# mycrazycracy/speaker-embedding-with-phonetic-information

Hardware: AMD Instinct MI355X
Metric: utterance-embeddings/sec (400-frame chunks) (higher is better)
Workload: dtype fp16mx; 1 GPU; v2_xvector TDNN, 256 chunks x 400 frames per GPU per step, utterance-sharded, weights broadcast once over RCCL; topology=v2_xvector, batch_chunks_per_gpu=256, frames_per_chunk=400, precision=default, arithmetic=fp16mx, lanes=2, output_node=embedding, chunk_lengths=400, library=xvec_hip 0.4 (gfx950; kernels 1123b5fc04a88fd3)

## Files before the change

### include/xvec_hip.h

```cpp
#ifndef XVEC_HIP_H_
#define XVEC_HIP_H_

#include <stddef.h>
#include <stdint.h>

#ifdef __cplusplus
extern "C" {
#endif

typedef enum {
  XV_OK = 0,
  XV_ERR_IO = 1,
  XV_ERR_MODEL = 2,
  XV_ERR_DEVICE = 3,
  XV_ERR_ARG = 4,
  XV_ERR_INTERNAL = 5
} xv_status;

typedef enum {
  XV_PREC_DEFAULT = -1,
  XV_PREC_BF16X3 = 0,
  XV_PREC_BF16 = 1,
  XV_PREC_FP16 = 2,
  XV_PREC_FP16X3 = 3,
// ... 55 lines not shown
  int32_t lite_dropped;
  float tail;
} xv_calibration;
xv_status xv_ctx_calibrate(xv_ctx* c, const float* feats, const int32_t* row_offsets, int32_t B, float tol, xv_calibration* out);
xv_status xv_ctx_set_fast_mode(xv_ctx* c, int32_t precision);
xv_status xv_ctx_fast_mode(const xv_ctx* c, int32_t* precision);
xv_status xv_ctx_set_lite_layers(xv_ctx* c, uint64_t mask);
xv_status xv_ctx_lite_layers(const xv_ctx* c, uint64_t* mask);
xv_status xv_calibrate_table(xv_ctx* c, const char* feature_rspecifier, int32_t chunk_size, int32_t min_chunk_size,
                             int32_t pad_input, int32_t max_utts, float tol, xv_calibration* out);
xv_status xv_ctx_set_calibration(xv_ctx* c, int32_t enable, float tol);
xv_status xv_calibration_file_read(const char* path, int32_t* found, uint64_t* model, int32_t* precision, uint64_t* lite_mask);
xv_status xv_calibration_file_publish(const char* path, uint64_t model, int32_t precision, uint64_t lite_mask, float tol,
                                      const char* note, int32_t* published, uint64_t* adopted_model, int32_t* adopted_precision,
                                      uint64_t* adopted_lite_mask);
xv_status xv_ctx_model_fingerprint(const xv_ctx* c, uint64_t* fingerprint);
xv_status xv_ctx_share_calibration(xv_ctx* c, const char* path, float tol, const char* note, int32_t* outcome);
xv_status xv_ctx_set_calibration_file(xv_ctx* c, const char* path);

xv_status xv_ctx_set_profiling(xv_ctx* c, int32_t enable);
size_t xv_ctx_profile_report(xv_ctx* c, char* buf, size_t n);

xv_status xv_extract_utterances(xv_ctx* c, const float* feats, const int32_t* row_offsets, int32_t n_utts,
                                int32_t chunk_size, int32_t min_chunk_size, int32_t pad_input, float* out,
                                int32_t* ok);

xv_status xv_extract_table(xv_ctx* c, const char* feature_rspecifier, const char* vector_wspecifier, int32_t chunk_size,
                           int32_t min_chunk_size, int32_t pad_input, int32_t batch_frames, int64_t* num_done,
                           int64_t* num_failed);

xv_status xv_recognize_feature_pipeline(const char* rspecifier, int32_t* found, char* feats, size_t feats_cap, char* vad, size_t vad_cap,
                                        int32_t* cmn_window, int32_t* min_cmn_window, int32_t* center);
xv_status xv_frontend_cmvn_select(xv_ctx* c, const float* raw, const int32_t* raw_off, int32_t n_utts, const float* vad,
                                  int32_t cmn_window, int32_t center, float* out, int32_t* out_off);

xv_status xv_plan_chunks(int32_t num_rows, int32_t chunk_size, int32_t min_chunk_size, int32_t pad_input,
                         int32_t min_net_frames, int32_t cap, int32_t* start, int32_t* len, int32_t* left_pad,
                         int32_t* right_pad, int32_t* n_chunks);

xv_status xv_ctx_create_broadcast(const xv_model* m, const int* devices, int n, int precision, xv_ctx** out);

xv_status xv_backend_apply(int device, const float* x, int32_t n, int32_t dim, const float* mean, const float* transform,
                           int32_t t_rows, int32_t t_cols, int32_t normalize, int32_t scaleup, float* out, float* ratio);
xv_status xv_segment_mean(int device, const float* x, int32_t n, int32_t dim, const int32_t* seg_off, const int32_t* idx,
                          int32_t n_seg, int32_t acc64, float* out);

xv_status xv_scatter_stats(int device, const float* x, int32_t n, int32_t dim, const int32_t* seg_off, const int32_t* idx,
                           int32_t n_seg, double* s_tot, double* sums, double* s_bet, float* device_ms);
xv_status xv_plda_transform(int device, const float* x, int32_t n, int32_t dim, const double* transform, const double* offset,
                            const double* psi, const double* num, int32_t normalize, int32_t simple, float* y, double* scale,
                            float* device_ms);
xv_status xv_plda_score(int device, const float* u, const double* num_u, int32_t n_u, const float* v, int32_t n_v, int32_t dim,
                        const double* psi, const int32_t* trials, int64_t n_trials, double* scores, float* device_ms);
xv_status xv_lda_estimate(int32_t dim, int64_t n, const double* s_tot, const double* s_bet, const float* mean,
                          double total_covariance_factor, double covariance_floor, int32_t lda_dim, float* out, int32_t* n_floored);
xv_status xv_plda_estimate(int32_t dim, int32_t n_spk, const double* sums, const int32_t* counts, const double* s_tot,
                           const double* s_bet, int32_t num_em_iters, double* mean, double* transform, double* psi,
                           int32_t* n_floored);
xv_status xv_plda_adapt(int32_t dim, int64_t n, const double* m, const double* v, const double* mean, const double* transform,
                        const double* psi, double mean_diff_scale, double within_covar_scale, double between_covar_scale,
                        double* mean_out, double* transform_out, double* psi_out, double* s_out);

typedef struct {
  float sample_frequency, frame_length_ms, frame_shift_ms, dither, preemphasis_coefficient, blackman_coeff;
  int32_t remove_dc_offset, window_type, round_to_power_of_two, snip_edges;
  int32_t num_mel_bins;
  float low_freq, high_freq;
  int32_t num_ceps;
  float cepstral_lifter;
  int32_t use_energy, raw_energy;
  float energy_floor;
} xv_mfcc_options;
typedef struct {
  float vad_energy_threshold, vad_energy_mean_scale, vad_proportion_threshold;
  int32_t vad_frames_context;
} xv_vad_options;
void xv_mfcc_options_default(xv_mfcc_options* opts);
int64_t xv_mfcc_num_frames(const xv_mfcc_options* opts, int64_t n_samples);
uint64_t xv_mfcc_utt_seed(const char* key);
xv_status xv_mfcc_compute(int device, const xv_mfcc_options* opts, const float* samples, const int64_t* sample_offsets,
                          int32_t n_utts, const uint64_t* utt_seeds, float* out, int32_t* out_row_offsets);
xv_status xv_mfcc_compute_i16(int device, const xv_mfcc_options* opts, const int16_t* samples, const int64_t* sample_offsets,
                              int32_t n_utts, const uint64_t* utt_seeds, float* out, int32_t* out_row_offsets);
xv_status xv_mfcc_kernel_time(int device, const xv_mfcc_options* opts, const int16_t* samples, const int64_t* sample_offsets,
                              int32_t n_utts, int32_t reps, float* kernel_ms);
xv_status xv_vad_energy(int device, const xv_vad_options* vad_opts, const float* feats, const int32_t* row_offsets,
                        int32_t n_utts, int32_t dim, float* out);
xv_status xv_wave_read(const char* rxfilename, int32_t channel, int32_t* rate, int16_t** samples, int64_t* n);
void xv_wave_free(int16_t* samples);

typedef struct {
  int32_t shift_output, normalize_output;
  float duration, volume;
  int32_t input_wave_channel, rir_channel, noise_channel;
} xv_reverb_options;
void xv_reverb_options_default(xv_reverb_options* opts);
int64_t xv_reverb_output_length(const xv_reverb_options* opts, float sample_rate, int64_t n_samples, int64_t rir_len);
xv_status xv_wav_reverberate(int device, const xv_reverb_options* opts, float sample_rate, const void* samples,
                             int32_t samples_are_i16, const int64_t* sample_offsets, int32_t n_utts, const float* rirs,
                             const int64_t* rir_offsets, int32_t n_rirs, const int32_t* utt_rir, const float* noises,
                             const int64_t* noise_offsets, int32_t n_noises, const int32_t* utt_add_offsets,
                             const int32_t* add_noise, const float* add_snr, const float* add_start, int64_t* out_offsets,
                             float* out_f32, int16_t* out_i16, int64_t* clipped);
xv_status xv_reverb_kernel_time(int device, const xv_reverb_options* opts, float sample_rate, const void* samples,
                                int32_t samples_are_i16, const int64_t* sample_offsets, int32_t n_utts, const float* rirs,
                                const int64_t* rir_offsets, int32_t n_rirs, const int32_t* utt_rir, const float* noises,
                                const int64_t* noise_offsets, int32_t n_noises, const int32_t* utt_add_offsets,
                                const int32_t* add_noise, const float* add_snr, const float* add_start, int32_t reps,
                                float* kernel_ms);
xv_status xv_recognize_wav_pipeline(const char* rxfilename, int32_t* found, char* description, size_t description_cap);
xv_status xv_wave_write(const char* wxfilename, int32_t rate, const float* samples, int64_t n, int64_t* clipped);

typedef struct {
  const void* hi;
  const void* lo;
  int32_t ld;
  int32_t row_shift;
  int32_t k_len;
  const void* gmax;
  const void* lo4; const void* lo4_scale;
} xv_seg_desc;
typedef struct {
  int32_t precision, epilogue;
  int32_t nseg;
  xv_seg_desc seg[8];
  const void* w_hi; const void* w_lo; int32_t ldw;
  int32_t rows;
  int32_t n_pad;
  const float* bias; const float* scale; const float* offset;
  int32_t relu, bn;
  void* out_hi; void* out_lo; int32_t ldo;
  float* out_f32; int32_t ldf; int32_t m_valid;
  float* partial; int32_t ldp; const int8_t* grp_range;
  void* hip_stream;
  const void* w4; int32_t ldw4; const void* w4_scale;
  void* gmax_out;
  const void* w4b; int32_t ldw4b; const void* w4b_scale;
  void* out_lo4; void* out_lo4_scale;
  int32_t p8;
  const int8_t* out_range;
  int32_t ksplit;
} xv_gemm_desc;
xv_status xv_pack_mx_residual(const float* w, const uint16_t* w_hi_f16, int32_t n_pad, int32_t nseg,
                              const int32_t* seg_src, const int32_t* seg_shift, const int32_t* seg_klen, uint8_t* w4,
                              uint8_t* w4_scale);
xv_status xv_pack_mx_residual64(const float* w, const uint16_t* w_hi_f16, int32_t n_pad, int32_t nseg, const int32_t* seg_src,
                                const int32_t* seg_shift, const int32_t* seg_klen, uint8_t* w4, uint8_t* w4_scale);
xv_status xv_pack_mx_weights(const float* w, int32_t n_pad, int32_t nseg, const int32_t* seg_src, const int32_t* seg_shift,
                             const int32_t* seg_klen, uint8_t* w4b, uint8_t* w4b_scale);
xv_status xv_pack_mx_weights64(const float* w, int32_t n_pad, int32_t nseg, const int32_t* seg_src, const int32_t* seg_shift,
                               const int32_t* seg_klen, uint8_t* w4b, uint8_t* w4b_scale);
xv_status xv_tile_mx_scales(const uint8_t* natural, int32_t n_pad, int32_t k_len, int32_t epilogue, uint8_t* tiled);
xv_status xv_kernel_tdnn_gemm(const xv_gemm_desc* d);

xv_status xv_compressed_size(int32_t rows, int32_t cols, int32_t method, size_t* nbytes, const char** format);
xv_status xv_compress_matrices(int device, const float* feats, const int32_t* row_off, int32_t n, int32_t cols, int32_t method,
                               uint8_t* out_bytes, int64_t* out_off, int32_t* nonfinite_flags);
xv_status xv_compress_kernel_time(int device, const float* feats, const int32_t* row_off, int32_t n, int32_t cols, int32_t method,
                                  int32_t reps, float* kernel_ms);
xv_status xv_cmvn_sliding(int device, const float* raw, const int32_t* raw_off, int32_t n, int32_t cols, int32_t cmn_window,
                          int32_t min_cmn_window, int32_t center, float* out);

xv_status xv_cmvn_stats(int device, const float* feats, const int32_t* row_off, int32_t n_utts, int32_t cols, double* stats,
                        float* device_ms);
xv_status xv_cmvn_norm(const double* stats, int32_t cols, int32_t norm_means, int32_t norm_vars, int32_t reverse,
                       const int32_t* skip_dims, int32_t n_skip, float* norm, int32_t* num_floored);
xv_status xv_cmvn_apply(int device, const float* feats, const int32_t* row_off, int32_t n_utts, int32_t cols, const float* norms,
                        const int32_t* utt_norm, float* out);
xv_status xv_cmvn_kernel_time(int device, const float* feats, const int32_t* row_off, int32_t n_utts, int32_t cols, int32_t reps,
                              float* stats_ms, float* apply_ms);

typedef struct {
  const float* feats;
  const int32_t* row_offsets;
  const int32_t* dev_off;
  int32_t B;
  int32_t rows;
  int32_t pad_left, pad_right;
  int32_t dim, noff;
  int32_t off[8];
  const void* w_hi; const void* w_lo;
  int32_t ldw, seg_pad;
  int32_t n_pad;
  int32_t epi_prec;
  const float* bias; const float* scale; const float* offset;
  int32_t relu, bn;
  void* out_hi; void* out_lo; int32_t ldo;
  void* out_lo4; void* out_lo4_scale;
  void* gmax_out; const int8_t* out_range;
  int32_t row0, nrows;
  int32_t max_wgs;
  void* hip_stream;
} xv_first_layer_desc;
xv_status xv_kernel_first_layer(const xv_first_layer_desc* d);
typedef struct {
  int32_t precision;
  const float* feats; const int32_t* src_off; const int32_t* dev_off; const int32_t* grp_utt;
  int32_t rows;
  int32_t dim, ld;
  void* out_hi; void* out_lo;
  int32_t pad_left, pad_right;
  void* zero_words; int32_t n_zero_words;
  void* hip_stream;
} xv_prep_input_desc;
xv_status xv_kernel_prep_input(const xv_prep_input_desc* d);
typedef struct {
  int32_t precision;
  const float* partial; int32_t ldp;
  const int32_t* utt_grp0; const int32_t* utt_grp1; const int32_t* utt_count;
  int32_t B, dim;
  float var_floor;
  void* out_hi; void* out_lo; int32_t ld;
  void* hip_stream;
} xv_pool_finalise_desc;
xv_status xv_kernel_pool_finalise(const xv_pool_finalise_desc* d);
typedef struct {
  const float* src; const void* src16; int32_t ld;
  const int32_t* out_row; int32_t n_out;
  int32_t dim, log_softmax;
  float* out; int32_t out_ld;
  void* hip_stream;
} xv_frame_output_desc;
xv_status xv_kernel_frame_output(const xv_frame_output_desc* d);

#ifdef __cplusplus
}
#endif
#endif
```

### speaker-embedding-with-phonetic-information_amd/__init__.py

```python
import ctypes
import os
import subprocess
import sys

_HERE = os.path.dirname(os.path.abspath(__file__))
CSRC = os.path.join(_HERE, "csrc")
LIB_PATH = os.environ.get("XVEC_LIB") or os.path.join(_HERE, "libxvec_hip.so")
BIN_DIR = os.path.join(_HERE, "bin")

XV_OK = 0
XV_ERR_IO, XV_ERR_MODEL, XV_ERR_DEVICE, XV_ERR_ARG, XV_ERR_INTERNAL = 1, 2, 3, 4, 5
PREC_BF16X3, PREC_BF16, PREC_FP16, PREC_FP16X3, PREC_FP16X2, PREC_AUTO, PREC_FP16MX, PREC_FP16MX2, PREC_FP16X3E = range(9)
PREC_DEFAULT = -1
PRECISIONS = {"default": PREC_DEFAULT, "bf16x3": PREC_BF16X3, "bf16": PREC_BF16, "fp16": PREC_FP16, "fp16x3": PREC_FP16X3,
              "fp16x2": PREC_FP16X2, "auto": PREC_AUTO, "fp16mx": PREC_FP16MX, "fp16mx2": PREC_FP16MX2}
PRECISION_NAMES = {v: k for k, v in PRECISIONS.items()}
MFMA_PASSES = {"bf16x3": 3, "bf16": 1, "fp16": 1, "fp16x3": 3, "fp16x2": 2, "fp16mx": 1.25}
EPI_ACT, EPI_F32, EPI_STATS = 0, 1, 2


class XvError(RuntimeError):
    def __init__(self, status, msg):
        super().__init__("xvec_hip status %d: %s" % (status, msg))
        self.status = status


class ModelInfo(ctypes.Structure):
    _fields_ = [(n, ctypes.c_int32) for n in ("input_dim", "output_dim", "left_context", "right_context",
                                              "min_frames", "num_layers", "output_is_segment", "reserved")]


class SegDesc(ctypes.Structure):
    _fields_ = [("hi", ctypes.c_void_p), ("lo", ctypes.c_void_p), ("ld", ctypes.c_int32),
                ("row_shift", ctypes.c_int32), ("k_len", ctypes.c_int32), ("gmax", ctypes.c_void_p),
                ("lo4", ctypes.c_void_p), ("lo4_scale", ctypes.c_void_p)]


class GemmDesc(ctypes.Structure):
    _fields_ = [("precision", ctypes.c_int32), ("epilogue", ctypes.c_int32), ("nseg", ctypes.c_int32),
                ("seg", SegDesc * 8),
                ("w_hi", ctypes.c_void_p), ("w_lo", ctypes.c_void_p), ("ldw", ctypes.c_int32),
                ("rows", ctypes.c_int32), ("n_pad", ctypes.c_int32),
                ("bias", ctypes.c_void_p), ("scale", ctypes.c_void_p), ("offset", ctypes.c_void_p),
                ("relu", ctypes.c_int32), ("bn", ctypes.c_int32),
                ("out_hi", ctypes.c_void_p), ("out_lo", ctypes.c_void_p), ("ldo", ctypes.c_int32),
                ("out_f32", ctypes.c_void_p), ("ldf", ctypes.c_int32), ("m_valid", ctypes.c_int32),
                ("partial", ctypes.c_void_p), ("ldp", ctypes.c_int32), ("grp_range", ctypes.c_void_p),
                ("hip_stream", ctypes.c_void_p),
                ("w4", ctypes.c_void_p), ("ldw4", ctypes.c_int32), ("w4_scale", ctypes.c_void_p),
                ("gmax_out", ctypes.c_void_p),
                ("w4b", ctypes.c_void_p), ("ldw4b", ctypes.c_int32), ("w4b_scale", ctypes.c_void_p),
                ("out_lo4", ctypes.c_void_p), ("out_lo4_scale", ctypes.c_void_p),
                ("p8", ctypes.c_int32),
                ("out_range", ctypes.c_void_p), ("ksplit", ctypes.c_int32)]


class FirstLayerDesc(ctypes.Structure):
    _fields_ = [("feats", ctypes.c_void_p), ("row_offsets", ctypes.c_void_p), ("dev_off", ctypes.c_void_p), ("B", ctypes.c_int32),
                ("rows", ctypes.c_int32), ("pad_left", ctypes.c_int32), ("pad_right", ctypes.c_int32),
                ("dim", ctypes.c_int32), ("noff", ctypes.c_int32), ("off", ctypes.c_int32 * 8),
                ("w_hi", ctypes.c_void_p), ("w_lo", ctypes.c_void_p), ("ldw", ctypes.c_int32), ("seg_pad", ctypes.c_int32),
                ("n_pad", ctypes.c_int32), ("epi_prec", ctypes.c_int32),
                ("bias", ctypes.c_void_p), ("scale", ctypes.c_void_p), ("offset", ctypes.c_void_p),
                ("relu", ctypes.c_int32), ("bn", ctypes.c_int32),
                ("out_hi", ctypes.c_void_p), ("out_lo", ctypes.c_void_p), ("ldo", ctypes.c_int32),
                ("out_lo4", ctypes.c_void_p), ("out_lo4_scale", ctypes.c_void_p),
                ("gmax_out", ctypes.c_void_p), ("out_range", ctypes.c_void_p),
                ("row0", ctypes.c_int32), ("nrows", ctypes.c_int32), ("max_wgs", ctypes.c_int32),
                ("hip_stream", ctypes.c_void_p)]


class PrepInputDesc(ctypes.Structure):
    _fields_ = [("precision", ctypes.c_int32), ("feats", ctypes.c_void_p), ("src_off", ctypes.c_void_p), ("dev_off", ctypes.c_void_p),
                ("grp_utt", ctypes.c_void_p), ("rows", ctypes.c_int32), ("dim", ctypes.c_int32), ("ld", ctypes.c_int32),
                ("out_hi", ctypes.c_void_p), ("out_lo", ctypes.c_void_p), ("pad_left", ctypes.c_int32), ("pad_right", ctypes.c_int32),
                ("zero_words", ctypes.c_void_p), ("n_zero_words", ctypes.c_int32), ("hip_stream", ctypes.c_void_p)]


class PoolFinaliseDesc(ctypes.Structure):
    _fields_ = [("precision", ctypes.c_int32), ("partial", ctypes.c_void_p), ("ldp", ctypes.c_int32),
                ("utt_grp0", ctypes.c_void_p), ("utt_grp1", ctypes.c_void_p), ("utt_count", ctypes.c_void_p),
                ("B", ctypes.c_int32), ("dim", ctypes.c_int32), ("var_floor", ctypes.c_float),
                ("out_hi", ctypes.c_void_p), ("out_lo", ctypes.c_void_p), ("ld", ctypes.c_int32), ("hip_stream", ctypes.c_void_p)]


class FrameOutputDesc(ctypes.Structure):
    _fields_ = [("src", ctypes.c_void_p), ("src16", ctypes.c_void_p), ("ld", ctypes.c_int32),
                ("out_row", ctypes.c_void_p), ("n_out", ctypes.c_int32), ("dim", ctypes.c_int32), ("log_softmax", ctypes.c_int32),
                ("out", ctypes.c_void_p), ("out_ld", ctypes.c_int32), ("hip_stream", ctypes.c_void_p)]


class Calibration(ctypes.Structure):
    _fields_ = [("chosen", ctypes.c_int32), ("checked", ctypes.c_int32), ("err_mx", ctypes.c_float), ("err_mx2", ctypes.c_float),
                ("checked_mx", ctypes.c_int32), ("err_lite", ctypes.c_float), ("lite_mask", ctypes.c_uint64),
                ("err_holdout", ctypes.c_float), ("checked_holdout", ctypes.c_int32), ("lite_dropped", ctypes.c_int32),
                ("tail", ctypes.c_float)]

    def as_dict(self):
        d = {"chosen": PRECISION_NAMES.get(self.chosen, str(self.chosen)), "checked": self.checked, "checked_mx": self.checked_mx,
             "err_mx": self.err_mx, "err_mx2": self.err_mx2, "tail": self.tail}
        if self.lite_mask:
            d["lite_mask"] = int(self.lite_mask)
            d["err_lite"] = self.err_lite
            d["err_holdout"] = self.err_holdout
            d["checked_holdout"] = self.checked_holdout
        if self.lite_dropped:
            d["lite_dropped"] = self.lite_dropped
        return d


ABI_SYMBOLS = [
    "xv_last_error", "xv_version", "xv_model_load", "xv_model_load_rxfilename", "xv_model_free", "xv_model_info",
    "xv_model_macs", "xv_model_describe", "xv_model_pack", "xv_ctx_create", "xv_ctx_create_from_blob",
    "xv_ctx_create_from_device_blob", "xv_ctx_free",
    "xv_ctx_info", "xv_forward_batch", "xv_forward_batch_device", "xv_ctx_synchronize", "xv_ctx_set_profiling",
    "xv_ctx_profile_report", "xv_extract_utterances", "xv_ctx_calibrate", "xv_ctx_set_fast_mode", "xv_ctx_fast_mode",
    "xv_calibrate_table", "xv_ctx_set_calibration", "xv_ctx_model_fingerprint", "xv_ctx_share_calibration",
    "xv_ctx_set_calibration_file", "xv_calibration_file_read", "xv_calibration_file_publish", "xv_recognize_feature_pipeline", "xv_ctx_set_lite_layers", "xv_ctx_lite_layers",
    "xv_extract_table", "xv_frontend_cmvn_select", "xv_plan_chunks", "xv_ctx_create_broadcast", "xv_kernel_tdnn_gemm",
    "xv_backend_apply", "xv_segment_mean", "xv_scatter_stats", "xv_plda_transform", "xv_plda_score", "xv_lda_estimate",
    "xv_plda_estimate", "xv_plda_adapt",
    "xv_mfcc_options_default", "xv_mfcc_num_frames", "xv_mfcc_utt_seed", "xv_mfcc_compute", "xv_mfcc_compute_i16", "xv_mfcc_kernel_time", "xv_vad_energy",
    "xv_reverb_options_default", "xv_reverb_output_length", "xv_wav_reverberate", "xv_reverb_kernel_time", "xv_wave_write", "xv_recognize_wav_pipeline",
    "xv_compressed_size", "xv_compress_matrices", "xv_compress_kernel_time", "xv_cmvn_sliding",
    "xv_cmvn_stats", "xv_cmvn_norm", "xv_cmvn_apply", "xv_cmvn_kernel_time",
    "xv_kernel_first_layer", "xv_kernel_prep_input", "xv_kernel_pool_finalise", "xv_kernel_frame_output",
    "xv_wave_read", "xv_wave_free", "xv_pack_mx_residual", "xv_pack_mx_residual64", "xv_tile_mx_scales", "xv_pack_mx_weights", "xv_pack_mx_weights64",
]

_lib = None


def build(verbose=False):
    cmd = ["make", "-C", CSRC, "-j8"]
    res = subprocess.run(cmd, stdout=subprocess.PIPE, stderr=subprocess.STDOUT, text=True)
    if verbose or res.returncode != 0:
        print(res.stdout)
    if res.returncode != 0:
        raise RuntimeError("building libxvec_hip.so failed")
    return LIB_PATH


def lib():
    global _lib
    if _lib is not None:
        return _lib
    if not os.path.exists(LIB_PATH):
        raise ImportError("%s is missing - run `python -c 'import __graft_entry__ as g; g.build()'` "
                          "(there is no Python/CPU fallback for the HIP path)" % LIB_PATH)
    if os.environ.get("XVEC_NO_TORCH_PRELOAD", "") != "1":
        try:
            import torch
        except Exception:
            pass
    L = ctypes.CDLL(LIB_PATH)
    L.xv_last_error.restype = ctypes.c_char_p
    L.xv_version.restype = ctypes.c_char_p
    L.xv_model_macs.restype = ctypes.c_double
    L.xv_model_macs.argtypes = [ctypes.c_void_p, ctypes.c_int32]
    L.xv_model_describe.restype = ctypes.c_size_t
    L.xv_model_describe.argtypes = [ctypes.c_void_p, ctypes.c_char_p, ctypes.c_size_t]
    L.xv_model_load.argtypes = [ctypes.c_void_p, ctypes.c_size_t, ctypes.c_char_p, ctypes.c_char_p,
                                ctypes.POINTER(ctypes.c_void_p)]
    L.xv_model_load_rxfilename.argtypes = [ctypes.c_char_p, ctypes.c_char_p, ctypes.c_char_p,
                                           ctypes.POINTER(ctypes.c_void_p)]
    L.xv_model_free.argtypes = [ctypes.c_void_p]
    L.xv_model_free.restype = None
    L.xv_model_info.argtypes = [ctypes.c_void_p, ctypes.POINTER(ModelInfo)]
    L.xv_model_pack.argtypes = [ctypes.c_void_p, ctypes.c_int, ctypes.c_void_p, ctypes.POINTER(ctypes.c_size_t)]
    L.xv_ctx_create.argtypes = [ctypes.c_void_p, ctypes.c_int, ctypes.c_int, ctypes.POINTER(ctypes.c_void_p)]
    L.xv_ctx_create_from_blob.argtypes = [ctypes.c_void_p, ctypes.c_size_t, ctypes.c_int,
                                          ctypes.POINTER(ctypes.c_void_p)]
    L.xv_ctx_create_from_device_blob.argtypes = [ctypes.c_void_p, ctypes.c_size_t, ctypes.c_int,
                                                 ctypes.POINTER(ctypes.c_void_p)]
    L.xv_pack_mx_residual.argtypes = [ctypes.c_void_p, ctypes.c_void_p, ctypes.c_int32, ctypes.c_int32, ctypes.c_void_p,
                                      ctypes.c_void_p, ctypes.c_void_p, ctypes.c_void_p, ctypes.c_void_p]
    L.xv_pack_mx_residual64.argtypes = L.xv_pack_mx_residual.argtypes
    L.xv_pack_mx_weights.argtypes = [ctypes.c_void_p, ctypes.c_int32, ctypes.c_int32, ctypes.c_void_p, ctypes.c_void_p,
                                     ctypes.c_void_p, ctypes.c_void_p, ctypes.c_void_p]
    L.xv_pack_mx_weights64.argtypes = L.xv_pack_mx_weights.argtypes
    L.xv_tile_mx_scales.argtypes = [ctypes.c_void_p, ctypes.c_int32, ctypes.c_int32, ctypes.c_int32, ctypes.c_void_p]
    L.xv_ctx_free.argtypes = [ctypes.c_void_p]
    L.xv_ctx_free.restype = None
    L.xv_ctx_info.argtypes = [ctypes.c_void_p, ctypes.POINTER(ModelInfo), ctypes.POINTER(ctypes.c_int32),
                              ctypes.POINTER(ctypes.c_int32)]
    L.xv_forward_batch.argtypes = [ctypes.c_void_p, ctypes.c_void_p, ctypes.c_void_p, ctypes.c_int32, ctypes.c_void_p]
    L.xv_forward_batch_device.argtypes = [ctypes.c_void_p, ctypes.c_void_p, ctypes.c_void_p, ctypes.c_int32,
                                          ctypes.c_void_p, ctypes.c_int32, ctypes.c_void_p]
    L.xv_ctx_synchronize.argtypes = [ctypes.c_void_p]
    L.xv_ctx_set_profiling.argtypes = [ctypes.c_void_p, ctypes.c_int32]
    L.xv_ctx_profile_report.argtypes = [ctypes.c_void_p, ctypes.c_char_p, ctypes.c_size_t]
    L.xv_ctx_profile_report.restype = ctypes.c_size_t
    L.xv_extract_utterances.argtypes = [ctypes.c_void_p, ctypes.c_void_p, ctypes.c_void_p, ctypes.c_int32,
                                        ctypes.c_int32, ctypes.c_int32, ctypes.c_int32, ctypes.c_void_p, ctypes.c_void_p]
    L.xv_ctx_create_broadcast.argtypes = [ctypes.c_void_p, ctypes.POINTER(ctypes.c_int), ctypes.c_int, ctypes.c_int,
                                          ctypes.POINTER(ctypes.c_void_p)]
    L.xv_kernel_tdnn_gemm.argtypes = [ctypes.POINTER(GemmDesc)]
    L.xv_kernel_first_layer.argtypes = [ctypes.POINTER(FirstLayerDesc)]
    L.xv_kernel_prep_input.argtypes = [ctypes.POINTER(PrepInputDesc)]
    L.xv_kernel_pool_finalise.argtypes = [ctypes.POINTER(PoolFinaliseDesc)]
    L.xv_kernel_frame_output.argtypes = [ctypes.POINTER(FrameOutputDesc)]
    L.xv_ctx_calibrate.argtypes = [ctypes.c_void_p, ctypes.c_void_p, ctypes.c_void_p, ctypes.c_int32, ctypes.c_float,
                                   ctypes.POINTER(Calibration)]
    L.xv_ctx_set_fast_mode.argtypes = [ctypes.c_void_p, ctypes.c_int32]
    L.xv_ctx_fast_mode.argtypes = [ctypes.c_void_p, ctypes.POINTER(ctypes.c_int32)]
    L.xv_ctx_set_lite_layers.argtypes = [ctypes.c_void_p, ctypes.c_uint64]
    L.xv_ctx_lite_layers.argtypes = [ctypes.c_void_p, ctypes.POINTER(ctypes.c_uint64)]
    L.xv_calibrate_table.argtypes = [ctypes.c_void_p, ctypes.c_char_p, ctypes.c_int32, ctypes.c_int32, ctypes.c_int32,
                                     ctypes.c_int32, ctypes.c_float, ctypes.POINTER(Calibration)]
    L.xv_ctx_set_calibration.argtypes = [ctypes.c_void_p, ctypes.c_int32, ctypes.c_float]
    L.xv_ctx_model_fingerprint.argtypes = [ctypes.c_void_p, ctypes.POINTER(ctypes.c_uint64)]
    L.xv_ctx_share_calibration.argtypes = [ctypes.c_void_p, ctypes.c_char_p, ctypes.c_float, ctypes.c_char_p,
                                           ctypes.POINTER(ctypes.c_int32)]
    L.xv_ctx_set_calibration_file.argtypes = [ctypes.c_void_p, ctypes.c_char_p]
    L.xv_calibration_file_read.argtypes = [ctypes.c_char_p, ctypes.POINTER(ctypes.c_int32), ctypes.POINTER(ctypes.c_uint64),
                                           ctypes.POINTER(ctypes.c_int32), ctypes.POINTER(ctypes.c_uint64)]
    L.xv_calibration_file_publish.argtypes = [ctypes.c_char_p, ctypes.c_uint64, ctypes.c_int32, ctypes.c_uint64, ctypes.c_float,
                                              ctypes.c_char_p, ctypes.POINTER(ctypes.c_int32), ctypes.POINTER(ctypes.c_uint64),
                                              ctypes.POINTER(ctypes.c_int32), ctypes.POINTER(ctypes.c_uint64)]
    _lib = L
    return L


def _check(status):
    if status != XV_OK:
        raise XvError(status, lib().xv_last_error().decode(errors="replace"))


class Model:

    def __init__(self, raw=None, rxfilename=None, nnet_config=None, output_node=None):
        L = lib()
        self._h = ctypes.c_void_p()
        cfg = nnet_config.encode() if nnet_config else None
        node = output_node.encode() if output_node else None
        if raw is not None:
            buf = ctypes.create_string_buffer(bytes(raw), len(raw))
            _check(L.xv_model_load(buf, len(raw), cfg, node, ctypes.byref(self._h)))
        else:
            _check(L.xv_model_load_rxfilename(rxfilename.encode(), cfg, node, ctypes.byref(self._h)))

    def __del__(self):
        if getattr(self, "_h", None) and self._h.value and lib is not None:
            lib().xv_model_free(self._h)
            self._h = ctypes.c_void_p()

    @property
    def info(self):
        mi = ModelInfo()
        _check(lib().xv_model_info(self._h, ctypes.byref(mi)))
        return mi

    def macs(self, frames):
        return lib().xv_model_macs(self._h, int(frames))

    def describe(self):
        n = lib().xv_model_describe(self._h, None, 0)
        buf = ctypes.create_string_buffer(n)
        lib().xv_model_describe(self._h, buf, n)
        return buf.value.decode()

    def pack(self, precision=PREC_DEFAULT):
        n = ctypes.c_size_t(0)
        _check(lib().xv_model_pack(self._h, precision, None, ctypes.byref(n)))
        buf = ctypes.create_string_buffer(n.value)
        _check(lib().xv_model_pack(self._h, precision, buf, ctypes.byref(n)))
        return buf.raw[:n.value]


class Context:

    def __init__(self, model=None, blob=None, device=0, precision=PREC_DEFAULT, device_blob=None):
# ... 608 lines not shown
                add_noise.append(len(noise_list) - 1)
                add_snr.append(snr)
                add_start.append(start)
            add_off[u + 1] = len(add_noise)
    noise_flat, noise_off = _ragged(noise_list, np.float32)
    add_noise = np.array(add_noise + [0], dtype=np.int32)
    add_snr = np.array(add_snr + [0], dtype=np.float32)
    add_start = np.array(add_start + [0], dtype=np.float32)
    lens = [reverb_output_length(off[u + 1] - off[u], rir_off[utt_rir[u] + 1] - rir_off[utt_rir[u]] if utt_rir[u] >= 0 else 0,
                                 rate, options=o) for u in range(n)]
    total = max(1, sum(max(0, x) for x in lens))
    common = (device, ctypes.byref(o), float(rate), samples.ctypes.data, 1 if i16 else 0, off.ctypes.data, n,
              rir_flat.ctypes.data, rir_off.ctypes.data, len(rir_list), utt_rir.ctypes.data,
              noise_flat.ctypes.data, noise_off.ctypes.data, len(noise_list), add_off.ctypes.data if additive is not None else None,
              add_noise.ctypes.data, add_snr.ctypes.data, add_start.ctypes.data)
    if kernel_time_reps > 0:
        L.xv_reverb_kernel_time.argtypes = _REVERB_ARGTYPES + [ctypes.c_int32, ctypes.POINTER(ctypes.c_float)]
        ms = ctypes.c_float(0)
        _check(L.xv_reverb_kernel_time(*common, int(kernel_time_reps), ctypes.byref(ms)))
        return ms.value
    out = np.empty(total, dtype=np.float32)
    out16 = np.empty(total, dtype=np.int16) if return_int16 else None
    clipped = np.zeros(max(1, n), dtype=np.int64)
    out_off = np.zeros(n + 1, dtype=np.int64)
    L.xv_wav_reverberate.argtypes = _REVERB_ARGTYPES + [ctypes.c_void_p, ctypes.c_void_p, ctypes.c_void_p, ctypes.c_void_p]
    _check(L.xv_wav_reverberate(*common, out_off.ctypes.data, out.ctypes.data, out16.ctypes.data if return_int16 else None,
                                clipped.ctypes.data))
    assert list(np.diff(out_off)) == [max(0, x) for x in lens]
    if return_int16:
        return [(out[out_off[u]:out_off[u + 1]].copy(), out16[out_off[u]:out_off[u + 1]].copy(), int(clipped[u])) for u in range(n)]
    return [out[out_off[u]:out_off[u + 1]].copy() for u in range(n)]


def _pack_matrices(mats, what):
    import numpy as np
    ms = [np.ascontiguousarray(m, dtype=np.float32) for m in mats]
    if any(m.ndim != 2 for m in ms):
        raise XvError(XV_ERR_ARG, "%s: every matrix must be two-dimensional" % what)
    widths = {m.shape[1] for m in ms if m.shape[0] > 0}
    if len(widths) > 1:
        raise XvError(XV_ERR_ARG, "%s: the matrices of one call share their column count" % what)
    cols = widths.pop() if widths else 0
    off = np.zeros(len(ms) + 1, dtype=np.int32)
    off[1:] = np.cumsum([m.shape[0] if cols else 0 for m in ms])
    rows = [m for m in ms if m.shape[0] > 0 and cols]
    packed = np.concatenate(rows, axis=0) if rows else np.zeros((0, max(cols, 1)), np.float32)
    return np.ascontiguousarray(packed), off, cols


def compressed_size(rows, cols, method=1):
    L = lib()
    n, fmt = ctypes.c_size_t(0), ctypes.c_char_p()
    L.xv_compressed_size.argtypes = [ctypes.c_int32, ctypes.c_int32, ctypes.c_int32, ctypes.POINTER(ctypes.c_size_t),
                                     ctypes.POINTER(ctypes.c_char_p)]
    _check(L.xv_compressed_size(rows, cols, method, ctypes.byref(n), ctypes.byref(fmt)))
    return int(n.value), fmt.value.decode()


def compress(mats, method=1, device=0, return_flags=False, kernel_time_reps=0):
    import numpy as np
    L = lib()
    packed, off, cols = _pack_matrices(mats, "compress")
    n = len(off) - 1
    common = [device, packed.ctypes.data if packed.size else None, off.ctypes.data, n, cols, method]
    types = [ctypes.c_int, ctypes.c_void_p, ctypes.c_void_p, ctypes.c_int32, ctypes.c_int32, ctypes.c_int32]
    if kernel_time_reps > 0:
        ms = ctypes.c_float(0)
        L.xv_compress_kernel_time.argtypes = types + [ctypes.c_int32, ctypes.POINTER(ctypes.c_float)]
        _check(L.xv_compress_kernel_time(*common, int(kernel_time_reps), ctypes.byref(ms)))
        return ms.value
    total = sum(compressed_size(int(off[u + 1] - off[u]), cols, method)[0] for u in range(n))
    out = np.zeros(max(1, total), dtype=np.uint8)
    out_off = np.zeros(n + 1, dtype=np.int64)
    flags = np.zeros(max(1, n), dtype=np.int32)
    L.xv_compress_matrices.argtypes = types + [ctypes.c_void_p, ctypes.c_void_p, ctypes.c_void_p]
    _check(L.xv_compress_matrices(*common, out.ctypes.data, out_off.ctypes.data, flags.ctypes.data))
    assert int(out_off[n]) == total
    objs = [out[out_off[u]:out_off[u + 1]].tobytes() for u in range(n)]
    return (objs, [bool(f) for f in flags[:n]]) if return_flags else objs


def cmvn_sliding(mats, cmn_window=600, min_cmn_window=100, center=False, device=0):
    import numpy as np
    L = lib()
    packed, off, cols = _pack_matrices(mats, "cmvn_sliding")
    n = len(off) - 1
    out = np.empty_like(packed)
    L.xv_cmvn_sliding.argtypes = [ctypes.c_int, ctypes.c_void_p, ctypes.c_void_p, ctypes.c_int32, ctypes.c_int32, ctypes.c_int32,
                                  ctypes.c_int32, ctypes.c_int32, ctypes.c_void_p]
    _check(L.xv_cmvn_sliding(device, packed.ctypes.data if packed.size else None, off.ctypes.data, n, max(cols, 1), cmn_window,
                             min_cmn_window, 1 if center else 0, out.ctypes.data if out.size else None))
    return [out[off[u]:off[u + 1]].copy() for u in range(n)]


def cmvn_stats(feats_list, device=0, kernel_time_reps=0):
    import numpy as np
    L = lib()
    packed, off, cols = _pack_matrices(feats_list, "cmvn_stats")
    n = len(off) - 1
    if cols < 1:
        raise XvError(XV_ERR_ARG, "cmvn_stats: no matrix with rows and columns")
    if kernel_time_reps > 0:
        a, b = ctypes.c_float(0), ctypes.c_float(0)
        L.xv_cmvn_kernel_time.argtypes = [ctypes.c_int, ctypes.c_void_p, ctypes.c_void_p, ctypes.c_int32, ctypes.c_int32, ctypes.c_int32,
                                          ctypes.POINTER(ctypes.c_float), ctypes.POINTER(ctypes.c_float)]
        _check(L.xv_cmvn_kernel_time(device, packed.ctypes.data, off.ctypes.data, n, cols, int(kernel_time_reps), ctypes.byref(a),
                                     ctypes.byref(b)))
        return a.value, b.value
    stats = np.zeros((n, 2, cols + 1), dtype=np.float64)
    L.xv_cmvn_stats.argtypes = [ctypes.c_int, ctypes.c_void_p, ctypes.c_void_p, ctypes.c_int32, ctypes.c_int32, ctypes.c_void_p,
                                ctypes.c_void_p]
    _check(L.xv_cmvn_stats(device, packed.ctypes.data if packed.size else None, off.ctypes.data, n, cols, stats.ctypes.data, None))
    return stats


def cmvn_norm(stats, norm_means=True, norm_vars=False, reverse=False, skip_dims=(), return_floored=False):
    import numpy as np
    L = lib()
    st = np.ascontiguousarray(stats, dtype=np.float64)
    if st.ndim != 2 or st.shape[0] != 2 or st.shape[1] < 2:
        raise XvError(XV_ERR_ARG, "cmvn_norm: the statistics are a [2][cols + 1] matrix")
    cols = st.shape[1] - 1
    skip = np.ascontiguousarray(list(skip_dims), dtype=np.int32)
    norm = np.zeros((2, cols), dtype=np.float32)
    floored = ctypes.c_int32(0)
    L.xv_cmvn_norm.argtypes = [ctypes.c_void_p, ctypes.c_int32, ctypes.c_int32, ctypes.c_int32, ctypes.c_int32, ctypes.c_void_p,
                               ctypes.c_int32, ctypes.c_void_p, ctypes.POINTER(ctypes.c_int32)]
    _check(L.xv_cmvn_norm(st.ctypes.data, cols, int(bool(norm_means)), int(bool(norm_vars)), int(bool(reverse)),
                          skip.ctypes.data if skip.size else None, int(skip.size), norm.ctypes.data, ctypes.byref(floored)))
    return (norm, int(floored.value)) if return_floored else norm


def apply_cmvn(feats_list, norms, utt_norm, device=0):
    import numpy as np
    L = lib()
    packed, off, cols = _pack_matrices(feats_list, "apply_cmvn")
    n = len(off) - 1
    nm = np.ascontiguousarray(norms, dtype=np.float32)
    un = np.ascontiguousarray(utt_norm, dtype=np.int32)
    if un.shape != (n,) or nm.ndim != 3 or nm.shape[1:] != (2, max(cols, 1)) or (n and (un.min() < 0 or un.max() >= nm.shape[0])):
        raise XvError(XV_ERR_ARG, "apply_cmvn: norms are [n_norms][2][cols] and utt_norm names one of them per matrix")
    out = np.empty_like(packed)
    L.xv_cmvn_apply.argtypes = [ctypes.c_int, ctypes.c_void_p, ctypes.c_void_p, ctypes.c_int32, ctypes.c_int32, ctypes.c_void_p,
                                ctypes.c_void_p, ctypes.c_void_p]
    _check(L.xv_cmvn_apply(device, packed.ctypes.data if packed.size else None, off.ctypes.data, n, max(cols, 1), nm.ctypes.data,
                           un.ctypes.data, out.ctypes.data if out.size else None))
    return [out[off[u]:off[u + 1]].copy() for u in range(n)]


def kernel_tdnn_gemm(desc):
    _check(lib().xv_kernel_tdnn_gemm(ctypes.byref(desc)))


def kernel_first_layer(desc):
    _check(lib().xv_kernel_first_layer(ctypes.byref(desc)))


def kernel_prep_input(desc):
    _check(lib().xv_kernel_prep_input(ctypes.byref(desc)))


def kernel_pool_finalise(desc):
    _check(lib().xv_kernel_pool_finalise(ctypes.byref(desc)))


def kernel_frame_output(desc):
    _check(lib().xv_kernel_frame_output(ctypes.byref(desc)))


def pack_mx_residual(w, w_hi_f16, segs, walk64=False):
    import numpy as np
    w = np.ascontiguousarray(w, dtype=np.float32)
    hi = np.ascontiguousarray(w_hi_f16, dtype=np.uint16)
    n_pad, K = w.shape
    src = np.array([s[0] for s in segs], dtype=np.int32)
    shift = np.array([s[1] for s in segs], dtype=np.int32)
    klen = np.array([s[2] for s in segs], dtype=np.int32)
    assert int(klen.sum()) == K and K % 128 == 0
    w4 = np.zeros((n_pad, K // 128 * 64), dtype=np.uint8)
    sc = np.zeros((n_pad, K // 32), dtype=np.uint8)
    fn = lib().xv_pack_mx_residual64 if walk64 else lib().xv_pack_mx_residual
    _check(fn(w.ctypes.data, hi.ctypes.data, n_pad, len(segs), src.ctypes.data, shift.ctypes.data,
              klen.ctypes.data, w4.ctypes.data, sc.ctypes.data))
    return w4, sc


def pack_mx_weights(w, segs, walk64=False):
    import numpy as np
    w = np.ascontiguousarray(w, dtype=np.float32)
    n_pad, K = w.shape
    src = np.array([s[0] for s in segs], dtype=np.int32)
    shift = np.array([s[1] for s in segs], dtype=np.int32)
    klen = np.array([s[2] for s in segs], dtype=np.int32)
    assert int(klen.sum()) == K and np.all(klen % (256 if walk64 else 128) == 0)
    w4b = np.zeros((n_pad, 2 * K if walk64 else K // 2), dtype=np.uint8)
    sc = np.zeros((n_pad, K // 32), dtype=np.uint8)
    fn = lib().xv_pack_mx_weights64 if walk64 else lib().xv_pack_mx_weights
    _check(fn(w.ctypes.data, n_pad, len(segs), src.ctypes.data, shift.ctypes.data, klen.ctypes.data, w4b.ctypes.data, sc.ctypes.data))
    return w4b, sc


def tile_mx_scales(scales, epilogue):
    import numpy as np
    sc = np.ascontiguousarray(scales, dtype=np.uint8)
    out = np.zeros(sc.size, dtype=np.uint8)
    _check(lib().xv_tile_mx_scales(sc.ctypes.data, sc.shape[0], sc.shape[1] * 32, int(epilogue), out.ctypes.data))
    return out
```

### speaker-embedding-with-phonetic-information_amd/csrc/capi.cc

```cpp
#include <dlfcn.h>
#include <stdlib.h>
#include <string.h>

#include <algorithm>
#include <memory>
#include <string>
#include <vector>

#include "../../include/xvec_hip.h"
#include "backend.h"
#include "cmvn.h"
#include "compress.h"
#include "engine.h"
#include "extractor.h"
#include "feat.h"
#include "reverb.h"
#include "wave.h"
#include "kernels.h"
#include "calib_file.h"
#include "fuse_pipe.h"
#include "fuse_wav.h"
#include "multi_gpu.h"
#include "nnet3_raw.h"
#include "plda.h"
#include "plda_kernels.h"
#include "program.h"
#include "table_extract.h"

struct xv_model {
  xv::TdnnProgram prog;
};

struct xv_ctx {
  std::unique_ptr<xv::Engine> eng;
  bool calibrate = false;
  float calibrate_tol = 7.5e-5f;
  std::string calibration_file;
};

namespace {

thread_local std::string g_err;

xv_status Fail(xv_status s, const std::string& m) {
  g_err = m;
  return s;
}

template <class F>
xv_status Guard(F&& f) {
  try {
    g_err.clear();
    return f();
  } catch (const xv::KioError& e) {
    return Fail(XV_ERR_IO, e.what());
  } catch (const xv::EngineError& e) {
    return Fail(XV_ERR_DEVICE, e.what());
  } catch (const std::bad_alloc&) {
    return Fail(XV_ERR_INTERNAL, "out of host memory");
  } catch (const std::exception& e) {
    return Fail(XV_ERR_INTERNAL, e.what());
  } catch (...) {
    return Fail(XV_ERR_INTERNAL, "unknown exception");
  }
}

void FillInfo(const xv::BlobInfo& b, xv_model_info_t* info) {
  memset(info, 0, sizeof *info);
  info->input_dim = b.input_dim;
  info->output_dim = b.output_dim;
  info->left_context = b.left_context;
  info->right_context = b.right_context;
  info->min_frames = b.min_frames;
  info->num_layers = (int32_t)b.layers.size();
  info->output_is_segment = b.output_is_segment;
}

xv_status LoadCommon(xv::RawNnet& net, const char* nnet_config, const char* output_node, xv_model** out) {
  if (nnet_config && *nnet_config) net.ApplyNnetConfig(nnet_config);
  std::unique_ptr<xv_model> m(new xv_model);
  try {
    m->prog = xv::LowerToProgram(net, output_node && *output_node ? output_node : "output");
  } catch (const xv::KioError& e) {
    return Fail(XV_ERR_MODEL, e.what());
  }
  *out = m.release();
  return XV_OK;
}

}

extern "C" {

const char* xv_last_error(void) { return g_err.c_str(); }
#ifndef XVEC_KERNELS_SHA
#define XVEC_KERNELS_SHA "unknown"
#endif
#ifdef XVEC_SCHED_FUZZ
#define XVEC_BUILD_KIND "; schedule-fuzzing build"
#else
#define XVEC_BUILD_KIND ""
#endif
const char* xv_version(void) { return "xvec_hip 0.4 (gfx950; kernels " XVEC_KERNELS_SHA XVEC_BUILD_KIND ")"; }

xv_status xv_model_load(const void* raw, size_t n, const char* nnet_config, const char* output_node, xv_model** out) {
  if (!raw || !out) return Fail(XV_ERR_ARG, "xv_model_load: null argument");
  return Guard([&] {
    xv::RawNnet net;
    net.Read(std::string((const char*)raw, n));
    return LoadCommon(net, nnet_config, output_node, out);
  });
}

xv_status xv_model_load_rxfilename(const char* rxfilename, const char* nnet_config, const char* output_node,
                                   xv_model** out) {
  if (!rxfilename || !out) return Fail(XV_ERR_ARG, "xv_model_load_rxfilename: null argument");
  return Guard([&] {
    xv::RawNnet net;
    net.ReadFrom(rxfilename);
    return LoadCommon(net, nnet_config, output_node, out);
  });
}

void xv_model_free(xv_model* m) { delete m; }

xv_status xv_model_info(const xv_model* m, xv_model_info_t* info) {
  if (!m || !info) return Fail(XV_ERR_ARG, "xv_model_info: null argument");
  memset(info, 0, sizeof *info);
  info->input_dim = m->prog.input_dim;
  info->output_dim = m->prog.output_dim;
  info->left_context = m->prog.left_context;
  info->right_context = m->prog.right_context;
  info->min_frames = m->prog.min_frames;
  info->num_layers = (int32_t)m->prog.layers.size();
  info->output_is_segment = m->prog.output_is_segment;
  return XV_OK;
}

double xv_model_macs(const xv_model* m, int32_t frames) { return m ? m->prog.Macs(frames) : 0.0; }

size_t xv_model_describe(const xv_model* m, char* buf, size_t n) {
  if (!m) return 0;
  const std::string s = m->prog.Describe();
  if (buf && n) {
    const size_t k = s.size() < n - 1 ? s.size() : n - 1;
    memcpy(buf, s.data(), k);
    buf[k] = 0;
  }
  return s.size() + 1;
}

xv_status xv_model_pack(const xv_model* m, int precision, void* blob, size_t* nbytes) {
  if (!m || !nbytes) return Fail(XV_ERR_ARG, "xv_model_pack: null argument");
  return Guard([&] {
    std::vector<uint8_t> b = xv::PackModelPolicy(m->prog, precision);
    if (blob) {
      if (*nbytes < b.size()) return Fail(XV_ERR_ARG, "xv_model_pack: buffer too small");
      memcpy(blob, b.data(), b.size());
    }
    *nbytes = b.size();
    return XV_OK;
  });
}

xv_status xv_ctx_create(const xv_model* m, int device, int precision, xv_ctx** out) {
  if (!m || !out) return Fail(XV_ERR_ARG, "xv_ctx_create: null argument");
  return Guard([&] {
    std::vector<uint8_t> b = xv::PackModelPolicy(m->prog, precision);
    std::unique_ptr<xv_ctx> c(new xv_ctx);
    c->eng.reset(new xv::Engine(b.data(), b.size(), device));
    *out = c.release();
// ... 724 lines not shown
    size_t total = 0;
    for (int u = 0; u < n; ++u) {
      size_t nb = 0;
      xv::CompressedSize(row_off[u + 1] - row_off[u], cols, method, &nb, nullptr);
      total += nb;
    }
    std::vector<uint8_t> out(total + 1);
    float best = 0.f;
    for (int r = 0; r <= reps; ++r) {
      float ms = 0.f;
      xv::CompressMatrices(device, feats, row_off, n, cols, method, out.data(), off.data(), nullptr, &ms);
      if (r == 1 || (r > 1 && ms < best)) best = ms;
    }
    *kernel_ms = best;
    return XV_OK;
  });
}

xv_status xv_cmvn_sliding(int device, const float* raw, const int32_t* raw_off, int32_t n, int32_t cols, int32_t cmn_window,
                          int32_t min_cmn_window, int32_t center, float* out) {
  if (n < 0 || cols < 1 || !raw_off) return Fail(XV_ERR_ARG, "xv_cmvn_sliding: bad argument");
  return Guard([&] {
    xv::CmvnSliding(device, raw, raw_off, n, cols, cmn_window, min_cmn_window, center != 0, out);
    return XV_OK;
  });
}

xv_status xv_cmvn_stats(int device, const float* feats, const int32_t* row_off, int32_t n_utts, int32_t cols, double* stats,
                        float* device_ms) {
  if (n_utts < 0 || cols < 1 || !row_off || (n_utts > 0 && !stats)) return Fail(XV_ERR_ARG, "xv_cmvn_stats: bad argument");
  return Guard([&] {
    xv::CmvnStats(device, feats, row_off, n_utts, cols, stats, device_ms);
    return XV_OK;
  });
}

xv_status xv_cmvn_norm(const double* stats, int32_t cols, int32_t norm_means, int32_t norm_vars, int32_t reverse,
                       const int32_t* skip_dims, int32_t n_skip, float* norm, int32_t* num_floored) {
  return Guard([&] {
    try {
      const int floored = xv::CmvnNorm(stats, cols, norm_means != 0, norm_vars != 0, reverse != 0, skip_dims, n_skip, norm);
      if (num_floored) *num_floored = floored;
    } catch (const xv::CmvnArgError& e) {
      return Fail(XV_ERR_ARG, e.what());
    }
    return XV_OK;
  });
}

xv_status xv_cmvn_apply(int device, const float* feats, const int32_t* row_off, int32_t n_utts, int32_t cols, const float* norms,
                        const int32_t* utt_norm, float* out) {
  if (n_utts < 0 || cols < 1 || !row_off || (n_utts > 0 && (!utt_norm || !norms))) return Fail(XV_ERR_ARG, "xv_cmvn_apply: bad argument");
  int n_norms = 0;
  for (int u = 0; u < n_utts; ++u) {
    if (utt_norm[u] < 0) return Fail(XV_ERR_ARG, "xv_cmvn_apply: negative norm index");
    n_norms = utt_norm[u] + 1 > n_norms ? utt_norm[u] + 1 : n_norms;
  }
  return Guard([&] {
    xv::CmvnApply(device, feats, row_off, n_utts, cols, norms, n_norms, utt_norm, out);
    return XV_OK;
  });
}

xv_status xv_cmvn_kernel_time(int device, const float* feats, const int32_t* row_off, int32_t n_utts, int32_t cols, int32_t reps,
                              float* stats_ms, float* apply_ms) {
  if (!feats || !row_off || !stats_ms || !apply_ms || n_utts < 1 || cols < 1 || reps < 1)
    return Fail(XV_ERR_ARG, "xv_cmvn_kernel_time: bad argument");
  return Guard([&] {
    std::vector<double> stats((size_t)n_utts * 2 * (cols + 1));
    std::vector<float> norms((size_t)n_utts * 2 * cols), out((size_t)row_off[n_utts] * cols);
    std::vector<int32_t> utt_norm(n_utts);
    float best_s = 0.f, best_a = 0.f;
    for (int r = 0; r <= reps; ++r) {
      float ms = 0.f;
      xv::CmvnStats(device, feats, row_off, n_utts, cols, stats.data(), &ms);
      if (r == 1 || (r > 1 && ms < best_s)) best_s = ms;
      if (r == 0)
        for (int u = 0; u < n_utts; ++u) {
          utt_norm[u] = u;
          xv::CmvnNorm(stats.data() + (size_t)u * 2 * (cols + 1), cols, true, true, false, nullptr, 0, norms.data() + (size_t)u * 2 * cols);
        }
      xv::CmvnApply(device, feats, row_off, n_utts, cols, norms.data(), n_utts, utt_norm.data(), out.data(), &ms);
      if (r == 1 || (r > 1 && ms < best_a)) best_a = ms;
    }
    *stats_ms = best_s;
    *apply_ms = best_a;
    return XV_OK;
  });
}

xv_status xv_ctx_create_broadcast(const xv_model* m, const int* devices, int n, int precision, xv_ctx** out) {
  if (!m || !devices || !out || n < 1) return Fail(XV_ERR_ARG, "xv_ctx_create_broadcast: bad argument");
  return Guard([&]() -> xv_status {
    const std::vector<uint8_t> blob = xv::PackModelPolicy(m->prog, precision);
    std::vector<std::unique_ptr<xv::Engine>> engines = xv::CreateEnginesBroadcast(blob, std::vector<int>(devices, devices + n));
    for (int i = 0; i < n; ++i) {
      xv_ctx* c = new xv_ctx;
      c->eng = std::move(engines[i]);
      out[i] = c;
    }
    return XV_OK;
  });
}

xv_status xv_kernel_tdnn_gemm(const xv_gemm_desc* d) {
  if (!d) return Fail(XV_ERR_ARG, "xv_kernel_tdnn_gemm: null descriptor");
  return Guard([&] {
    if (d->nseg < 1 || d->nseg > xv::kMaxSeg || d->rows % xv::kBM || d->n_pad % xv::kBN)
      return Fail(XV_ERR_ARG, "xv_kernel_tdnn_gemm: bad geometry");
    xv::GemmArgs a;
    memset(&a, 0, sizeof a);
    a.nseg = d->nseg;
    for (int j = 0; j < d->nseg; ++j) {
      if (d->seg[j].k_len % xv::kBK) return Fail(XV_ERR_ARG, "xv_kernel_tdnn_gemm: k_len must be a multiple of 32");
      a.seg[j].hi = (const uint16_t*)d->seg[j].hi;
      a.seg[j].lo = (const uint16_t*)d->seg[j].lo;
      a.seg[j].ld = d->seg[j].ld;
      a.seg[j].row_shift = d->seg[j].row_shift;
      a.seg[j].ksteps = d->seg[j].k_len / xv::kBK;
      a.seg[j].gmax = (const unsigned*)d->seg[j].gmax;
      a.seg[j].lo4 = (const uint8_t*)d->seg[j].lo4;
      a.seg[j].lo4s = (const uint8_t*)d->seg[j].lo4_scale;
      a.total_ksteps += a.seg[j].ksteps;
    }
    a.w_hi = (const uint16_t*)d->w_hi;
    a.w_lo = (const uint16_t*)d->w_lo;
    a.ldw = d->ldw;
    a.m_tiles = d->rows / xv::kBM;
    a.n_tiles = d->n_pad / xv::kBN;
    a.relu = d->relu;
    a.bn = d->bn;
    a.bias = d->bias;
    a.scale = d->scale;
    a.offset = d->offset;
    a.out_hi = (uint16_t*)d->out_hi;
    a.out_lo = (uint16_t*)d->out_lo;
    a.ldo = d->ldo;
    a.out_f32 = d->out_f32;
    a.ldf = d->ldf;
    a.m_valid = d->m_valid;
    a.partial = d->partial;
    a.ldp = d->ldp;
    a.grp_range = d->grp_range;
    a.w4 = (const uint8_t*)d->w4;
    a.ldw4 = d->ldw4;
    a.w4_scale = (const uint8_t*)d->w4_scale;
    a.gmax_out = (unsigned*)d->gmax_out;
    a.w4b = (const uint8_t*)d->w4b;
    a.ldw4b = d->ldw4b;
    a.w4b_scale = (const uint8_t*)d->w4b_scale;
    a.out_lo4 = (uint8_t*)d->out_lo4;
    a.out_lo4s = (uint8_t*)d->out_lo4_scale;
    a.p8 = d->p8;
    a.out_range = d->out_range;
    if (d->ksplit > 1) {
      if (d->precision < xv::kPrecBf16x3 || d->precision > xv::kPrecFp16x3 || a.p8 ||
          (d->epilogue != xv::kEpiAct && d->epilogue != xv::kEpiF32))
        return Fail(XV_ERR_ARG, "xv_kernel_tdnn_gemm: split-K needs XV_PREC_BF16X3 .. XV_PREC_FP16X3, epilogue 0 or 1 and no p8");
      a.ksteps_per_slice = xv::SplitKStepsPerSlice(a.total_ksteps);
      a.ksplit = (a.total_ksteps + a.ksteps_per_slice - 1) / a.ksteps_per_slice;
      if (a.ksplit != d->ksplit)
        return Fail(XV_ERR_ARG, "xv_kernel_tdnn_gemm: " + std::to_string(a.total_ksteps) + " K steps are split over " +
                                    std::to_string(a.ksplit) + " slices, not " + std::to_string(d->ksplit));
      void* ws = nullptr;
      hipError_t e = hipMalloc(&ws, (size_t)a.ksplit * d->rows * d->n_pad * 4);
      if (e != hipSuccess) return Fail(XV_ERR_DEVICE, std::string("hipMalloc(split-K workspace): ") + hipGetErrorString(e));
      a.splitk_ws = (float*)ws;
      e = xv::launch_tdnn_gemm(a, d->precision, d->epilogue, (hipStream_t)d->hip_stream);
      const hipError_t e2 = hipStreamSynchronize((hipStream_t)d->hip_stream);
      (void)hipFree(ws);
      if (e != hipSuccess || e2 != hipSuccess)
        return Fail(XV_ERR_DEVICE, std::string("tdnn_gemm split-K launch: ") + hipGetErrorString(e != hipSuccess ? e : e2));
      return XV_OK;
    }
    if (a.p8) {
      if (!xv::gemm_p8_applicable(a, d->precision) || (d->epilogue != xv::kEpiAct && d->epilogue != xv::kEpiStats))
        return Fail(XV_ERR_ARG, "xv_kernel_tdnn_gemm: p8 needs XV_PREC_FP16, XV_PREC_FP16MX or XV_PREC_FP16MX2, epilogue 0 or 2, rows and n_pad "
                                "multiples of 256, K groups of whole 64-column tiles (128-column blocks for XV_PREC_FP16MX, 256 for XV_PREC_FP16MX2)");
    } else
    if (d->precision == xv::kPrecFp16Mx2 && !xv::gemm_mx2_applicable(a))
      return Fail(XV_ERR_ARG, "xv_kernel_tdnn_gemm: XV_PREC_FP16MX2 needs what XV_PREC_FP16MX needs and the 4-bit planes of the "
                              "weights and of every source (whole 128-column steps)");
    if (!a.p8 && d->precision == xv::kPrecFp16Mx && !xv::gemm_mx_applicable(a))
      return Fail(XV_ERR_ARG, "xv_kernel_tdnn_gemm: XV_PREC_FP16MX needs the residual plane, a group-max table per source, "
                              "K groups of whole 128-column blocks and an even number of 128-row tiles");
    hipError_t e = xv::launch_tdnn_gemm(a, d->precision, d->epilogue, (hipStream_t)d->hip_stream);
    if (e != hipSuccess) return Fail(XV_ERR_DEVICE, std::string("tdnn_gemm launch: ") + hipGetErrorString(e));
    return XV_OK;
  });
}

namespace {
struct DevMem {
  void* p = nullptr;
  ~DevMem() {
    if (p) (void)hipFree(p);
  }
  hipError_t Alloc(size_t n) { return hipMalloc(&p, n ? n : 1); }
};
}

xv_status xv_kernel_first_layer(const xv_first_layer_desc* d) {
  if (!d) return Fail(XV_ERR_ARG, "xv_kernel_first_layer: null descriptor");
  return Guard([&] {
    const char* who = "xv_kernel_first_layer: ";
    if (!d->feats || !d->row_offsets || !d->dev_off || !d->w_hi || !d->w_lo || !d->bias || !d->out_hi || (d->bn && (!d->scale || !d->offset)))
      return Fail(XV_ERR_ARG, std::string(who) + "a required pointer is null");
    const int p = d->epi_prec;
    if (p != xv::kPrecBf16x3 && p != xv::kPrecFp16x3 && p != xv::kPrecFp16x2 && p != xv::kPrecFp16x3E)
      return Fail(XV_ERR_ARG, std::string(who) + "epi_prec must be XV_PREC_BF16X3, XV_PREC_FP16X3, XV_PREC_FP16X2 or XV_PREC_FP16X3E");
    if ((p == xv::kPrecBf16x3 || p == xv::kPrecFp16x3) && !d->out_lo) return Fail(XV_ERR_ARG, std::string(who) + "the split planes need out_lo");
    if (p == xv::kPrecFp16x3E && (!d->out_lo4 || !d->out_lo4_scale))
      return Fail(XV_ERR_ARG, std::string(who) + "XV_PREC_FP16X3E needs out_lo4 and out_lo4_scale");
    if (d->B < 1 || d->rows < xv::kFirstRows || d->rows % xv::kFirstRows || d->n_pad < xv::kBN || d->n_pad % xv::kBN ||
        d->ldo < d->n_pad || d->ldo % 64 || d->pad_left < 0 || d->pad_right < 0)
      return Fail(XV_ERR_ARG, std::string(who) + "bad geometry (rows: multiple of 64, n_pad: multiple of 128, ldo: multiple of 64, >= n_pad)");
    if (d->nrows < xv::kFirstRows || d->nrows % xv::kFirstRows || d->row0 < 0 || d->row0 % xv::kFirstRows || d->row0 + (long)d->nrows > d->rows)
      return Fail(XV_ERR_ARG, std::string(who) + "row0 and nrows must be multiples of 64 inside [0, rows]");
    if (d->dim < 1 || d->noff < 1 || d->noff > 8) return Fail(XV_ERR_ARG, std::string(who) + "dim >= 1 and 1 .. 8 offsets");
    int off[8];
    for (int j = 0; j < d->noff; ++j) {
      off[j] = d->off[j];
      if (off[j] < -15 || off[j] > 15) return Fail(XV_ERR_ARG, std::string(who) + "time offsets beyond +-15 frames");
    }
    if (!xv::FirstLayerApplicable(d->dim, d->noff, off))
      return Fail(XV_ERR_ARG, std::string(who) + "tdnn_first_kernel cannot run this shape (dim rounded up to 8 must be <= 24, noff x that <= 128, "
                                                 "and (64 + offset span) x that <= 2048)");
    if (d->seg_pad < d->dim || (long)(d->noff - 1) * d->seg_pad + d->dim > d->ldw)
      return Fail(XV_ERR_ARG, std::string(who) + "the weight planes do not hold noff segments of dim columns");
    const int ngrp = d->rows / xv::kRowAlign;
    std::vector<int32_t> grp_utt(ngrp, -1);
    long next_free = 0;
    if (d->row_offsets[0] < 0) return Fail(XV_ERR_ARG, std::string(who) + "negative row offset");
    for (int b = 0; b < d->B; ++b) {
      const long len = (long)d->row_offsets[b + 1] - d->row_offsets[b];
      const long span = (len + d->pad_left + d->pad_right + xv::kRowAlign - 1) / xv::kRowAlign * xv::kRowAlign;
      if (len < 1 || d->dev_off[b] % xv::kRowAlign || d->dev_off[b] < next_free || d->dev_off[b] + span > d->rows)
        return Fail(XV_ERR_ARG, std::string(who) + "chunk " + std::to_string(b) + ": empty, not on a 16-row boundary, overlapping or beyond rows");
      next_free = d->dev_off[b] + span;
      for (long g = d->dev_off[b] / xv::kRowAlign; g < next_free / xv::kRowAlign; ++g) grp_utt[g] = b;
    }
    std::vector<int32_t> grp_src((size_t)ngrp * 4);
    xv::FillFirstGroupSources(ngrp, grp_utt.data(), d->dev_off, d->row_offsets, d->pad_left, d->pad_right, grp_src.data());
    hipStream_t s = (hipStream_t)d->hip_stream;
    DevMem tab, wch, wcl;
    const size_t wc_bytes = (size_t)d->n_pad * xv::kFirstK * 2;
    hipError_t e = tab.Alloc(grp_src.size() * 4);
    if (e == hipSuccess) e = wch.Alloc(wc_bytes);
    if (e == hipSuccess) e = wcl.Alloc(wc_bytes);
    if (e == hipSuccess) e = hipMemcpy(tab.p, grp_src.data(), grp_src.size() * 4, hipMemcpyHostToDevice);
    if (e != hipSuccess) return Fail(XV_ERR_DEVICE, std::string("first_layer tables: ") + hipGetErrorString(e));
    xv::FirstArgs fa;
    memset(&fa, 0, sizeof fa);
    fa.g.n_tiles = d->n_pad / xv::kBN;
    fa.g.m_tiles = d->rows / xv::kBM;
    fa.g.relu = d->relu;
    fa.g.bn = d->bn;
    fa.g.bias = d->bias;
    fa.g.scale = d->scale;
    fa.g.offset = d->offset;
    fa.g.out_hi = (uint16_t*)d->out_hi;
    fa.g.out_lo = (uint16_t*)d->out_lo;
    fa.g.ldo = d->ldo;
    fa.g.out_lo4 = (uint8_t*)d->out_lo4;
    fa.g.out_lo4s = (uint8_t*)d->out_lo4_scale;
    fa.g.gmax_out = (unsigned*)d->gmax_out;
    fa.g.out_range = d->out_range;
    fa.feats = d->feats;
    fa.feats_valid_idx = (long)d->row_offsets[0] * d->dim;
    fa.grp_src = (const int4*)tab.p;
    fa.rows = d->rows;
    fa.dim = d->dim;
    fa.row0 = d->row0;
    fa.nrows = d->nrows;
    fa.noff = d->noff;
    for (int j = 0; j < d->noff; ++j) fa.off[j] = off[j];
    fa.wc_hi = (const uint16_t*)wch.p;
    fa.wc_lo = (const uint16_t*)wcl.p;
    fa.max_wgs = d->max_wgs > 0 ? d->max_wgs : 0;
    e = xv::launch_compact_first((const uint16_t*)d->w_hi, d->ldw, d->seg_pad, d->n_pad, d->noff, d->dim, (uint16_t*)wch.p, s);
    if (e == hipSuccess) e = xv::launch_compact_first((const uint16_t*)d->w_lo, d->ldw, d->seg_pad, d->n_pad, d->noff, d->dim, (uint16_t*)wcl.p, s);
    if (e == hipSuccess) e = xv::launch_tdnn_first(fa, p, s);
    const hipError_t e2 = hipStreamSynchronize(s);
    if (e != hipSuccess || e2 != hipSuccess)
      return Fail(XV_ERR_DEVICE, std::string("tdnn_first launch: ") + hipGetErrorString(e != hipSuccess ? e : e2));
    return XV_OK;
  });
}

xv_status xv_kernel_prep_input(const xv_prep_input_desc* d) {
  if (!d) return Fail(XV_ERR_ARG, "xv_kernel_prep_input: null descriptor");
  return Guard([&] {
    if (d->precision < xv::kPrecBf16x3 || d->precision > xv::kPrecFp16x3) return Fail(XV_ERR_ARG, "xv_kernel_prep_input: precision must be 0 .. 3");
    const bool split = xv::PrecXPlanes(d->precision) == 2;
    if (!d->feats || !d->src_off || !d->dev_off || !d->grp_utt || !d->out_hi || (split && !d->out_lo))
      return Fail(XV_ERR_ARG, "xv_kernel_prep_input: a required pointer is null");
    if (d->rows < xv::kBM || d->rows % xv::kBM || d->ld < xv::kBK || d->ld % xv::kBK || d->dim < 1 || d->dim > d->ld || d->pad_left < 0 ||
        d->pad_right < 0 || d->n_zero_words < 0 || (d->n_zero_words > 0 && !d->zero_words))
      return Fail(XV_ERR_ARG, "xv_kernel_prep_input: bad geometry (rows: multiple of 128, ld: multiple of 32, >= dim)");
    xv::PrepArgs a;
    memset(&a, 0, sizeof a);
    a.feats = d->feats;
    a.src_off = d->src_off;
    a.dev_off = d->dev_off;
    a.grp_utt = d->grp_utt;
    a.rows = d->rows;
    a.dim = d->dim;
    a.ld = d->ld;
    a.out_hi = (uint16_t*)d->out_hi;
    a.out_lo = (uint16_t*)d->out_lo;
    a.pad_left = d->pad_left;
    a.pad_right = d->pad_right;
    a.zero_words = (unsigned*)d->zero_words;
    a.n_zero_words = d->n_zero_words;
    const hipError_t e = xv::launch_prep_input(a, d->precision, (hipStream_t)d->hip_stream);
    if (e != hipSuccess) return Fail(XV_ERR_DEVICE, std::string("prep_input launch: ") + hipGetErrorString(e));
    return XV_OK;
  });
}

xv_status xv_kernel_pool_finalise(const xv_pool_finalise_desc* d) {
  if (!d) return Fail(XV_ERR_ARG, "xv_kernel_pool_finalise: null descriptor");
  return Guard([&] {
    if (d->precision < xv::kPrecBf16x3 || d->precision > xv::kPrecFp16x3) return Fail(XV_ERR_ARG, "xv_kernel_pool_finalise: precision must be 0 .. 3");
    const bool split = xv::PrecXPlanes(d->precision) == 2;
    if (!d->partial || !d->utt_grp0 || !d->utt_grp1 || !d->utt_count || !d->out_hi || (split && !d->out_lo))
      return Fail(XV_ERR_ARG, "xv_kernel_pool_finalise: a required pointer is null");
    if (d->B < 1 || d->dim < 1 || d->ldp < d->dim || d->ld < 2 * d->dim)
      return Fail(XV_ERR_ARG, "xv_kernel_pool_finalise: bad geometry (ldp >= dim, ld >= 2 dim)");
    xv::PoolArgs a;
    memset(&a, 0, sizeof a);
    a.partial = d->partial;
    a.ldp = d->ldp;
    a.utt_grp0 = d->utt_grp0;
    a.utt_grp1 = d->utt_grp1;
    a.utt_count = d->utt_count;
    a.B = d->B;
    a.dim = d->dim;
    a.var_floor = d->var_floor;
    a.out_hi = (uint16_t*)d->out_hi;
    a.out_lo = (uint16_t*)d->out_lo;
    a.ld = d->ld;
    const hipError_t e = xv::launch_pool_finalise(a, d->precision, (hipStream_t)d->hip_stream);
// ... 120 lines not shown
```

### speaker-embedding-with-phonetic-information_amd/csrc/engine.cc

```cpp
#include "engine.h"
#include "knobs.h"

#include <stddef.h>
#include <time.h>
#include <stdlib.h>
#include <string.h>

#include <algorithm>
#include <atomic>
#include <cmath>
#include <exception>
#include <sstream>
#include <thread>

namespace xv {

namespace {

constexpr int kDefaultFastMinPooledMx2 = 160;
constexpr int kHalo = 32;
constexpr uint32_t kBlobVersion = 8;
constexpr uint64_t kNone = ~0ull;

uint64_t Hash64(const uint8_t* p, size_t n) {
// ... 483 lines not shown
        ok = ok && b.w4 != kNone && b.ldw4b == b.k_pad / 128 * 64 && inside(b.w4b, (uint64_t)b.n_pad * b.ldw4b) &&
             b.w4b_scale != kNone && inside(b.w4b_scale, 2 * (uint64_t)b.n_pad * (uint64_t)(b.k_pad / kBK));
      const uint64_t sc_bytes = 2 * (uint64_t)b.n_pad * (uint64_t)(b.k_pad / kBK);
      if (b.w4p != kNone)
        ok = ok && b.w4 != kNone && b.n_pad % 256 == 0 && inside(b.w4p, (uint64_t)b.n_pad * b.ldw4) && b.w4p_scale != kNone &&
             inside(b.w4p_scale, sc_bytes);
      else
        ok = ok && b.w4p_scale == kNone;
      if (b.w4bp != kNone)
        ok = ok && b.w4p != kNone && b.w4b != kNone && inside(b.w4bp, (uint64_t)b.n_pad * b.k_pad * 2) && b.w4bp_scale != kNone &&
             inside(b.w4bp_scale, sc_bytes);
      else
        ok = ok && b.w4bp_scale == kNone;
      if (!ok) throw EngineError("model blob: layer " + std::to_string(i) + " is inconsistent");
    }
    BlobLayerInfo li;
    li.name = b.name;
    li.in_dim = b.in_dim;
    li.out_dim = b.out_dim;
    li.k_pad = b.k_pad;
    li.n_pad = b.n_pad;
    li.relu = b.relu;
    li.bn = b.bn;
    li.log_softmax = b.log_softmax;
    li.segment_level = b.segment_level;
    li.left = b.left;
    li.right = b.right;
    li.has_w4 = b.w4 != kNone;
    li.has_w4b = b.w4b != kNone;
    li.has_w4p = b.w4p != kNone;
    for (int j = 0; j < b.nsrc; ++j) {
      LayerSource s;
      s.layer = b.src_layer[j];
      s.offset = b.src_offset[j];
      s.dim = b.src_dim[j];
      li.src.push_back(s);
    }
    info.layers.push_back(li);
  }
  return info;
}

double BlobInfo::Macs(int T) const {
  const int n = (int)layers.size();
  std::vector<int> nl(n, 1 << 30), nr(n, 1 << 30);
  const int root = output_is_segment ? pooled_layer : output_layer;
  nl[root] = layers[root].left;
  nr[root] = layers[root].right;
  for (int i = n - 1; i >= 0; --i) {
    if (layers[i].segment_level || nl[i] == (1 << 30)) continue;
    for (const LayerSource& s : layers[i].src)
      if (s.layer >= 0) {
        nl[s.layer] = std::min(nl[s.layer], nl[i] + s.offset);
        nr[s.layer] = std::min(nr[s.layer], nr[i] - s.offset);
      }
  }
  double macs = 0;
  for (int i = 0; i < n; ++i) {
    if (layers[i].segment_level) macs += (double)layers[i].in_dim * layers[i].out_dim;
    else if (nl[i] != (1 << 30)) macs += (double)layers[i].in_dim * layers[i].out_dim * std::max(0, T - nl[i] - nr[i]);
  }
  return macs;
}

void Engine::Check(hipError_t e, const char* what) const {
  if (e != hipSuccess) {
    std::ostringstream m;
    m << what << ": " << hipGetErrorString(e) << " (HIP error " << (int)e << ", device " << device_ << ")";
    throw EngineError(m.str());
  }
}

Engine::Engine(const uint8_t* blob, size_t n, int device, const void* device_image) : device_(device) {
  info_ = ParseBlobInfo(blob, n);
  int count = 0;
  hipError_t e = hipGetDeviceCount(&count);
  if (e != hipSuccess || count <= 0)
    throw EngineError("no HIP device available: this library has no CPU path (hipGetDeviceCount: " +
                      std::string(hipGetErrorString(e)) + ")");
  if (device < 0 || device >= count) throw EngineError("HIP device index out of range");
  Check(hipSetDevice(device_), "hipSetDevice");
  hipDeviceProp_t prop;
  Check(hipGetDeviceProperties(&prop, device_), "hipGetDeviceProperties");
  if (strncmp(prop.gcnArchName, "gfx950", 6) != 0)
    throw EngineError(std::string("kernels are built for gfx950 (MI355X) only; device is ") + prop.gcnArchName);
  frame_mode_ = !info_.output_is_segment;
  if (frame_mode_) {
    if (info_.pooled_layer >= 0) throw EngineError("a frame-level output that depends on statistics pooling is not supported");
    pad_left_ = info_.left_context;
    pad_right_ = info_.right_context;
  } else {
    if (info_.pooled_layer < 0) throw EngineError("model has no statistics pooling");
    for (size_t i = 0; i < info_.layers.size(); ++i)
      for (const LayerSource& s : info_.layers[i].src)
        if (s.layer == info_.pooled_layer)
          throw EngineError("the pooled layer must feed only the statistics pooling");
  }
  nplanes_ = PrecWPlanes(info_.precision);
  fast_mode_ = info_.precision;
  if (info_.precision == kPrecAuto || info_.precision == kPrecFp16Mx2) {
    const char* e = getenv("XVEC_FAST_MIN_POOLED");
    fast_min_pooled_ = (e && *e) ? atoi(e) : (info_.precision == kPrecAuto ? kDefaultFastMinPooled : kDefaultFastMinPooledMx2);
    mx2_min_pooled_ = (e && *e) ? atoi(e) : kDefaultFastMinPooledMx2;
    mx_min_pooled_ = (e && *e) ? atoi(e) : kDefaultFastMinPooled;
  }
  Check(hipStreamCreateWithFlags(&stream_, hipStreamNonBlocking), "hipStreamCreate");
  {
    const char* e = getenv("XVEC_LANES");
    int nl = e && *e ? atoi(e) : 2;
    if (nl < 1) nl = 1;
    if (nl > kMaxLanes) nl = kMaxLanes;
    lanes_.resize(nl);
    for (Lane& L : lanes_) {
      Check(hipStreamCreateWithFlags(&L.stream, hipStreamNonBlocking), "hipStreamCreate(lane)");
      Check(hipEventCreateWithFlags(&L.done, hipEventDisableTiming), "hipEventCreate(lane)");
      L.act.resize(info_.layers.size());
    }
  }

  BlobHeader h;
  memcpy(&h, blob, sizeof h);
  blob_data_bytes_ = (size_t)(h.total_bytes - h.data_offset);
  Check(hipMalloc(&d_blob_, blob_data_bytes_), "hipMalloc(weights)");
  if (device_image)
    Check(hipMemcpy(d_blob_, (const uint8_t*)device_image + h.data_offset, blob_data_bytes_, hipMemcpyDeviceToDevice),
          "hipMemcpy(weights, device to device)");
  else
    Check(hipMemcpy(d_blob_, blob + h.data_offset, blob_data_bytes_, hipMemcpyHostToDevice), "hipMemcpy(weights)");
  layers_.resize(info_.layers.size());
  for (size_t i = 0; i < layers_.size(); ++i) {
    BlobLayer b;
    memcpy(&b, blob + sizeof h + i * sizeof(BlobLayer), sizeof b);
    const uint8_t* base = (const uint8_t*)d_blob_;
    layers_[i].w_hi = (const uint16_t*)(base + b.w_hi);
    layers_[i].w_lo = b.w_lo == kNone ? nullptr : (const uint16_t*)(base + b.w_lo);
    layers_[i].bias = (const float*)(base + b.bias);
    layers_[i].scale = (const float*)(base + b.scale);
    layers_[i].offset = (const float*)(base + b.offset);
    layers_[i].w4 = b.w4 == kNone ? nullptr : base + b.w4;
    layers_[i].w4_scale = b.w4_scale == kNone ? nullptr : base + b.w4_scale;
    layers_[i].ldw4 = b.ldw4;
    layers_[i].w4b = b.w4b == kNone ? nullptr : base + b.w4b;
    layers_[i].w4b_scale = b.w4b_scale == kNone ? nullptr : base + b.w4b_scale;
    layers_[i].ldw4b = b.ldw4b;
    layers_[i].w4p = b.w4p == kNone ? nullptr : base + b.w4p;
    layers_[i].w4p_scale = b.w4p_scale == kNone ? nullptr : base + b.w4p_scale;
    layers_[i].w4bp = b.w4bp == kNone ? nullptr : base + b.w4bp;
    layers_[i].w4bp_scale = b.w4bp_scale == kNone ? nullptr : base + b.w4bp_scale;
  }
  Check(hipStreamSynchronize(nullptr), "hipStreamSynchronize(weights)");
  {
    use_p8_ = DebugKnobInt("p8", 1) != 0;
    p8_whole_ = DebugKnobInt("p8_whole", 0);
  }
  in_ld_ = RoundUp(info_.input_dim, kBK);
  stats_ld_ = RoundUp(2 * info_.pool_dim, kBK);
  {
    const bool allow = DebugKnobInt("first_kernel", 1) != 0 && nplanes_ == 2;
    need_prep_ = false;
    for (size_t i = 0; i < layers_.size(); ++i) {
      const BlobLayerInfo& li = info_.layers[i];
      bool reads_input = false, only_input = !li.segment_level && !li.src.empty();
      int off[kMaxSeg] = {0};
      for (size_t j = 0; j < li.src.size(); ++j) {
        if (li.src[j].layer == kSrcInput) reads_input = true;
        if (li.src[j].layer != kSrcInput || li.src[j].dim != info_.input_dim) only_input = false;
        off[j] = li.src[j].offset;
      }
      const bool planes_out = (int)i != info_.pooled_layer && !(frame_mode_ && (int)i == info_.output_layer);
      if (allow && only_input && planes_out && layers_[i].w_lo && FirstLayerApplicable(info_.input_dim, (int)li.src.size(), off)) {
        first_buf_.emplace_back();
        first_buf_.emplace_back();
        Buf& bh = first_buf_[first_buf_.size() - 2];
        Buf& bl = first_buf_[first_buf_.size() - 1];
        Ensure(&bh, (size_t)li.n_pad * kFirstK * 2, false);
        Ensure(&bl, (size_t)li.n_pad * kFirstK * 2, false);
        const int seg_pad = SrcKPad(info_.input_dim, kSrcInput, false, info_.precision);
        Check(launch_compact_first(layers_[i].w_hi, li.k_pad, seg_pad, li.n_pad, (int)li.src.size(), info_.input_dim, (uint16_t*)bh.p, stream_),
              "compact_first launch");
        Check(launch_compact_first(layers_[i].w_lo, li.k_pad, seg_pad, li.n_pad, (int)li.src.size(), info_.input_dim, (uint16_t*)bl.p, stream_),
              "compact_first launch");
        layers_[i].first = true;
        layers_[i].wc_hi = (const uint16_t*)bh.p;
        layers_[i].wc_lo = (const uint16_t*)bl.p;
      } else if (reads_input) {
        need_prep_ = true;
      }
    }
    Check(hipStreamSynchronize(stream_), "hipStreamSynchronize(compact_first)");
  }
}

Engine::~Engine() {
  (void)hipSetDevice(device_);
  if (stream_) (void)hipStreamSynchronize(stream_);
  plan_cache_.clear();
  auto fr = [](Buf& b) {
    if (b.p) (void)hipFree(b.p);
    b.p = nullptr;
  };
  if (stream_) release_stream_workspace(stream_);
  for (Lane& L : lanes_) {
    if (L.stream) (void)hipStreamSynchronize(L.stream);
    if (L.stream) release_stream_workspace(L.stream);
    fr(L.gmax);
    for (ActBuf& a : L.act) {
      fr(a.act_hi);
      fr(a.act_lo);
      fr(a.act_lo4);
      fr(a.act_lo4s);
    }
    fr(L.in_hi);
    fr(L.in_lo);
    fr(L.partial);
    fr(L.stats_hi);
    fr(L.stats_lo);
    fr(L.out_f32);
    fr(L.splitk_ws);
    fr(L.frame_f32);
    if (L.done) (void)hipEventDestroy(L.done);
    if (L.stream) (void)hipStreamDestroy(L.stream);
  }
  for (HostSlot& S : host_slots_) {
    if (S.done) {
      (void)hipEventSynchronize(S.done);
      (void)hipEventDestroy(S.done);
    }
    if (S.h2d_done) (void)hipEventDestroy(S.h2d_done);
    S.plan.reset();
    fr(S.d_feats);
    fr(S.d_out);
    fr(S.d_tables);
    fr(S.d_raw);
    fr(S.d_prefix);
    fr(S.d_fetab);
    fr(S.d_cm);
    if (S.h_fetab) (void)hipHostFree(S.h_fetab);
    if (S.h_feats) (void)hipHostFree(S.h_feats);
    if (S.h_out) (void)hipHostFree(S.h_out);
    if (S.h_tables) (void)hipHostFree(S.h_tables);
  }
  for (Buf& b : first_buf_) fr(b);
  fr(feats_stage_);
  fr(fe_raw_);
  fr(fe_tab_);
  fr(fe_prefix_);
  fr(fe_out_);
  fr(out_stage_);
  if (d_blob_) (void)hipFree(d_blob_);
  if (copy_stream_) (void)hipStreamDestroy(copy_stream_);
  if (stream_) (void)hipStreamDestroy(stream_);
}

void Engine::Ensure(Buf* b, size_t bytes, bool zero, hipStream_t consumer) {
  if (b->bytes >= bytes && b->p) return;
  if (b->p) Check(hipFree(b->p), "hipFree");
  b->p = nullptr;
  Check(hipMalloc(&b->p, bytes), "hipMalloc");
  b->bytes = bytes;
  if (zero) {
    Check(hipMemsetAsync(b->p, 0, bytes, consumer), "hipMemsetAsync");
  }
}

void Engine::EnsureCapacity(Lane& L, int rows, int b_pad, hipStream_t s) {
  bool grew = false;
  if (rows > L.cap_rows) {
    grew = true;
    if (L.busy) Check(hipEventSynchronize(L.done), "hipEventSynchronize(lane)");
    const size_t r = (size_t)rows + 2 * kHalo;
    Ensure(&L.in_hi, r * in_ld_ * 2, true, s);
    if (nplanes_ == 2) Ensure(&L.in_lo, r * in_ld_ * 2, true, s);
    for (size_t i = 0; i < layers_.size(); ++i) {
      const BlobLayerInfo& li = info_.layers[i];
      if (li.segment_level) continue;
      if ((int)i == info_.pooled_layer) {
        Ensure(&L.partial, (size_t)(rows / kRowAlign) * 2 * li.n_pad * 4, true, s);
        continue;
      }
      if (frame_mode_ && (int)i == info_.output_layer) {
        Ensure(&L.frame_f32, (size_t)rows * li.n_pad * (logits16() ? 2 : 4), false);
        continue;
      }
      Ensure(&L.act[i].act_hi, r * li.n_pad * 2, true, s);
      if (nplanes_ == 2) Ensure(&L.act[i].act_lo, r * li.n_pad * 2, true, s);
      if (info_.precision == kPrecFp16Mx2 && !frame_mode_) {
        Ensure(&L.act[i].act_lo4, r * (li.n_pad / 2), true, s);
        Ensure(&L.act[i].act_lo4s, r * Lo4ScalePitch(li.n_pad), true, s);
      }
    }
    if (fast_mx() || can_switch_fast_mode()) Ensure(&L.gmax, layers_.size() * (size_t)(rows / kRowAlign) * 4, true, s);
    L.gmax_stride = rows / kRowAlign;
    L.cap_rows = rows;
  }
  if (!frame_mode_ && b_pad > L.cap_b) {
    if (L.busy) Check(hipEventSynchronize(L.done), "hipEventSynchronize(lane)");
    Ensure(&L.stats_hi, (size_t)b_pad * stats_ld_ * 2, true, s);
    if (nplanes_ == 2) Ensure(&L.stats_lo, (size_t)b_pad * stats_ld_ * 2, true, s);
    for (size_t i = 0; i < layers_.size(); ++i) {
      const BlobLayerInfo& li = info_.layers[i];
      if (!li.segment_level) continue;
      if ((int)i == info_.output_layer) {
        Ensure(&L.out_f32, (size_t)b_pad * li.n_pad * 4, true, s);
      } else {
        Ensure(&L.act[i].act_hi, (size_t)b_pad * li.n_pad * 2, true, s);
        if (nplanes_ == 2) Ensure(&L.act[i].act_lo, (size_t)b_pad * li.n_pad * 2, true, s);
// ... 199 lines not shown
    const bool frame_src = !li.segment_level && src.layer >= 0 && !info_.layers[src.layer].segment_level;
    sg.gmax = (mx_pass && frame_src) ? gmax_of(src.layer) : nullptr;
    if (fast_mx2() && frame_src) {
      const int pn = info_.layers[src.layer].n_pad;
      sg.lo4 = (const uint8_t*)L.act[src.layer].act_lo4.p + (size_t)kHalo * (pn / 2);
      sg.lo4s = (const uint8_t*)L.act[src.layer].act_lo4s.p + (size_t)kHalo * Lo4ScalePitch(pn);
    }
    ksteps += sg.ksteps;
  }
  ga.total_ksteps = ksteps;
  ga.w_hi = dl.w_hi;
  ga.w_lo = dl.w_lo;
  ga.ldw = li.k_pad;
  ga.w4 = dl.w4;
  ga.w4_scale = dl.w4_scale;
  ga.ldw4 = dl.ldw4;
  ga.w4b = dl.w4b;
  ga.w4b_scale = dl.w4b_scale;
  ga.ldw4b = dl.ldw4b;
  ga.n_tiles = li.n_pad / kBN;
  ga.relu = li.relu;
  ga.bn = li.bn;
  ga.bias = dl.bias;
  ga.scale = dl.scale;
  ga.offset = dl.offset;
  int epi;
  if (!li.segment_level) {
    ga.m_tiles = plan.rows / kBM;
    if ((int)i == info_.pooled_layer) {
      epi = kEpiStats;
      ga.partial = (float*)L.partial.p;
      ga.ldp = li.n_pad;
      ga.grp_range = plan.d_grp_range;
    } else if (frame_mode_ && (int)i == info_.output_layer && logits16()) {
      epi = kEpiAct;
      ga.out_hi = (uint16_t*)L.frame_f32.p;
      ga.out_lo = nullptr;
      ga.ldo = li.n_pad;
    } else if (frame_mode_ && (int)i == info_.output_layer) {
      epi = kEpiF32;
      ga.out_f32 = (float*)L.frame_f32.p;
      ga.ldf = li.n_pad;
      ga.m_valid = plan.rows;
    } else {
      epi = kEpiAct;
      ga.out_hi = ActBase(L.act[i].act_hi, li.n_pad);
      ga.out_lo = ActBase(L.act[i].act_lo, li.n_pad);
      ga.ldo = li.n_pad;
      if (fast_mx2()) {
        ga.out_lo4 = (uint8_t*)L.act[i].act_lo4.p + (size_t)kHalo * (li.n_pad / 2);
        ga.out_lo4s = (uint8_t*)L.act[i].act_lo4s.p + (size_t)kHalo * Lo4ScalePitch(li.n_pad);
      }
      if (mx_pass) {
        ga.gmax_out = gmax_of((int)i);
        ga.out_range = plan.d_act_range + (size_t)i * plan.ngrp * 2;
      }
    }
  } else {
    ga.m_tiles = plan.b_pad / kBM;
    const int per = SplitKStepsPerSlice(ksteps);
    ga.ksteps_per_slice = per;
    ga.ksplit = (ksteps + per - 1) / per;
    if (ga.ksplit > 1) {
      Ensure(&L.splitk_ws, (size_t)ga.ksplit * plan.b_pad * li.n_pad * 4, false);
      ga.splitk_ws = (float*)L.splitk_ws.p;
    }
    if ((int)i == info_.output_layer) {
      epi = kEpiF32;
      ga.out_f32 = direct_out ? out_dev : (float*)L.out_f32.p;
      ga.ldf = direct_out ? out_ld : li.n_pad;
      ga.m_valid = plan.B;
    } else {
      epi = kEpiAct;
      ga.out_hi = (uint16_t*)L.act[i].act_hi.p;
      ga.out_lo = (uint16_t*)L.act[i].act_lo.p;
      ga.ldo = li.n_pad;
    }
  }
  if (ga.w4_scale && epi == kEpiStats) ga.w4_scale += (size_t)li.n_pad * (li.k_pad / kBK);
  if (ga.w4b_scale && epi == kEpiStats) ga.w4b_scale += (size_t)li.n_pad * (li.k_pad / kBK);
  return epi;
}

FirstArgs Engine::FirstLayerArgs(const Plan& plan, size_t i, const GemmArgs& ga, const float* feats_dev, int r0, int r1) const {
  const BlobLayerInfo& li = info_.layers[i];
  FirstArgs fa;
  memset(&fa, 0, sizeof fa);
  fa.g = ga;
  fa.feats = feats_dev;
  fa.feats_valid_idx = (long)plan.src_off[0] * info_.input_dim;
  fa.grp_src = (const int4*)plan.d_grp_src;
  fa.rows = plan.rows;
  fa.dim = info_.input_dim;
  fa.noff = (int)li.src.size();
  for (int j = 0; j < fa.noff; ++j) fa.off[j] = li.src[j].offset;
  fa.wc_hi = layers_[i].wc_hi;
  fa.wc_lo = layers_[i].wc_lo;
  fa.row0 = r0;
  fa.nrows = r1 - r0;
  return fa;
}

static GemmArgs SliceRows(GemmArgs g, long r0, long r1) {
  g.m_tiles = (int)((r1 - r0) / kBM);
  g.m_valid = (int)(r1 - r0);
  for (int j = 0; j < g.nseg; ++j) {
    Seg& sg = g.seg[j];
    sg.hi += r0 * sg.ld;
    if (sg.lo) sg.lo += r0 * sg.ld;
    if (sg.lo4) sg.lo4 += r0 * (sg.ld / 2);
    if (sg.lo4s) sg.lo4s += r0 * Lo4ScalePitch(sg.ld);
  }
  if (g.out_hi) g.out_hi += r0 * g.ldo;
  if (g.out_lo) g.out_lo += r0 * g.ldo;
  if (g.out_lo4) g.out_lo4 += r0 * (g.ldo / 2);
  if (g.out_lo4s) g.out_lo4s += r0 * Lo4ScalePitch(g.ldo);
  if (g.out_f32) g.out_f32 += r0 * g.ldf;
  if (g.partial) g.partial += (r0 / kRowAlign) * 2 * g.ldp;
  if (g.grp_range) g.grp_range += (r0 / kRowAlign) * 2;
  return g;
}

int Engine::LaunchPrec(size_t i, int epi, bool fast, GemmArgs* g) const {
  const BlobLayerInfo& li = info_.layers[i];
  const DevLayer& dl = layers_[i];
  int p = slow_prec();
  if (!fast) {
    g->gmax_out = nullptr;
    g->out_range = nullptr;
    for (int j = 0; j < g->nseg; ++j) g->seg[j].gmax = nullptr;
    if (dl.first || p != kPrecFp16 || li.segment_level) return p;
  } else if (dl.first) {
    return (fast_mx2() && (!lite_mask_ || lite_emits_[i])) ? (int)kPrecFp16x3E : (int)kPrecFp16x2;
  } else if (fast_mx2() && lite_mask_ && lite_[i] && gemm_mx_applicable(*g)) {
    p = (lite_emits_[i] && epi == kEpiAct) ? (int)kPrecFp16MxE : (int)kPrecFp16Mx;
    if (p == kPrecFp16Mx) {
      g->out_lo4 = nullptr;
      g->out_lo4s = nullptr;
    }
  } else if (fast_mx2()) {
    p = gemm_mx2_applicable(*g) ? (int)kPrecFp16Mx2 : (int)kPrecFp16x3E;
    if (p == kPrecFp16x3E && epi != kEpiAct) throw EngineError("fp16mx2: layer " + li.name + " cannot run the mode");
    if (p == kPrecFp16x3E) return p;
  } else {
    p = (fast_mx() && gemm_mx_applicable(*g)) ? (int)kPrecFp16Mx : (int)kPrecFp16x2;
    if (p == kPrecFp16x2) return p;
  }
  const bool mx = p != kPrecFp16, mx2 = p == kPrecFp16Mx2;
  if (!use_p8_ || (epi != kEpiAct && epi != kEpiStats) || (mx && !dl.w4p) || (mx2 && !dl.w4bp)) return p;
  const size_t so = epi == kEpiStats ? (size_t)li.n_pad * (li.k_pad / kBK) : 0;
  GemmArgs g8 = *g;
  g8.p8 = 1;
  g8.p8_whole = p8_whole_;
  if (mx) {
    g8.w4 = dl.w4p;
    g8.w4_scale = dl.w4p_scale + so;
  }
  if (mx2) {
    g8.w4b = dl.w4bp;
    g8.ldw4b = li.k_pad * 2;
    g8.w4b_scale = dl.w4bp_scale + so;
  }
  if (gemm_p8_applicable(g8, p)) *g = g8;
  return p;
}

PrepArgs Engine::PrepInputArgs(const Lane& L, const Plan& plan, const float* feats_dev, bool mx_pass) const {
  PrepArgs pa;
  pa.feats = feats_dev;
  pa.src_off = plan.d_src_off;
  pa.dev_off = plan.d_dev_off;
  pa.grp_utt = plan.d_grp_utt;
  pa.rows = plan.rows;
  pa.dim = info_.input_dim;
  pa.ld = in_ld_;
  pa.out_hi = ActBase(L.in_hi, in_ld_);
  pa.out_lo = ActBase(L.in_lo, in_ld_);
  pa.pad_left = pad_left_;
  pa.pad_right = pad_right_;
  pa.zero_words = mx_pass ? (unsigned*)L.gmax.p : nullptr;
  pa.n_zero_words = mx_pass ? (int)(layers_.size() * (size_t)L.gmax_stride) : 0;
  return pa;
}

PoolArgs Engine::PoolingArgs(const Lane& L, const Plan& plan) const {
  PoolArgs po;
  po.partial = (const float*)L.partial.p;
  po.ldp = info_.layers[info_.pooled_layer].n_pad;
  po.utt_grp0 = plan.d_utt_grp0;
  po.utt_grp1 = plan.d_utt_grp1;
  po.utt_count = plan.d_utt_count;
  po.B = plan.B;
  po.dim = info_.pool_dim;
  po.var_floor = info_.variance_floor;
  po.out_hi = (uint16_t*)L.stats_hi.p;
  po.out_lo = (uint16_t*)L.stats_lo.p;
  po.ld = stats_ld_;
  return po;
}

FrameOutArgs Engine::OutputArgs(const Lane& L, const Plan& plan, float* out_dev, int out_ld) const {
  const BlobLayerInfo& ol = info_.layers[info_.output_layer];
  FrameOutArgs fo;
  fo.src = logits16() ? nullptr : (const float*)(frame_mode_ ? L.frame_f32.p : L.out_f32.p);
  fo.src16 = logits16() ? (const uint16_t*)L.frame_f32.p : nullptr;
  fo.ld = ol.n_pad;
  fo.out_row = frame_mode_ ? plan.d_out_row : nullptr;
  fo.n_out = frame_mode_ ? plan.n_out : plan.B;
  fo.dim = info_.output_dim;
  fo.log_softmax = ol.log_softmax;
  fo.out = out_dev;
  fo.out_ld = out_ld;
  return fo;
}

void Engine::ForwardOnLane(size_t lane, const Plan& plan, const float* feats_dev, float* out_dev, int out_ld,
                           hipStream_t stream) {
  Check(hipSetDevice(device_), "hipSetDevice");
  Lane& L = lanes_[lane % lanes_.size()];
  hipStream_t s = stream ? stream : L.stream;
  if (stream && stream != stream_ && std::find(ext_streams_.begin(), ext_streams_.end(), stream) == ext_streams_.end()) {
    bool own = false;
    for (const Lane& l : lanes_) own = own || l.stream == stream;
    if (!own) ext_streams_.push_back(stream);
  }
  if (L.busy) Check(hipStreamWaitEvent(s, L.done, 0), "hipStreamWaitEvent(lane)");
  EnsureCapacity(L, plan.rows, plan.b_pad, s);
  const bool mx_pass = fast_mx() && plan.rows_fast > 0;
  std::vector<hipEvent_t> prof_run;
  const bool first_prof = prof_on_ && prof_labels_.empty();
  auto arm = [&](const std::string& label) {
    if (!prof_on_) return;
    hipEvent_t e0, e1;
    Check(hipEventCreate(&e0), "hipEventCreate");
    Check(hipEventCreate(&e1), "hipEventCreate");
    prof_run.push_back(e0);
    prof_run.push_back(e1);
    if (first_prof) prof_labels_.push_back(label);
    set_launch_events(e0, e1);
  };
  auto disarm = [&]() {
    if (prof_on_) set_launch_events(nullptr, nullptr);
  };
  const PrepArgs pa = PrepInputArgs(L, plan, feats_dev, mx_pass);
  if (need_prep_) {
    arm("prep_input");
    Check(launch_prep_input(pa, slow_prec(), s), "prep_input launch");
    disarm();
  } else if (pa.n_zero_words > 0) {
    Check(hipMemsetAsync(pa.zero_words, 0, (size_t)pa.n_zero_words * 4, s), "hipMemsetAsync(group maxima)");
  }

  const BlobLayerInfo& ol = info_.layers[info_.output_layer];
  const bool direct_out = ol.segment_level && !ol.log_softmax && ol.n_pad == info_.output_dim && (out_ld & 3) == 0 &&
                          out_ld >= ol.n_pad && ((uintptr_t)out_dev & 15) == 0;
  for (size_t i = 0; i < layers_.size(); ++i) {
    const BlobLayerInfo& li = info_.layers[i];
    GemmArgs ga;
    const int epi = LayerArgs(L, plan, i, mx_pass, out_dev, out_ld, direct_out, &ga);
    arm(std::string("tdnn_gemm<") + (epi == kEpiAct ? "act" : epi == kEpiF32 ? "f32" : "stats") + ">:" + li.name);
    if (!layers_[i].first && (li.segment_level || plan.rows_fast == 0)) {
      const int p = LaunchPrec(i, epi, false, &ga);
      Check(launch_tdnn_gemm(ga, p, epi, s), "tdnn_gemm launch");
      if (first_prof) prof_labels_.back() += std::string(" ") + last_gemm_kernel();
    } else {
      for (int region = 0; region < 2; ++region) {
        const int r0 = region == 0 ? 0 : plan.rows_fast, r1 = region == 0 ? plan.rows_fast : plan.rows;
        if (r1 <= r0) continue;
        if (layers_[i].first) {
          FirstArgs fa = FirstLayerArgs(plan, i, ga, feats_dev, r0, r1);
          const int p = LaunchPrec(i, epi, region == 0, &fa.g);
          Check(launch_tdnn_first(fa, p, s), "tdnn_first launch");
        } else {
          GemmArgs gr = SliceRows(ga, r0, r1);
          const int p = LaunchPrec(i, epi, region == 0, &gr);
          Check(launch_tdnn_gemm(gr, p, epi, s), "tdnn_gemm launch");
        }
        if (first_prof) prof_labels_.back() += std::string(" ") + last_gemm_kernel();
      }
    }
    disarm();

    if ((int)i == info_.pooled_layer) {
      arm("pool_finalise");
      Check(launch_pool_finalise(PoolingArgs(L, plan), slow_prec(), s), "pool_finalise launch");
      disarm();
    }
  }
  if (frame_mode_ || ol.log_softmax) {
    arm("frame_output");
    Check(launch_frame_output(OutputArgs(L, plan, out_dev, out_ld), s), "frame_output launch");
    disarm();
  } else if (!direct_out) {
    Check(hipMemcpy2DAsync(out_dev, (size_t)out_ld * 4, L.out_f32.p, (size_t)ol.n_pad * 4, (size_t)info_.output_dim * 4,
                           (size_t)plan.B, hipMemcpyDeviceToDevice, s),
          "hipMemcpy2DAsync(out)");
  }
  Check(hipEventRecord(L.done, s), "hipEventRecord(lane)");
  L.busy = true;
  if (prof_on_) prof_runs_.push_back(std::move(prof_run));
}

void Engine::SetFastMode(int mode) {
  if (!can_switch_fast_mode()) throw EngineError("this context cannot switch its arithmetic (it was not packed as fp16mx2 with a pooled output)");
  if (mode != kPrecFp16Mx2 && mode != kPrecFp16Mx && mode != kPrecFp16x3) throw EngineError("SetFastMode: fp16mx2, fp16mx or fp16x3");
  if (mode == fast_mode_ && lite_mask_ == 0) return;
// ... 492 lines not shown
```

### speaker-embedding-with-phonetic-information_amd/csrc/engine.h

```cpp
#pragma once
#include <hip/hip_runtime_api.h>
#include <stdint.h>

#include <map>
#include <memory>
#include <stdexcept>
#include <string>
#include <vector>

#include "kernels.h"
#include "program.h"

namespace xv {

struct EngineError : public std::runtime_error {
  explicit EngineError(const std::string& m) : std::runtime_error(m) {}
};

std::vector<uint8_t> PackModel(const TdnnProgram& prog, int precision);
constexpr int kPrecDefault = -1;
std::vector<uint8_t> PackModelPolicy(const TdnnProgram& prog, int precision, int* resolved = nullptr);
const char* PrecisionName(int precision);

void PackMxRow(const float* res, int k_pad, const int* step_wcol, uint8_t* row, uint8_t* scales);
// ... 28 lines not shown
  Engine(const Engine&) = delete;
  Engine& operator=(const Engine&) = delete;

  const BlobInfo& info() const { return info_; }
  int device() const { return device_; }

  std::shared_ptr<Plan> MakePlan(const int32_t* row_offsets, int B);
  void Forward(const Plan& plan, const float* feats_dev, float* out_dev, int out_ld, hipStream_t stream);
  void ForwardHost(const float* feats, const int32_t* row_offsets, int B, float* out);
  static constexpr int kNumHostSlots = 3;
  float* HostFeats(int slot, size_t rows);
  struct FrontEndJob {
    const int32_t* raw_off;
    int n_utts;
    const int32_t* sel_row;
    const int32_t* sel_utt;
    int n_out;
    int cmn_window;
    bool center;
    int min_window;
    const int64_t* cm_off = nullptr;
    size_t cm_bytes = 0;
    int max_rows = 0;
  };
  void SubmitHost(int slot, long seq, const int32_t* row_offsets, int B, const FrontEndJob* fe = nullptr);
  const float* WaitHost(int slot);
  bool frame_mode() const { return frame_mode_; }
  void FrontEndHost(const float* raw, const int32_t* raw_off, int n_utts, const int32_t* sel_row, const int32_t* sel_utt,
                    int n_out, int cmn_window, bool center, int min_window, float* out);

  struct Calibration {
    int chosen = 0;
    int checked = 0;
    float err_mx = 0.f;
    float err_mx2 = 0.f;
    int checked_mx = 0;
    uint64_t lite_mask = 0;
    float err_lite = 0.f;
    int checked_holdout = 0;
    float err_holdout = 0.f;
    int lite_dropped = 0;
    float tail = 0.f;
    float tail_mx = 0.f;
  };
  static constexpr int kCalibMinChunks = 16;
  static constexpr double kTailSigmas = 6.0;
  static constexpr float kTailOverTol = 1.10f;
  static constexpr float kTailOverTolPacked = 1.20f;
  static constexpr int kMaxLanes = 4;
  static constexpr int kMaxLiteLayers = 64;
  bool can_switch_fast_mode() const { return info_.precision == kPrecFp16Mx2 && !frame_mode_; }
  int fast_mode() const { return can_switch_fast_mode() ? fast_mode_ : info_.precision; }
  void SetFastMode(int mode);
  void SetLiteMask(uint64_t mask);
  uint64_t lite_mask() const { return lite_mask_; }
  Calibration Calibrate(const float* feats, const int32_t* row_offsets, int B, float tol);

  hipStream_t stream() const { return stream_; }
  int num_lanes() const { return (int)lanes_.size(); }
  size_t weight_bytes() const { return blob_data_bytes_; }
  void SetProfiling(bool on) { prof_on_ = on; }
  std::string ProfileReport();

 private:
  struct Buf {
    void* p = nullptr;
    size_t bytes = 0;
  };
  struct DevLayer {
    const uint16_t* w_hi;
    const uint16_t* w_lo;
    const float* bias;
    const float* scale;
    const float* offset;
    const uint8_t* w4;
    const uint8_t* w4_scale;
    int ldw4;
    const uint8_t* w4b;
    const uint8_t* w4b_scale;
    int ldw4b;
    const uint8_t* w4p = nullptr;
    const uint8_t* w4p_scale = nullptr;
    const uint8_t* w4bp = nullptr;
    const uint8_t* w4bp_scale = nullptr;
    bool first = false;
    const uint16_t* wc_hi = nullptr;
    const uint16_t* wc_lo = nullptr;
  };
  struct ActBuf {
    Buf act_hi, act_lo;
    Buf act_lo4, act_lo4s;
  };
  struct Lane {
    hipStream_t stream = nullptr;
    hipEvent_t done = nullptr;
    bool busy = false;
    std::vector<ActBuf> act;
    Buf in_hi, in_lo, partial, stats_hi, stats_lo, out_f32, splitk_ws, frame_f32;
    Buf gmax;
    int gmax_stride = 0;
    int cap_rows = 0, cap_b = 0;
  };
  struct HostSlot {
    void* h_feats = nullptr;
    size_t h_feats_bytes = 0;
    void* h_out = nullptr;
    size_t h_out_bytes = 0;
    void* h_tables = nullptr;
    size_t h_tables_bytes = 0;
    Buf d_feats, d_out, d_tables;
    Buf d_raw, d_prefix, d_fetab;
    Buf d_cm;
    void* h_fetab = nullptr;
    size_t h_fetab_bytes = 0;
    hipEvent_t done = nullptr;
    hipEvent_t h2d_done = nullptr;
    bool pending = false;
    int lane = 0;
    std::unique_ptr<Plan> plan;
  };
  HostSlot host_slots_[kNumHostSlots];
  void EnsurePinned(void** p, size_t* have, size_t bytes);
  void FillPlan(const int32_t* row_offsets, int B, Plan* plan, std::vector<uint8_t>* tables) const;
  static void BindPlan(Plan* plan, const void* device_tables);
  void ForwardOnLane(size_t lane, const Plan& plan, const float* feats_dev, float* out_dev, int out_ld, hipStream_t stream);
  int LayerArgs(Lane& L, const Plan& plan, size_t i, bool mx_pass, float* out_dev, int out_ld, bool direct_out, GemmArgs* args);
  FirstArgs FirstLayerArgs(const Plan& plan, size_t i, const GemmArgs& ga, const float* feats_dev, int r0, int r1) const;
  int LaunchPrec(size_t i, int epi, bool fast, GemmArgs* g) const;
  PrepArgs PrepInputArgs(const Lane& L, const Plan& plan, const float* feats_dev, bool mx_pass) const;
  PoolArgs PoolingArgs(const Lane& L, const Plan& plan) const;
  FrameOutArgs OutputArgs(const Lane& L, const Plan& plan, float* out_dev, int out_ld) const;
  void Check(hipError_t e, const char* what) const;
 public:
  void CheckKernelFaults(int lane = -1) const;
  mutable unsigned fault_mask_ = 0;
  std::vector<hipStream_t> ext_streams_;
 private:
  void Ensure(Buf* b, size_t bytes, bool zero, hipStream_t consumer = nullptr);
  void EnsureCapacity(Lane& L, int rows, int b_pad, hipStream_t s);
  uint16_t* ActBase(const Buf& b, int ld) const;

  BlobInfo info_;
  int device_ = 0;
  bool frame_mode_ = false;
  int pad_left_ = 0, pad_right_ = 0;
  int nplanes_ = 1;
  static constexpr int kDefaultFastMinPooled = 300;
  static bool fast_family(int p) { return p == kPrecFp16x2 || p == kPrecAuto || p == kPrecFp16Mx || p == kPrecFp16Mx2; }
  int slow_prec() const { return fast_family(info_.precision) ? (int)kPrecFp16x3 : info_.precision; }
  bool has_fast() const { return !frame_mode_ && fast_family(fast_mode_); }
  bool fast_mx() const { return has_fast() && fast_mode_ != kPrecFp16x2; }
  bool fast_mx2() const { return has_fast() && fast_mode_ == kPrecFp16Mx2; }
  int p8_whole_ = 0;
  bool use_p8_ = true;
  bool logits16() const { return frame_mode_ && info_.precision == kPrecFp16 && info_.layers[info_.output_layer].log_softmax; }
  int fast_min_pooled_ = 0;
  int fast_mode_ = 0;
  uint64_t lite_mask_ = 0;
  std::vector<char> lite_, lite_emits_;
  int mx2_min_pooled_ = 0, mx_min_pooled_ = 0;
  hipStream_t stream_ = nullptr;
  hipStream_t copy_stream_ = nullptr;
  void* d_blob_ = nullptr;
  size_t blob_data_bytes_ = 0;
  std::vector<DevLayer> layers_;
  std::vector<Buf> first_buf_;
  bool need_prep_ = true;
  int in_ld_ = 0;
  int stats_ld_ = 0;
  std::vector<Lane> lanes_;
  size_t next_lane_ = 0;
  Buf feats_stage_, out_stage_;
  Buf fe_raw_, fe_tab_, fe_prefix_, fe_out_;
  std::map<std::vector<int32_t>, std::shared_ptr<Plan>> plan_cache_;
  bool prof_on_ = false;
  std::vector<std::string> prof_labels_;
  std::vector<std::vector<hipEvent_t>> prof_runs_;
};

struct Engine::Plan {
  int B = 0, b_pad = 0, rows = 0, src_rows = 0;
  int rows_fast = 0;
  std::vector<int32_t> src_off;
  void* d_tables = nullptr;
  bool borrowed_tables = false;
  size_t o_src = 0, o_dev = 0, o_gu = 0, o_gr = 0, o_g0 = 0, o_g1 = 0, o_cn = 0, o_or = 0, o_ar = 0, o_gs = 0;
  int ngrp = 0;
  const int8_t* d_act_range = nullptr;
  const int32_t* d_src_off = nullptr;
  const int32_t* d_dev_off = nullptr;
  const int32_t* d_grp_utt = nullptr;
  const void* d_grp_src = nullptr;
  const int8_t* d_grp_range = nullptr;
  const int32_t* d_utt_grp0 = nullptr;
  const int32_t* d_utt_grp1 = nullptr;
  const int32_t* d_utt_count = nullptr;
  const int32_t* d_out_row = nullptr;
  std::vector<int32_t> out_off;
  int n_out = 0;
  ~Plan();
};

struct FrontEndBuffers {
  void* raw;
  void* prefix;
  void* out;
  void* tab;
};
struct FrontEndBytes {
  size_t raw, prefix, out, tab;
};
FrontEndBytes FrontEndSizes(long raw_rows, int n_utts, int n_out, int dim);
void FrontEndRun(hipStream_t s, const FrontEndBuffers& b, int dim, const float* raw, const int32_t* raw_off, int n_utts,
                 const int32_t* sel_row, const int32_t* sel_utt, int n_out, int cmn_window, bool center, int min_window, float* out);

}
```

### speaker-embedding-with-phonetic-information_amd/csrc/kernels.h

```cpp
#pragma once
#include <hip/hip_runtime.h>
#include <stdint.h>

namespace xv {

constexpr int kBM = 128;
constexpr int kBN = 128;
constexpr int kBK = 32;
constexpr int kMaxSeg = 8;
constexpr int kRowAlign = 16;

enum Precision : int {
  kPrecBf16x3 = 0,
  kPrecBf16 = 1,
  kPrecFp16 = 2,
  kPrecFp16x3 = 3,
  kPrecFp16x2 = 4,
  kPrecAuto = 5,
  kPrecFp16Mx = 6,
  kPrecFp16Mx2 = 7,
  kPrecFp16x3E = 8,
  kPrecFp16MxE = 9,
};
constexpr bool PrecF16(int p) { return p == kPrecFp16 || p == kPrecFp16x3 || p == kPrecFp16x2 || p == kPrecAuto || p == kPrecFp16Mx || p == kPrecFp16Mx2 || p == kPrecFp16x3E || p == kPrecFp16MxE; }
constexpr bool PrecMx(int p) { return p == kPrecFp16Mx || p == kPrecFp16Mx2 || p == kPrecFp16MxE; }
constexpr bool PrecMx2(int p) { return p == kPrecFp16Mx2; }
constexpr bool PrecEmitsLo4(int p) { return p == kPrecFp16Mx2 || p == kPrecFp16x3E || p == kPrecFp16MxE; }
constexpr int PrecXPlanes(int p) { return (p == kPrecBf16x3 || p == kPrecFp16x3 || p == kPrecFp16x3E) ? 2 : 1; }
constexpr int PrecWPlanes(int p) { return (p == kPrecBf16x3 || p == kPrecFp16x3 || p == kPrecFp16x2 || p == kPrecAuto || p == kPrecFp16Mx || p == kPrecFp16Mx2 || p == kPrecFp16x3E || p == kPrecFp16MxE) ? 2 : 1; }
constexpr int PrecPasses(int p) { return PrecXPlanes(p) + PrecWPlanes(p) - 1; }

enum Epilogue : int {
  kEpiAct = 0,
  kEpiF32 = 1,
  kEpiStats = 2,
  kEpiSplitK = 3,
};

struct Seg {
  const uint16_t* hi;
  const uint16_t* lo;
  int ld;
  int row_shift;
  int ksteps;
  int pad_;
  const unsigned* gmax;
  const uint8_t* lo4;
  const uint8_t* lo4s;
};
constexpr int Lo4ScalePitch(int ld) { return ((ld >> 6) + 3) & ~3; }

struct Grp {
  const uint16_t* hi;
  const uint16_t* lo;
  int ld;
  int ksteps;
  int nshift;
  int shift0;
  int dstep;
  int wcol0;
  int wstride;
  int pad_;
  const unsigned* gmax;
  const uint8_t* lo4s;
  int ld4s;
  int pad2_;
};

struct WalkGroup {
  int first_seg, nshift, ksteps, shift0, dstep, wcol0, wstride;
};
inline int PlanWalkGroups(int nseg, const long* src_key, const int* row_shift, const int* ksteps, WalkGroup* out) {
  int ng = 0, wcol = 0;
  for (int j = 0; j < nseg;) {
    WalkGroup& G = out[ng++];
    G.first_seg = j;
    G.ksteps = ksteps[j];
    G.nshift = 1;
    G.shift0 = row_shift[j];
    G.dstep = 0;
    G.wcol0 = wcol;
    G.wstride = ksteps[j] * kBK;
    int k = j + 1;
    while (k < nseg && src_key[k] == src_key[j] && ksteps[k] == ksteps[j]) {
      const int d = row_shift[k] - row_shift[k - 1];
      if (d <= 0 || (G.nshift > 1 && d != G.dstep) || row_shift[k] - row_shift[j] > 16) break;
      G.dstep = d;
      ++G.nshift;
      ++k;
    }
    wcol += G.nshift * G.wstride;
    j = k;
  }
  return ng;
}
inline int PlanWalkSteps(int ng, const WalkGroup* g, int* step_wcol, int cap, bool* mx_ok) {
  int n = 0;
  bool ok = true;
  for (int i = 0; i < ng; ++i) {
    if ((g[i].ksteps * g[i].nshift) % 4) ok = false;
    for (int kk = 0; kk < g[i].ksteps; ++kk)
      for (int ij = 0; ij < g[i].nshift; ++ij) {
        if (n < cap) step_wcol[n] = g[i].wcol0 + ij * g[i].wstride + kk * kBK;
        ++n;
      }
  }
  if (mx_ok) *mx_ok = ok;
  return n;
}

inline int PlanWalkSteps64(int ng, const WalkGroup* g, int* step_wcol, int cap, bool* ok64) {
  int n = 0;
  bool ok = true;
  for (int i = 0; i < ng; ++i) {
    if (g[i].ksteps % 4) ok = false;
    for (int c = 0; c < g[i].ksteps / 2; ++c)
      for (int ij = 0; ij < g[i].nshift; ++ij)
        for (int k = 0; k < 2; ++k) {
          if (n < cap) step_wcol[n] = g[i].wcol0 + ij * g[i].wstride + (2 * c + k) * kBK;
          ++n;
        }
  }
  if (ok64) *ok64 = ok;
  return n;
}

inline int PlanWalkLoSteps64(int ng, const WalkGroup* g, int* lo_wcol, int cap) {
  int n = 0;
  for (int i = 0; i < ng; ++i)
    for (int c = 0; c < g[i].ksteps / 8; ++c)
      for (int ij = 0; ij < g[i].nshift; ++ij)
        for (int k = 0; k < 2; ++k) {
          if (n < cap) lo_wcol[n] = g[i].wcol0 + ij * g[i].wstride + (2 * c + k) * 4 * kBK;
          ++n;
        }
  return n;
}

inline int PlanWalkLoSteps(int ng, const WalkGroup* g, int* lo_wcol, int cap) {
  int n = 0;
  for (int i = 0; i < ng; ++i)
    for (int kq = 0; kq < g[i].ksteps / 4; ++kq)
      for (int ij = 0; ij < g[i].nshift; ++ij) {
        if (n < cap) lo_wcol[n] = g[i].wcol0 + ij * g[i].wstride + kq * 4 * kBK;
        ++n;
      }
  return n;
}

struct GemmArgs {
  Seg seg[kMaxSeg];
  int nseg;
  Grp grp[2 * kMaxSeg];
  int ngrp;
  int total_ksteps;
  int ngrp_lo;
  int lo_ksteps;
  const uint16_t* w_hi;
  const uint16_t* w_lo;
  int ldw;
  const uint8_t* w4;
  int ldw4;
  const uint8_t* w4_scale;
  const uint8_t* w4b;
  int ldw4b;
  const uint8_t* w4b_scale;
  int m_tiles;
  int n_tiles;
  int relu;
  int bn;
  const float* bias;
  const float* scale;
  const float* offset;
  uint16_t* out_hi;
  uint16_t* out_lo;
  int ldo;
  uint8_t* out_lo4;
  uint8_t* out_lo4s;
  unsigned* gmax_out;
  const int8_t* out_range;
  float* out_f32;
  int ldf;
  int m_valid;
  float* partial;
  int ldp;
  const int8_t* grp_range;
  int ksplit;
  int ksteps_per_slice;
  float* splitk_ws;
  int stagger_wgs, stagger_units;
  int sk_mtiles;
  int sk_lanes;
  float* sk_ws;
  unsigned* sk_flags;
  unsigned sk_epoch;
  unsigned* sk_error;
  int p8;
  int p8_ktiles;
  int p8_whole;
  int p8_ktiles_lo;
};

inline int SplitKStepsPerSlice(int ksteps) {
  const int per = (ksteps + 23) / 24;
  return per < 4 ? 4 : per;
}

void set_launch_events(hipEvent_t start, hipEvent_t stop);

hipError_t launch_tdnn_gemm(const GemmArgs& a, int precision, int epilogue, hipStream_t s);
const char* last_gemm_kernel();
bool gemm_mx_applicable(const GemmArgs& a);
bool gemm_mx2_applicable(const GemmArgs& a);
constexpr bool kP8Mx2Built = true;
bool gemm_p8_applicable(const GemmArgs& a, int precision);
void release_stream_workspace(hipStream_t s);
unsigned sk_take_error(hipStream_t s);

constexpr int kFirstK = 128;
constexpr int kFirstRows = 64;
constexpr int kFirstMaxSlots = 4;
inline bool FirstLayerApplicable(int dim, int noff, const int* off) {
  if (noff < 1 || noff > 8 || dim < 1) return false;
  const int dp = (dim + 7) / 8 * 8;
  int lo = off[0], hi = off[0];
  for (int j = 1; j < noff; ++j) {
    lo = off[j] < lo ? off[j] : lo;
    hi = off[j] > hi ? off[j] : hi;
  }
  return dp <= 24 && noff * dp <= kFirstK && hi - lo <= 30 && (kFirstRows + hi - lo) * dp <= 512 * kFirstMaxSlots;
}
struct FirstArgs {
  GemmArgs g;
  const float* feats;
  long feats_valid_idx;
  const int4* grp_src;
  int rows;
  int dim;
  int row0, nrows;
  int noff;
  int off[8];
  const uint16_t* wc_hi;
  const uint16_t* wc_lo;
  int max_wgs;
};
inline void FillFirstGroupSources(int ngrp, const int32_t* grp_utt, const int32_t* dev_off, const int32_t* row_offsets, int pad_left,
                                  int pad_right, int32_t* grp_src) {
  for (int g = 0; g < ngrp; ++g) {
    int32_t* e = grp_src + 4 * (size_t)g;
    e[0] = e[1] = e[2] = e[3] = 0;
    const int b = grp_utt[g];
    if (b < 0) continue;
    const int t0 = g * kRowAlign - dev_off[b];
    const int s0 = row_offsets[b], len = row_offsets[b + 1] - row_offsets[b];
    e[0] = s0 + t0 - pad_left;
    e[1] = len + pad_left + pad_right - t0;
    e[2] = s0;
    e[3] = s0 + len - 1;
  }
}
hipError_t launch_tdnn_first(const FirstArgs& a, int epi_prec, hipStream_t s);
hipError_t launch_compact_first(const uint16_t* src, int ldw, int seg_pad, int n_pad, int noff, int dim, uint16_t* dst, hipStream_t s);

struct PrepArgs {
  const float* feats;
  const int32_t* src_off;
  const int32_t* dev_off;
  const int32_t* grp_utt;
  int rows;
  int dim;
  int ld;
  uint16_t* out_hi;
  uint16_t* out_lo;
  int pad_left, pad_right;
  unsigned* zero_words;
  int n_zero_words;
};
hipError_t launch_prep_input(const PrepArgs& a, int precision, hipStream_t s);

struct PoolArgs {
  const float* partial;
  int ldp;
  const int32_t* utt_grp0;
  const int32_t* utt_grp1;
  const int32_t* utt_count;
  int B;
  int dim;
  float var_floor;
  uint16_t* out_hi;
  uint16_t* out_lo;
  int ld;
};
hipError_t launch_pool_finalise(const PoolArgs& a, int precision, hipStream_t s);

struct FrameOutArgs {
  const float* src;
  const uint16_t* src16;
  int ld;
  const int32_t* out_row;
  int n_out;
  int dim;
  int log_softmax;
  float* out;
  int out_ld;
};
hipError_t launch_frame_output(const FrameOutArgs& a, hipStream_t s);

struct FrontEndArgs {
  const float* raw;
  const int32_t* raw_off;
  double* prefix;
  int n_utts;
  int dim;
  const int32_t* sel_row;
  const int32_t* sel_utt;
  int n_out;
  int cmn_window;
  int center;
  int min_window;
  float* out;
};
hipError_t launch_frontend(const FrontEndArgs& a, hipStream_t s);

struct CmExpandArgs {
  const uint8_t* cm;
  const int64_t* cm_off;
  const int32_t* raw_off;
  int n_utts, dim, max_rows;
  float* out;
};
hipError_t launch_cm_expand(const CmExpandArgs& a, hipStream_t s);

struct BackendArgs {
  const float* x;
  int n, dim, ldx;
  const float* mean;
  const float* t;
  int t_rows, t_cols;
  int normalize, scaleup;
  float* out;
  int ldo;
  float* ratio;
};
hipError_t launch_backend(const BackendArgs& a, hipStream_t s);

struct SegMeanArgs {
  const float* x;
  int dim, ldx;
  const int32_t* seg_off;
  const int32_t* idx;
  int n_seg;
  int acc64;
// ... 11 lines not shown
```

### speaker-embedding-with-phonetic-information_amd/csrc/kernels.hip

```cpp
#include "kernels.h"
#include "knobs.h"

#include <hip/hip_ext.h>

#include <stdlib.h>
#include <string.h>

#include <algorithm>
#include <atomic>
#include <map>
#include <mutex>
#include <type_traits>
#include <utility>

namespace xv {

typedef __attribute__((ext_vector_type(8))) __bf16 bf16x8;
typedef __attribute__((ext_vector_type(8))) _Float16 f16x8;
typedef __attribute__((ext_vector_type(8))) short s16x8;
typedef __attribute__((ext_vector_type(4))) float f32x4;
typedef __attribute__((ext_vector_type(2))) float f32x2;
typedef __attribute__((ext_vector_type(4))) unsigned int u32x4;

#define XV_AS1 __attribute__((address_space(1)))
// ... 1758 lines not shown
    if (kind == 2) {
      const int prev = bid - 8 * L;
      if (tid == 0) {
        const unsigned long long t0 = __builtin_readcyclecounter();
        while (__hip_atomic_load(a.sk_flags + prev, __ATOMIC_RELAXED, __HIP_MEMORY_SCOPE_AGENT) != a.sk_epoch) {
          __builtin_amdgcn_s_sleep(8);
          if (__builtin_readcyclecounter() - t0 > 4000000000ull) {
            __hip_atomic_store(a.sk_error, a.sk_epoch, __ATOMIC_RELAXED, __HIP_MEMORY_SCOPE_AGENT);
            break;
          }
        }
      }
      __syncthreads();
      const __amdgpu_buffer_rsrc_t rs = __builtin_amdgcn_make_buffer_rsrc(
          (void*)(a.sk_ws + (long)prev * kPartialFloats), 0, (int)(kPartialFloats * 4), 0x00020000);
#pragma unroll
      for (int h = 0; h < NH; ++h)
#pragma unroll
        for (int p = 0; p < 4; ++p)
#pragma unroll
          for (int q = 0; q < 4; ++q)
            acc[h][p][q] = __builtin_bit_cast(
                f32x4, __builtin_amdgcn_raw_buffer_load_b128(rs, tid * 16, ((h * 4 + p) * 4 + q) * 8192, kAuxCoherent));
    } else {
#pragma unroll
      for (int h = 0; h < NH; ++h)
#pragma unroll
        for (int p = 0; p < 4; ++p)
#pragma unroll
          for (int q = 0; q < 4; ++q) acc[h][p][q] = f32x4{0.f, 0.f, 0.f, 0.f};
    }

    __builtin_amdgcn_s_waitcnt(0x0F70);
    wait_and_barrier(0);
    if (group == 1) plain_barrier();
    Frags f;
    const int ns = n_steps;
    const int ns_hi = MX2 ? n_hi : ns;
    if constexpr (MX) {
#pragma nounroll
      for (int j = 0; j < ns_hi; j += 4, ++rblk) {
#pragma unroll
        for (int s = 0; s < 4; ++s) {
          XV_FUZZ();
          __builtin_amdgcn_s_setprio(1);
          read_step(f);
          if (s == 3) read_scales(rblk % 3);
          XV_FUZZ();
          const int n = (j + s + 2 < ns) ? issue_step() : 0;
          wait_and_barrier(n);
          XV_FUZZ();
          __builtin_amdgcn_s_setprio(0);
          mfmas(f);
          convert(f, s);
          if (s == 3) mx_mfmas(f);
          plain_barrier();
        }
      }
      if constexpr (MX2) {
        rstep += ns_hi;
#pragma nounroll
        for (int j = ns_hi; j < ns; ++j, ++rstep) {
          __builtin_amdgcn_s_setprio(1);
          const int lg = rg, lkk = rkk, lj = rj;
          if ((lj == 0 && (lkk & 1) == 0) || (j == ns_hi && ns_hi == 0)) ++rslab;
          read_step(f);
          read_scales((rstep - SH + (SH >> 2)) % 3);
          XV_FUZZ();
          const int n = (j + 2 < ns) ? issue_step() : 0;
          wait_and_barrier(n);
          XV_FUZZ();
          __builtin_amdgcn_s_setprio(0);
          lo_mfmas(f, lg, lkk, lj, (rslab - 1) % 3);
          plain_barrier();
        }
      }
      asm volatile("s_nop 15\n\ts_nop 15" ::: "memory");
    } else {
#pragma nounroll
      for (int j = 0; j < ns; ++j) {
        XV_FUZZ();
        read_step(f);
        XV_FUZZ();
        const int n = (j + 2 < ns) ? issue_step() : 0;
        wait_and_barrier(n);
        XV_FUZZ();
        __builtin_amdgcn_s_setprio(1);
        mfmas(f);
        __builtin_amdgcn_s_setprio(0);
        plain_barrier();
      }
    }
    if (group == 0) plain_barrier();
    XV_FUZZ();
    const int e_kind = kind, e_m0 = m0, e_n0 = n0;
    const float* e_par = (const float*)(smem + PB + (part & 1) * 1536);
    constexpr bool SPLIT_EPI = WIDE && EPI == kEpiAct && PrecEmitsLo4(PREC);
    float gm_carry[4] = {0.f, 0.f, 0.f, 0.f};
    if constexpr (SPLIT_EPI) {
      if (kind != 1) {
        EpiRegs er;
        epilogue_prefetch_lds<EPI, true>(a, e_par, e_m0 + row_w, 0, lane, er);
        gemm_epilogue<PREC, EPI, true>(a, acc[0], e_m0 + row_w, e_n0, lane, er, gm_carry, 1, e_par, 0);
      }
    }
    if (part + 1 < n_parts) open_part(part + 1);

#ifdef XVEC_CLOCK_PROBE
    const unsigned long long xp_e0 = __builtin_readcyclecounter();
#endif
    if (e_kind == 1) {
      const __amdgpu_buffer_rsrc_t rs = __builtin_amdgcn_make_buffer_rsrc(
          (void*)(a.sk_ws + (long)bid * kPartialFloats), 0, (int)(kPartialFloats * 4), 0x00020000);
#pragma unroll
      for (int h = 0; h < NH; ++h)
#pragma unroll
        for (int p = 0; p < 4; ++p)
#pragma unroll
          for (int q = 0; q < 4; ++q)
            __builtin_amdgcn_raw_buffer_store_b128(__builtin_bit_cast(u32x4, acc[h][p][q]), rs, tid * 16,
                                                   ((h * 4 + p) * 4 + q) * 8192, kAuxCoherent);
      XV_FUZZ();
      __builtin_amdgcn_s_waitcnt(0x0f70);
      asm volatile("s_waitcnt vmcnt(0)" ::: "memory");
      __syncthreads();
      if (tid == 0) __hip_atomic_store(a.sk_flags + bid, a.sk_epoch, __ATOMIC_RELAXED, __HIP_MEMORY_SCOPE_AGENT);
    } else {
      if constexpr (WIDE) {
        float (&gm)[4] = gm_carry;
#pragma unroll
        for (int h = SPLIT_EPI ? 1 : 0; h < NH; ++h) {
          constexpr bool LAZY = (EPI == kEpiAct || EPI == kEpiF32) && MX;
          EpiRegs er;
          epilogue_prefetch_lds<EPI, LAZY>(a, e_par, e_m0 + row_w, h * 64, lane, er);
          gemm_epilogue<PREC, EPI, LAZY>(a, acc[h], e_m0 + row_w, e_n0 + h * 64, lane, er, gm, h == 0 ? 1 : 2, e_par, h * 64);
        }
      } else {
        EpiRegs er;
        epilogue_prefetch_lds<EPI>(a, e_par, e_m0 + row_w, col_w, lane, er);
        float gm[4] = {0.f, 0.f, 0.f, 0.f};
        gemm_epilogue<PREC, EPI>(a, acc[0], e_m0 + row_w, e_n0 + col_w, lane, er, gm, 0);
      }
    }
  }
}

constexpr int kP8Buf = 65536, kP8XW = 32768, kP8Unit = 16384;
constexpr int kP8W4 = 2 * kP8Buf;
constexpr int kP8SC = kP8W4 + 16384;
constexpr int kP8PB = kP8SC + 1024;
constexpr int kP8WSL = kP8PB + 2 * 3072;
constexpr int kP8XSL = kP8WSL + 2 * 2048;
constexpr int kP8Lds = kP8XSL + 2 * 1024;

__device__ __forceinline__ void wait_vmcnt_n(int n) {
  switch (n) {
    case 0: asm volatile("s_waitcnt vmcnt(0)" ::: "memory"); break;
    case 1: asm volatile("s_waitcnt vmcnt(1)" ::: "memory"); break;
    case 2: asm volatile("s_waitcnt vmcnt(2)" ::: "memory"); break;
    case 3: asm volatile("s_waitcnt vmcnt(3)" ::: "memory"); break;
    case 4: asm volatile("s_waitcnt vmcnt(4)" ::: "memory"); break;
    case 5: asm volatile("s_waitcnt vmcnt(5)" ::: "memory"); break;
    case 6: asm volatile("s_waitcnt vmcnt(6)" ::: "memory"); break;
    case 7: asm volatile("s_waitcnt vmcnt(7)" ::: "memory"); break;
    case 8: asm volatile("s_waitcnt vmcnt(8)" ::: "memory"); break;
    case 9: asm volatile("s_waitcnt vmcnt(9)" ::: "memory"); break;
    case 10: asm volatile("s_waitcnt vmcnt(10)" ::: "memory"); break;
    case 11: asm volatile("s_waitcnt vmcnt(11)" ::: "memory"); break;
    case 12: asm volatile("s_waitcnt vmcnt(12)" ::: "memory"); break;
    case 13: asm volatile("s_waitcnt vmcnt(13)" ::: "memory"); break;
    case 14: asm volatile("s_waitcnt vmcnt(14)" ::: "memory"); break;
    case 15: asm volatile("s_waitcnt vmcnt(15)" ::: "memory"); break;
    default: asm volatile("s_waitcnt vmcnt(16)" ::: "memory"); break;
  }
}

#ifdef XVEC_CLOCK_PROBE
__device__ unsigned long long g_clock_probe[3 * 512 * 2];
__device__ unsigned long long g_exchange_probe[3 * 512 * 4];
__device__ unsigned long long g_part_probe[3 * 512 * 2];
extern "C" int xvec_part_probe_read(unsigned long long* out) {
  return (int)hipMemcpyFromSymbol(out, HIP_SYMBOL(g_part_probe), sizeof(g_part_probe), 0, hipMemcpyDeviceToHost);
}
extern "C" int xvec_clock_probe_read(unsigned long long* out) {
  return (int)hipMemcpyFromSymbol(out, HIP_SYMBOL(g_clock_probe), sizeof(g_clock_probe), 0, hipMemcpyDeviceToHost);
}
extern "C" int xvec_exchange_probe_read(unsigned long long* out) {
  return (int)hipMemcpyFromSymbol(out, HIP_SYMBOL(g_exchange_probe), sizeof(g_exchange_probe), 0, hipMemcpyDeviceToHost);
}
#endif

template <int PREC, int EPI>
__global__ __launch_bounds__(512) void tdnn_gemm_kernel_p8(const GemmArgs a) {
  static_assert(PREC == kPrecFp16 || PREC == kPrecFp16Mx || PREC == kPrecFp16Mx2 || PREC == kPrecFp16MxE,
                "single-pass fp16, the 1.25-pass arithmetic (with or without the residual plane of its output), the 1.5-pass arithmetic");
  constexpr bool MX = PrecMx(PREC);
  constexpr bool MX2 = PrecMx2(PREC);
  constexpr bool SWAP = (EPI != kEpiStats);
  extern __shared__ __attribute__((aligned(16))) char smem[];
  const int tid = threadIdx.x;
  const int lane = tid & 63;
  const int wave = __builtin_amdgcn_readfirstlane(tid >> 6);
  const int wm = wave & 3, wn = wave >> 2;
  const int fr_i = lane & 15, fr_g = lane >> 4;
  const int bid = blockIdx.x;
  const unsigned lds_base = (unsigned)(size_t)(XV_AS3 char*)smem;
  XV_FUZZ_INIT();

  const int S = a.p8_ktiles;
  const int S_lo = MX2 ? a.p8_ktiles_lo : 0;
  const int ST = S + S_lo;
  const int NG = a.ngrp + (MX2 ? a.ngrp_lo : 0);
  const int G8 = gridDim.x >> 3;
  const int xcd = bid & 7, jb = bid >> 3;
  const int L = a.sk_lanes, NT = a.n_tiles >> 1, cpl = NT / L, Ng = G8 / L;
  const int col_lane = jb % L, grp_j = jb / L;
  const int tb0 = (int)((long)a.sk_mtiles * xcd / 8), tb1 = (int)((long)a.sk_mtiles * (xcd + 1) / 8);
  long s0, s1;
  {
    const long all = (long)(tb1 - tb0) * cpl * ST;
    auto cut = [&](long g) __attribute__((always_inline)) {
      const long s = all * g / Ng;
      if (a.p8_whole) return (s + ST / 2) / ST * ST;
      int k = (int)(s % ST);
      if (k < S) k &= ~1;
      return s - s % ST + k;
    };
    s0 = cut(grp_j);
    s1 = cut(grp_j + 1);
  }
  const int k_head = (int)(s0 % ST), k_tail = (int)(s1 % ST);
  const int t_first = (int)((s0 + ST - 1) / ST), t_end = (int)(s1 / ST);
  const int n_parts = (k_tail ? 1 : 0) + (t_end - t_first) + (k_head ? 1 : 0);
  if (s1 <= s0) return;
#ifdef XVEC_CLOCK_PROBE
  const unsigned long long clk_t0 = __builtin_readcyclecounter(), clk_r0 = __builtin_amdgcn_s_memrealtime();
#endif

  constexpr bool RECOMPUTE = MX2;
  auto lane_now = [&]() __attribute__((always_inline)) {
    int l = lane;
    if constexpr (RECOMPUTE) asm volatile("" : "+v"(l));
    return l;
  };
  auto unit_offsets = [&](const int ld_elems, const bool weights, unsigned (&off)[2]) __attribute__((always_inline)) {
    const int l = lane_now();
#pragma unroll
    for (int j = 0; j < 2; ++j) {
      const int ru = wave * 16 + j * 8 + (l >> 3);
      const int c = (l & 7) ^ ((j * 4 + (l >> 4)) & 7);
      int row = ru;
      if (weights) {
        const int rho = ru & 63;
        row = (ru >> 6) * 128 + (SWAP ? swap_fields(rho) : rho);
      }
      off[j] = (unsigned)(row * ld_elems + c * 8) * 2u;
    }
  };
  auto w4_offsets = [&](unsigned (&off)[2]) __attribute__((always_inline)) {
    const int l = lane_now();
#pragma unroll
    for (int u = 0; u < 2; ++u) {
      const int r4 = wave * 32 + u * 16 + (l >> 2);
      const int rho = r4 & 63;
      const int wrow = ((r4 >> 6) & 1) * 128 + (r4 >> 7) * 64 + (SWAP ? swap_fields(rho) : rho);
      off[u] = (unsigned)(wrow * a.ldw4 + ((l & 3) ^ ((l >> 3) & 3)) * 16);
    }
  };
  unsigned woff_r[2] = {0u, 0u}, woff4_r[2] = {0u, 0u}, xoff_r[2] = {0u, 0u};
  if constexpr (!RECOMPUTE) {
    unit_offsets(a.ldw, true, woff_r);
    if constexpr (MX) w4_offsets(woff4_r);
  }
  const unsigned st_lane = lds_base + wave * 2048;

  int m0 = 0, n0 = 0, nt = 0;
  int kind = 0, n_tiles_part = 0, kb_part = 0;
  int it = 0, ig = 0, ic = 0, ij = 0;
  Grp gi = a.grp[0];
  const char* xb = nullptr;
  const char* wb = nullptr;
  const char* wtile = nullptr;
  int x_next = 0, x_wrap = 0, w_next = 0, w_wrap = 0;
  auto bind_group = [&]() __attribute__((always_inline)) {
    if constexpr (!RECOMPUTE) unit_offsets(gi.ld, false, xoff_r);
    xb = (const char*)gi.hi + ((long)(m0 + gi.shift0 + ij * gi.dstep) * gi.ld + ic * 64) * 2;
    x_next = gi.dstep * gi.ld * 2;
    x_wrap = 128 - (gi.nshift - 1) * gi.dstep * gi.ld * 2;
    const bool lo_i = MX2 && it >= S;
    const char* wb_hi = wtile + (long)(gi.wcol0 + ij * gi.wstride + ic * 64) * 2;
    const char* wb_lo = MX2 ? (const char*)a.w4b + (long)n0 * a.ldw * 2 + (long)(it - S) * 128 : wb_hi;
    wb = lo_i ? wb_lo : wb_hi;
    w_next = lo_i ? 128 : gi.wstride * 2;
    w_wrap = lo_i ? 128 : 128 - (gi.nshift - 1) * gi.wstride * 2;
  };
  auto adv = [&]() __attribute__((always_inline)) {
    ++it;
    if (++ij == gi.nshift) {
      ij = 0;
      xb += x_wrap;
      wb += w_wrap;
      if (++ic == (gi.ksteps >> 1)) {
        ic = 0;
        if (++ig < NG) {
          gi = a.grp[ig];
          bind_group();
        }
      }
    } else {
      xb += x_next;
      wb += w_next;
    }
  };
  auto issue = [&](const int unit, const int buf) __attribute__((always_inline)) {
    if (unit == 0 || unit == 3) {
      const unsigned dst = st_lane + 2 * kP8XW + buf * kP8XW + (unit == 3 ? kP8Unit : 0);
      const char* src = wb + (unit == 3 ? (long)a.ldw * 128 : 0);
      unsigned woff[2] = {woff_r[0], woff_r[1]};
      if constexpr (RECOMPUTE) unit_offsets(a.ldw, true, woff);
      glds16_sbase_m0(src, woff[0], dst);
      glds16_sbase_m0(src, woff[1], dst + 1024);
    } else {
      const char* src = xb + (unit == 2 ? (long)gi.ld * 256 : 0);
      const unsigned dst = st_lane + buf * kP8XW + (unit == 2 ? kP8Unit : 0);
      unsigned xoff[2] = {xoff_r[0], xoff_r[1]};
      if constexpr (RECOMPUTE) unit_offsets(gi.ld, false, xoff);
      glds16_sbase_m0(src, xoff[0], dst);
      glds16_sbase_m0(src, xoff[1], dst + 1024);
    }
  };
  auto issue_w4 = [&](const int blk) __attribute__((always_inline)) {
    if constexpr (MX) {
      const unsigned d4 = lds_base + kP8W4 + wave * 2048;
      unsigned woff4[2] = {woff4_r[0], woff4_r[1]};
      if constexpr (RECOMPUTE) w4_offsets(woff4);
      const uint8_t* w4t = a.w4 + (long)n0 * a.ldw4 + blk * 64;
      glds16_sbase(w4t, woff4[0], d4);
      glds16_sbase(w4t, woff4[1], d4 + 1024);
      const int pc = wave & 3;
      glds4_sbase(a.w4_scale + ((long)(nt * 2 + (pc >> 1)) * (S >> 1) + blk) * 512 + (pc & 1) * 256, (unsigned)lane * 4u,
                  lds_base + kP8SC + pc * 256);
    }
  };
  auto issue_scales = [&](const int sb) __attribute__((always_inline)) {
    if constexpr (MX2) {
      const int t_lo = it - S;
      const int t128 = (wave >> 1) & 1, ks = wave >> 2, half = wave & 1;
      glds4_sbase(a.w4b_scale + ((long)(nt * 2 + t128) * (2 * S_lo) + 2 * t_lo + ks) * 512 + half * 256, (unsigned)lane * 4u,
                  lds_base + kP8WSL + sb * 2048 + ks * 1024 + t128 * 512 + half * 256);
      const uint8_t* xs = gi.lo4s + (long)(m0 + gi.shift0 + ij * gi.dstep + (wave & 3) * 64) * gi.ld4s + ic * 4;
      glds4_sbase(xs, (unsigned)(lane * gi.ld4s), lds_base + kP8XSL + sb * 1024 + (wave & 3) * 256);
    }
  };

  const int sw = (fr_g ^ ((fr_i >> 1) & 7)) * 16;
  const int xrd0 = (wm * 64 + fr_i) * 128 + sw, xrd1 = xrd0 ^ 64;
  const int wrd0 = 2 * kP8XW + (wn * 64 + fr_i) * 128 + sw, wrd1 = wrd0 ^ 64;
  const int w4rd = kP8W4 + (wn * 64 + fr_i) * 64 + (fr_g ^ ((fr_i >> 1) & 3)) * 16;

  int xs_b = 0;
  float xs_f[MX ? 4 : 1];
  typedef __attribute__((ext_vector_type(4))) unsigned xs_uvec;
  auto xs_request = [&](const unsigned* gmax, xs_uvec& g) __attribute__((always_inline)) {
    if constexpr (MX) {
      const unsigned* p = gmax + ((m0 + wm * 64) >> 4);
      asm volatile("s_load_dwordx4 %0, %1, 0x0" : "=&s"(g) : "s"(p) : "memory");
    }
  };
  auto xs_finish = [&](xs_uvec& g) __attribute__((always_inline)) {
    if constexpr (MX) {
      asm volatile("s_waitcnt lgkmcnt(0)" : "+s"(g) : : "memory");
      xs_b = 0;
#pragma unroll
      for (int f = 0; f < 4; ++f) {
        unsigned e = (g[f] >> 23) & 255u;
        e = e < 16u ? 16u : (e > 200u ? 200u : e);
        xs_b |= (int)((e - 2u) << (8 * f));
        xs_f[f] = __builtin_bit_cast(float, (e - 2u) << 23);
      }
    }
  };
  int rg = 0, r_left = 0;

  f32x4 acc[2][4][4];
  s16x8 xf[4][2], wf[4][2];
  i32x4 x4[MX ? 4 : 1];
  int ws_lo[MX2 ? 2 : 1], xs_lo[MX2 ? 2 : 1];

  auto barrier = [&]() __attribute__((always_inline)) {
    __builtin_amdgcn_sched_barrier(0);
    asm volatile("s_barrier" ::: "memory");
    __builtin_amdgcn_sched_barrier(0);
  };
  constexpr bool prio_load = true, prio_mfma = false;
  auto mfma = [&](auto HH, auto PP, auto QQ, const int k) __attribute__((always_inline)) {
    constexpr int H = decltype(HH)::value, pw = decltype(PP)::value, qx = decltype(QQ)::value;
    if constexpr (SWAP) mfma16_f16_inplace(wf[pw][k], xf[qx][k], acc[H][pw][qx]);
    else mfma16_f16_inplace(xf[qx][k], wf[pw][k], acc[H][qx][pw]);
  };
  int c0 = 0, c1 = 0, c2 = 0, c3 = 0;
  auto phase = [&](auto PP, auto BB, auto OO, auto LL, auto FF, const int unit, const int ibuf, const int w4_blk, const int sc_buf,
                   const bool steady) __attribute__((always_inline)) {
    constexpr int P = decltype(PP)::value, B = decltype(BB)::value, ODD = decltype(OO)::value;
    constexpr bool LO = decltype(LL)::value != 0;
    constexpr bool FAST = decltype(FF)::value != 0;
    const char* xs0 = smem + xrd0 + B * kP8XW;
    const char* xs1 = smem + xrd1 + B * kP8XW;
    const char* ws0 = smem + wrd0 + B * kP8XW;
    const char* ws1 = smem + wrd1 + B * kP8XW;
    XV_FUZZ();
    if (prio_load) __builtin_amdgcn_s_setprio(1);
    if constexpr (P == 0) {
#pragma unroll
      for (int p = 0; p < 4; ++p) {
        wf[p][0] = *(const s16x8*)(ws0 + p * 2048);
        wf[p][1] = *(const s16x8*)(ws1 + p * 2048);
      }
#pragma unroll
      for (int q = 0; q < 2; ++q) {
        xf[q][0] = *(const s16x8*)(xs0 + q * 2048);
        xf[q][1] = *(const s16x8*)(xs1 + q * 2048);
      }
      if constexpr (MX2 && LO) {
        const uint8_t* xsl = (const uint8_t*)smem + kP8XSL + B * 1024 + (wm * 64 + fr_i) * 4 + (fr_g >> 1);
#pragma unroll
        for (int k = 0; k < 2; ++k) {
          int x = 0;
#pragma unroll
          for (int q = 0; q < 4; ++q) x |= (int)xsl[q * 64 + 2 * k] << (8 * q);
          xs_lo[k] = x;
        }
      }
    } else if constexpr (P == 1) {
#pragma unroll
      for (int q = 2; q < 4; ++q) {
        xf[q][0] = *(const s16x8*)(xs0 + q * 2048);
        xf[q][1] = *(const s16x8*)(xs1 + q * 2048);
      }
    } else if constexpr (P == 2) {
#pragma unroll
      for (int p = 0; p < 4; ++p) {
        wf[p][0] = *(const s16x8*)(ws0 + kP8Unit + p * 2048);
        wf[p][1] = *(const s16x8*)(ws1 + kP8Unit + p * 2048);
      }
    }
    if constexpr (MX2 && LO && (P == 0 || P == 2)) {
      const char* wsl = smem + kP8WSL + B * 2048 + wn * 512 + (P >> 1) * 256 + (fr_i * 4 + fr_g) * 4;
      ws_lo[0] = *(const int*)(wsl);
      ws_lo[1] = *(const int*)(wsl + 1024);
    }
    constexpr int E1 = (MX && !LO && !ODD) ? 3 : 0;
    XV_FUZZ();
    if constexpr (FAST) {
      constexpr int UNIT = P == 0 ? 2 : P == 1 ? 3 : P == 2 ? 0 : 1;
      issue(UNIT, P < 2 ? 1 - B : B);
      if constexpr (MX && P == 1 && !ODD) issue_w4(w4_blk);
      __builtin_amdgcn_sched_barrier(0);
      if constexpr (P == 1) asm volatile("s_waitcnt vmcnt(%0)" ::"n"(8 + E1) : "memory");
      if constexpr (P == 3) asm volatile("s_waitcnt vmcnt(%0)" ::"n"(6 + E1) : "memory");
    } else {
      c3 = c2;
      c2 = c1;
      c1 = c0;
      c0 = 0;
      if (unit >= 0) {
        issue(unit, ibuf);
        c0 += 2;
      }
      if (w4_blk >= 0) {
        issue_w4(w4_blk);
        c0 += 3;
      }
      if (sc_buf >= 0) {
        issue_scales(sc_buf);
        c0 += 2;
      }
      __builtin_amdgcn_sched_barrier(0);
      if constexpr (P == 1) {
        if (!MX2 && steady) asm volatile("s_waitcnt vmcnt(%0)" ::"n"(8 + E1) : "memory");
        else wait_vmcnt_n(c0 + c1 + c2 + c3);
      }
      if constexpr (P == 3) {
        if (!MX2 && steady) asm volatile("s_waitcnt vmcnt(%0)" ::"n"(6 + E1) : "memory");
        else wait_vmcnt_n(c0 + c1 + c2);
      }
    }
    asm volatile("s_barrier" ::: "memory");
    XV_FUZZ();
    __builtin_amdgcn_s_waitcnt(0xc07f);
    __builtin_amdgcn_sched_barrier(0);
    constexpr int H = P >> 1;
    constexpr int Q0 = (P == 0 || P == 3) ? 0 : 2;
    if (prio_load) __builtin_amdgcn_s_setprio(0);
    if (prio_mfma) __builtin_amdgcn_s_setprio(1);
    if constexpr (MX2 && LO) {
      asm volatile("s_nop 4" ::: "memory");
      static_for<0, 2>([&](auto K) {
        static_for<0, 4>([&](auto PW) {
          static_for<Q0, Q0 + 2>([&](auto QX) {
            constexpr int k = decltype(K)::value, pw = decltype(PW)::value, qx = decltype(QX)::value;
            if constexpr (SWAP) mfma_mx4_inplace<pw, qx>(wf[pw][k], xf[qx][k], acc[H][pw][qx], ws_lo[k], xs_lo[k]);
            else mfma_mx4_inplace<qx, pw>(xf[qx][k], wf[pw][k], acc[H][qx][pw], xs_lo[k], ws_lo[k]);
          });
        });
      });
    } else if constexpr (MX && P < 2) {
      static_for<0, 16>([&](auto I) {
        constexpr int i = decltype(I)::value;
        constexpr int mk = i >> 3, mp = (i >> 1) & 3, mq = Q0 + (i & 1);
        mfma(std::integral_constant<int, H>{}, std::integral_constant<int, mp>{}, std::integral_constant<int, mq>{}, mk);
        constexpr int cq = Q0 + (i & 1), ck = (i >> 1) & 1, cj = i >> 2;
        const u32x4 u = __builtin_bit_cast(u32x4, xf[cq][ck]);
        const float xsc = xs_f[cq];
        int d;
        if constexpr (cj == 0) {
          asm volatile("v_cvt_scalef32_pk_fp4_f16 %0, %1, %2" : "=v"(d) : "v"(u[0]), "v"(xsc));
        } else {
          d = x4[cq][2 * ODD + ck];
          asm volatile("v_cvt_scalef32_pk_fp4_f16 %0, %1, %2 op_sel:[0,0,%3,%4]"
                       : "+v"(d)
                       : "v"(u[cj]), "v"(xsc), "n"(cj & 1), "n"(cj >> 1));
        }
        x4[cq][2 * ODD + ck] = d;
      });
    } else if constexpr (MX && ODD && P == 3) {
      int ws_v[2];
      const char* sc = smem + kP8SC + wn * 512 + (fr_i * 4 + fr_g) * 4;
      ws_v[0] = *(const int*)(sc);
      ws_v[1] = *(const int*)(sc + 256);
      static_for<0, 4>([&](auto PW) {
        static_for<Q0, Q0 + 2>([&](auto QX) { mfma(std::integral_constant<int, H>{}, PW, QX, 0); });
      });
      __builtin_amdgcn_sched_barrier(0);
#pragma unroll
      for (int w = 0; w < 4; ++w) wf[w][0] = *(const s16x8*)(smem + w4rd + w * 1024);
      __builtin_amdgcn_sched_barrier(0);
      static_for<0, 4>([&](auto PW) {
        static_for<Q0, Q0 + 2>([&](auto QX) { mfma(std::integral_constant<int, H>{}, PW, QX, 1); });
      });
      __builtin_amdgcn_sched_barrier(0);
#pragma unroll
      for (int w = 0; w < 4; ++w) wf[w][1] = *(const s16x8*)(smem + w4rd + 8192 + w * 1024);
      asm volatile("s_waitcnt lgkmcnt(4)\n\ts_nop 4" ::: "memory");
      __builtin_amdgcn_sched_barrier(0);
      static_for<0, 2>([&](auto HH) {
        constexpr int h = decltype(HH)::value;
        if constexpr (h == 1) {
          __builtin_amdgcn_sched_barrier(0);
          __builtin_amdgcn_s_waitcnt(0xc07f);
          __builtin_amdgcn_sched_barrier(0);
        }
        static_for<0, 4>([&](auto PW) {
          static_for<0, 4>([&](auto QX) {
            constexpr int pw = decltype(PW)::value, qx = decltype(QX)::value;
            if constexpr (SWAP) mfma_mx4_inplace<pw, qx>(wf[pw][h], x4[qx], acc[h][pw][qx], ws_v[h], xs_b);
            else mfma_mx4_inplace<qx, pw>(x4[qx], wf[pw][h], acc[h][qx][pw], xs_b, ws_v[h]);
          });
        });
      });
    } else {
      static_for<0, 2>([&](auto K) {
        static_for<0, 4>([&](auto PW) {
          static_for<Q0, Q0 + 2>([&](auto QX) { mfma(std::integral_constant<int, H>{}, PW, QX, decltype(K)::value); });
        });
      });
    }
    if (prio_mfma) __builtin_amdgcn_s_setprio(0);
    barrier();
  };
  typedef std::integral_constant<int, 0> I0;
  typedef std::integral_constant<int, 1> I1;
  typedef std::integral_constant<int, 2> I2;
  typedef std::integral_constant<int, 3> I3;
  auto pair = [&](auto LL, const int n_left, const int blk, const bool first) __attribute__((always_inline)) {
    constexpr int LOW = decltype(LL)::value;
    const bool t1 = n_left > 1, t2 = n_left > 2, t3 = n_left > 3;
#ifdef XVEC_FUZZ_INJECT_HAZARD
    (void)first;
    phase(I0{}, I0{}, I0{}, LL, I0{}, t1 ? 2 : -1, 1, -1, -1, t3);
    phase(I1{}, I0{}, I0{}, LL, I0{}, t1 ? 3 : -1, 1, (MX && !LOW) ? blk : -1, -1, t3);
    if (t2) adv();
    phase(I2{}, I0{}, I0{}, LL, I0{}, t2 ? 0 : -1, 0, -1, (MX2 && t2 && it >= S) ? 0 : -1, t3);
    phase(I3{}, I0{}, I0{}, LL, I0{}, t2 ? 1 : -1, 0, -1, -1, t3);
    if (t1) {
      phase(I0{}, I1{}, I1{}, LL, I0{}, t2 ? 2 : -1, 0, -1, -1, t3);
      phase(I1{}, I1{}, I1{}, LL, I0{}, t2 ? 3 : -1, 0, -1, -1, t3);
      if (t3) adv();
      phase(I2{}, I1{}, I1{}, LL, I0{}, t3 ? 0 : -1, 1, -1, (MX2 && t3 && it >= S) ? 1 : -1, t3);
      phase(I3{}, I1{}, I1{}, LL, I0{}, t3 ? 1 : -1, 1, -1, -1, t3);
    }
#else
    phase(I0{}, I0{}, I0{}, LL, I0{}, t1 ? 2 : -1, 1, -1, (MX2 && t1 && !first && it >= S) ? 1 : -1, t3);
    phase(I1{}, I0{}, I0{}, LL, I0{}, t1 ? 3 : -1, 1, (MX && !LOW) ? blk : -1, -1, t3);
    if (t2) adv();
    phase(I2{}, I0{}, I0{}, LL, I0{}, t2 ? 0 : -1, 0, -1, -1, t3);
    phase(I3{}, I0{}, I0{}, LL, I0{}, t2 ? 1 : -1, 0, -1, -1, t3);
    if (t1) {
      phase(I0{}, I1{}, I1{}, LL, I0{}, t2 ? 2 : -1, 0, -1, (MX2 && t2 && it >= S) ? 0 : -1, t3);
      phase(I1{}, I1{}, I1{}, LL, I0{}, t2 ? 3 : -1, 0, -1, -1, t3);
      if (t3) adv();
      phase(I2{}, I1{}, I1{}, LL, I0{}, t3 ? 0 : -1, 1, -1, -1, t3);
      phase(I3{}, I1{}, I1{}, LL, I0{}, t3 ? 1 : -1, 1, -1, -1, t3);
    }
#endif
  };

  auto pair_fast = [&](const int blk) __attribute__((always_inline)) {
    phase(I0{}, I0{}, I0{}, I0{}, I1{}, 0, 0, blk, -1, true);
    phase(I1{}, I0{}, I0{}, I0{}, I1{}, 0, 0, blk, -1, true);
    adv();
    phase(I2{}, I0{}, I0{}, I0{}, I1{}, 0, 0, blk, -1, true);
    phase(I3{}, I0{}, I0{}, I0{}, I1{}, 0, 0, blk, -1, true);
    phase(I0{}, I1{}, I1{}, I0{}, I1{}, 0, 0, blk, -1, true);
    phase(I1{}, I1{}, I1{}, I0{}, I1{}, 0, 0, blk, -1, true);
    adv();
    phase(I2{}, I1{}, I1{}, I0{}, I1{}, 0, 0, blk, -1, true);
    phase(I3{}, I1{}, I1{}, I0{}, I1{}, 0, 0, blk, -1, true);
    c0 = c1 = c2 = c3 = 2;
  };

  auto seek = [&](int k, int& g, int& c, int& j) __attribute__((always_inline)) {
    g = 0;
    for (;;) {
      const int n = (a.grp[g].ksteps >> 1) * a.grp[g].nshift;
      if (k < n || g + 1 >= NG) break;
      k -= n;
      ++g;
    }
    const int ns = a.grp[g].nshift;
    c = k / ns;
    j = k - c * ns;
  };
  constexpr long kPartialFloats = 256L * 256;
  constexpr int kAuxCoherent = 1 | 16;
  auto open_part = [&](int part) __attribute__((always_inline)) {
    int tile, kb, ke;
    if (k_tail && part == 0) {
      tile = t_end; kb = 0; ke = k_tail; kind = 1;
    } else {
      const int w = part - (k_tail ? 1 : 0);
      if (w < t_end - t_first) {
        tile = t_first + w; kb = 0; ke = ST; kind = 0;
      } else {
        tile = t_first - 1; kb = k_head; ke = ST; kind = 2;
      }
    }
    const int mt = tb0 + tile / cpl;
    nt = col_lane * cpl + tile % cpl;
    m0 = mt * 256;
    n0 = nt * 256;
    wtile = (const char*)a.w_hi + (long)n0 * a.ldw * 2;
    it = kb;
    seek(kb, ig, ic, ij);
    gi = a.grp[ig];
    bind_group();
    rg = ig;
    r_left = (gi.ksteps >> 1) * gi.nshift - (ic * gi.nshift + ij);
    kb_part = kb;
    n_tiles_part = ke - kb;
    if (EPI != kEpiSplitK && kind != 1 && wave < 6) {
#pragma unroll
      for (int hh = 0; hh < 2; ++hh) {
        const unsigned dst = lds_base + kP8PB + (part & 1) * 3072 + hh * 1536 + wave * 256;
        if (wave < 2 || a.bn) {
          const float* src = (wave < 2 ? a.bias : wave < 4 ? a.scale : a.offset) + n0 + hh * 128 + (wave & 1) * 64;
          glds4_sbase(src, (unsigned)lane * 4u, dst);
        } else {
          *(float*)(smem + kP8PB + (part & 1) * 3072 + hh * 1536 + wave * 256 + lane * 4) = wave < 4 ? 1.f : 0.f;
        }
      }
    }
    xs_uvec xg;
    const bool first_walk = kb < S;
    if constexpr (MX) {
      if (first_walk) xs_request(gi.gmax, xg);
    }
    issue(0, 0);
    issue(1, 0);
    issue(2, 0);
    issue(3, 0);
    if (MX2 && it >= S) issue_scales(0);
    if (n_tiles_part > 1) {
      adv();
      issue(0, 1);
      issue(1, 1);
      if (MX2 && it >= S) issue_scales(1);
    }
    if (MX && first_walk) xs_finish(xg);
  };

  open_part(0);
#ifdef XVEC_CLOCK_PROBE
  unsigned long long pp_sum = 0, pp_n = 0;
#endif
#pragma nounroll
  for (int part = 0; part < n_parts; ++part) {
#ifdef XVEC_CLOCK_PROBE
    unsigned long long xp_t0 = __builtin_readcyclecounter(), xp_t1 = xp_t0;
#endif
    XV_FUZZ();
    if (kind == 2) {
      const int prev = bid - 8 * L;
      if (tid == 0) {
        const unsigned long long t0 = __builtin_readcyclecounter();
        while (__hip_atomic_load(a.sk_flags + prev, __ATOMIC_RELAXED, __HIP_MEMORY_SCOPE_AGENT) != a.sk_epoch) {
          __builtin_amdgcn_s_sleep(8);
          if (__builtin_readcyclecounter() - t0 > 4000000000ull) {
            __hip_atomic_store(a.sk_error, a.sk_epoch, __ATOMIC_RELAXED, __HIP_MEMORY_SCOPE_AGENT);
            break;
          }
        }
      }
      __syncthreads();
      const __amdgpu_buffer_rsrc_t rs = __builtin_amdgcn_make_buffer_rsrc(
          (void*)(a.sk_ws + (long)prev * kPartialFloats), 0, (int)(kPartialFloats * 4), 0x00020000);
#pragma unroll
      for (int h = 0; h < 2; ++h)
#pragma unroll
        for (int p = 0; p < 4; ++p)
#pragma unroll
          for (int q = 0; q < 4; ++q)
            acc[h][p][q] = __builtin_bit_cast(
                f32x4, __builtin_amdgcn_raw_buffer_load_b128(rs, tid * 16, ((h * 4 + p) * 4 + q) * 8192, kAuxCoherent));
    } else {
#pragma unroll
      for (int h = 0; h < 2; ++h)
#pragma unroll
        for (int p = 0; p < 4; ++p)
#pragma unroll
          for (int q = 0; q < 4; ++q) acc[h][p][q] = f32x4{0.f, 0.f, 0.f, 0.f};
    }
#ifdef XVEC_CLOCK_PROBE
    xp_t1 = __builtin_readcyclecounter();
#endif
    XV_FUZZ();
    __builtin_amdgcn_s_waitcnt(0x0F70);
    __builtin_amdgcn_sched_barrier(0);
    asm volatile("s_waitcnt vmcnt(0) lgkmcnt(0)\n\ts_barrier" ::: "memory");
    __builtin_amdgcn_sched_barrier(0);
#ifdef XVEC_CLOCK_PROBE
    if (tid == 0 && bid < 512 && kind == 2) {
      const int slot = EPI == kEpiStats ? 2 : (S > 8 ? 1 : 0);
      g_exchange_probe[(slot * 512 + bid) * 4 + 1] = xp_t1 - xp_t0;
      g_exchange_probe[(slot * 512 + bid) * 4 + 2] = __builtin_readcyclecounter() - xp_t1;
    }
    if (kind == 0 && part > 0) {
      pp_sum += __builtin_readcyclecounter() - xp_t1;
      ++pp_n;
    }
#endif
    c0 = c1 = c2 = c3 = 0;
    if (wn == 1) barrier();
    const int ntp = n_tiles_part;
    const int n_hi = MX2 ? (kb_part >= S ? 0 : (kb_part + ntp <= S ? ntp : S - kb_part)) : ntp;
    auto enter_pair = [&]() __attribute__((always_inline)) {
      if constexpr (MX) {
        if (r_left == 0) {
          ++rg;
          r_left = (a.grp[rg].ksteps >> 1) * a.grp[rg].nshift;
          xs_uvec xg;
          xs_request(a.grp[rg].gmax, xg);
          xs_finish(xg);
        }
        r_left -= 2;
      }
    };
    int t = 0;
    if constexpr (!MX2 && PREC != kPrecFp16MxE) {
#pragma nounroll
      for (; ntp - t > 3; t += 2) {
        enter_pair();
        pair_fast((kb_part + t) >> 1);
      }
    }
#pragma nounroll
    for (; t < n_hi; t += 2) {
      enter_pair();
      pair(I0{}, ntp - t, (kb_part + t) >> 1, t == 0);
    }
    if constexpr (MX2) {
#pragma nounroll
      for (t = n_hi; t < ntp; t += 2) pair(I1{}, ntp - t, 0, t == 0);
    }
    if (wn == 0) barrier();
    XV_FUZZ();
    asm volatile("s_nop 15\n\ts_nop 15" ::: "memory");
    const int e_kind = kind, e_m0 = m0, e_n0 = n0;
    const float* e_par = (const float*)(smem + kP8PB + (part & 1) * 3072 + wn * 1536);
    if (part + 1 < n_parts) open_part(part + 1);
#ifdef XVEC_CLOCK_PROBE
    const unsigned long long xp_e0 = __builtin_readcyclecounter();
#endif
    if (e_kind == 1) {
      const __amdgpu_buffer_rsrc_t rs = __builtin_amdgcn_make_buffer_rsrc(
          (void*)(a.sk_ws + (long)bid * kPartialFloats), 0, (int)(kPartialFloats * 4), 0x00020000);
#pragma unroll
      for (int h = 0; h < 2; ++h)
#pragma unroll
        for (int p = 0; p < 4; ++p)
#pragma unroll
          for (int q = 0; q < 4; ++q)
            __builtin_amdgcn_raw_buffer_store_b128(__builtin_bit_cast(u32x4, acc[h][p][q]), rs, tid * 16,
                                                   ((h * 4 + p) * 4 + q) * 8192, kAuxCoherent);
      XV_FUZZ();
      __builtin_amdgcn_s_waitcnt(0x0f70);
      asm volatile("s_waitcnt vmcnt(0)" ::: "memory");
      __syncthreads();
      if (tid == 0) __hip_atomic_store(a.sk_flags + bid, a.sk_epoch, __ATOMIC_RELAXED, __HIP_MEMORY_SCOPE_AGENT);
#ifdef XVEC_CLOCK_PROBE
      if (tid == 0 && bid < 512) g_exchange_probe[((EPI == kEpiStats ? 2 : (S > 8 ? 1 : 0)) * 512 + bid) * 4 + 0] = __builtin_readcyclecounter() - xp_e0;
#endif
    } else {
      float gm[4] = {0.f, 0.f, 0.f, 0.f};
#pragma unroll
      for (int h = 0; h < 2; ++h) {
        constexpr bool LAZY = (EPI == kEpiAct || EPI == kEpiF32);
        EpiRegs er;
        epilogue_prefetch_lds<EPI, LAZY>(a, e_par, e_m0 + wm * 64, h * 64, lane, er);
        gemm_epilogue<PREC, EPI, LAZY>(a, acc[h], e_m0 + wm * 64, e_n0 + wn * 128 + h * 64, lane, er, gm, h == 0 ? 1 : 2, e_par, h * 64);
      }
#ifdef XVEC_CLOCK_PROBE
      if (tid == 0 && bid < 512 && e_kind == 0) g_exchange_probe[((EPI == kEpiStats ? 2 : (S > 8 ? 1 : 0)) * 512 + bid) * 4 + 3] = __builtin_readcyclecounter() - xp_e0;
#endif
    }
  }
#ifdef XVEC_CLOCK_PROBE
  if (tid == 0 && bid < 512) {
    const int slot = EPI == kEpiStats ? 2 : (S > 8 ? 1 : 0);
    g_part_probe[(slot * 512 + bid) * 2] = pp_sum;
    g_part_probe[(slot * 512 + bid) * 2 + 1] = pp_n;
    g_clock_probe[(slot * 512 + bid) * 2] = __builtin_readcyclecounter() - clk_t0;
    g_clock_probe[(slot * 512 + bid) * 2 + 1] = __builtin_amdgcn_s_memrealtime() - clk_r0;
  }
#endif
}

struct SkWorkspace {
  float* ws = nullptr;
  unsigned* flags = nullptr;
  unsigned* error = nullptr;
  size_t ws_bytes = 0;
  int grid = 0;
};
static std::mutex g_sk_mu;
static std::map<std::pair<int, hipStream_t>, SkWorkspace> g_sk_table;
static unsigned g_sk_epoch = 0;

static void sk_free(SkWorkspace* w) {
  if (w->ws) (void)hipFree(w->ws);
  if (w->flags) (void)hipFree(w->flags);
  if (w->error) (void)hipHostFree(w->error);
  *w = SkWorkspace();
}

static hipError_t sk_workspace(hipStream_t s, int grid, size_t ws_bytes, SkWorkspace* out, unsigned* epoch, unsigned** err) {
  std::lock_guard<std::mutex> lock(g_sk_mu);
  int dev = 0;
  hipError_t e = hipGetDevice(&dev);
  if (e != hipSuccess) return e;
  SkWorkspace& w = g_sk_table[std::make_pair(dev, s)];
  if (w.ws_bytes < ws_bytes || w.grid < grid) {
    unsigned* keep_error = w.error;
    w.error = nullptr;
    sk_free(&w);
    w.error = keep_error;
    if (!w.error) {
      if ((e = hipHostMalloc((void**)&w.error, 64, hipHostMallocMapped | hipHostMallocPortable)) != hipSuccess) return e;
      *w.error = 0;
    }
    if ((e = hipExtMallocWithFlags((void**)&w.ws, ws_bytes, hipDeviceMallocFinegrained)) != hipSuccess) {
      sk_free(&w);
      return e;
    }
    if ((e = hipExtMallocWithFlags((void**)&w.flags, (size_t)grid * sizeof(unsigned), hipDeviceMallocFinegrained)) != hipSuccess ||
        (e = hipMemsetAsync(w.flags, 0, (size_t)grid * sizeof(unsigned), s)) != hipSuccess) {
      sk_free(&w);
      return e;
    }
    w.ws_bytes = ws_bytes;
    w.grid = grid;
  }
  if (++g_sk_epoch == 0) ++g_sk_epoch;
  *epoch = g_sk_epoch;
  *err = w.error;
  *out = w;
  return hipSuccess;
}

void release_stream_workspace(hipStream_t s) {
  std::lock_guard<std::mutex> lock(g_sk_mu);
  int dev = 0;
  if (hipGetDevice(&dev) != hipSuccess) return;
  auto it = g_sk_table.find(std::make_pair(dev, s));
  if (it == g_sk_table.end()) return;
  sk_free(&it->second);
  g_sk_table.erase(it);
}

unsigned sk_take_error(hipStream_t s) {
  std::lock_guard<std::mutex> lock(g_sk_mu);
  int dev = 0;
  if (hipGetDevice(&dev) != hipSuccess) return 0u;
  auto it = g_sk_table.find(std::make_pair(dev, s));
  if (it == g_sk_table.end() || !it->second.error) return 0u;
  volatile unsigned* w = it->second.error;
  const unsigned v = *w;
  if (v) *w = 0u;
  return v;
}

template <int PREC, int MF>
static bool sk_applicable(const GemmArgs& a) {
  constexpr int lds = 3 * (PrecXPlanes(PREC) * (64 * MF + 16) * kBK * 2 + PrecWPlanes(PREC) * kTileBytes) + 1536 + 2 * 1536 + (PrecMx2(PREC) ? 3 * (64 * MF + 16) * 4 : 0);
  if (lds > 160 * 1024) return false;
  const int rows = a.m_tiles * kBM;
  if (rows % (64 * MF)) return false;
  const int grid = device_cu_count() / 8 * 8;
  if (grid < 8) return false;
  if ((long)(rows / (64 * MF) / 8) * a.n_tiles >= grid / 8) return true;
  return MF == 8 && rows / (64 * MF) / 8 >= 4 && (long)(a.m_tiles / 2) * a.n_tiles > device_cu_count();
}

template <int MF>
static int sk_groups(const GemmArgs& a, int grid, int lanes) {
  const int tiles_min = std::max(1, (a.m_tiles * kBM / (64 * MF) / 8) * (a.n_tiles / lanes));
  return std::min(grid / 8 / lanes, tiles_min);
}

template <int PREC, int EPI, int MF>
static hipError_t launch_one_sk(const GemmArgs& a, hipStream_t s) {
  constexpr int lds = 3 * (PrecXPlanes(PREC) * (64 * MF + 16) * kBK * 2 + PrecWPlanes(PREC) * kTileBytes) + 1536 + 2 * 1536 + (PrecMx2(PREC) ? 3 * (64 * MF + 16) * 4 : 0);
  if constexpr (lds > 160 * 1024) {
    return hipErrorInvalidValue;
  } else {
    static std::atomic<unsigned long long> attr_done{0};
    int attr_dev = 0;
    if (lds_attr_needed(&attr_done, &attr_dev)) {
      hipError_t e = hipFuncSetAttribute((const void*)tdnn_gemm_kernel_sk<PREC, EPI, MF>,
                                         hipFuncAttributeMaxDynamicSharedMemorySize, lds);
      if (e != hipSuccess) return e;
      attr_done.fetch_or(1ull << (attr_dev & 63), std::memory_order_release);
    }
    int grid = device_cu_count() / 8 * 8;
    GemmArgs b = a;
    build_groups(&b);
    if constexpr (PrecMx2(PREC)) build_lo_groups(&b);
    b.sk_mtiles = a.m_tiles * kBM / (64 * MF);
    {
      static const int max_lanes = [] {
        const int x = DebugKnobInt("sk_lanes", 4);
        return (x != 1 && x != 2 && x != 4) ? 4 : x;
      }();
      int l = max_lanes;
      while (l > 1 && (a.n_tiles % l || (grid / 8) % l)) l >>= 1;
      b.sk_lanes = l;
      grid = 8 * l * sk_groups<MF>(a, grid, l);
    }
    SkWorkspace w;
    hipError_t e = sk_workspace(s, grid, (size_t)grid * 64 * MF * kBN * sizeof(float), &w, &b.sk_epoch, &b.sk_error);
    if (e != hipSuccess) return e;
    b.sk_ws = w.ws;
    b.sk_flags = w.flags;
    note_kernel("_sk", PREC, EPI, MF);
    XV_LAUNCH((tdnn_gemm_kernel_sk<PREC, EPI, MF>), dim3(grid), dim3(512), lds, s, b);
    return hipGetLastError();
  }
}


bool gemm_p8_applicable(const GemmArgs& a, int precision) {
  if (precision == kPrecFp16MxE) precision = kPrecFp16Mx;
  if (precision != kPrecFp16 && precision != kPrecFp16Mx && precision != kPrecFp16Mx2) return false;
  if ((a.m_tiles & 1) || (a.n_tiles & 1) || a.ksplit > 1) return false;
  const bool mx = precision != kPrecFp16, mx2 = precision == kPrecFp16Mx2;
  GemmArgs b = a;
  build_groups(&b);
  int t = 0;
  for (int i = 0; i < b.ngrp; ++i) {
    if (b.grp[i].ksteps % (mx2 ? 8 : mx ? 4 : 2) || b.grp[i].ld % (mx2 ? 256 : 64)) return false;
    if (mx && !b.grp[i].gmax) return false;
    t += (b.grp[i].ksteps >> 1) * b.grp[i].nshift;
  }
  if (t < 2 || (t & 1)) return false;
  if (mx && (!a.w4 || !a.w4_scale || a.ldw4 <= 0)) return false;
  if (mx2) {
    if (!a.w4b || !a.w4b_scale || a.ldw4b <= 0) return false;
    for (int j = 0; j < a.nseg; ++j)
      if (!a.seg[j].lo4 || !a.seg[j].lo4s) return false;
  }
  return true;
}

template <int PREC, int EPI>
static hipError_t launch_one_p8(const GemmArgs& a, hipStream_t s) {
  if (!gemm_p8_applicable(a, PREC)) return hipErrorInvalidValue;
  static std::atomic<unsigned long long> attr_done{0};
  int attr_dev = 0;
  if (lds_attr_needed(&attr_done, &attr_dev)) {
    hipError_t e = hipFuncSetAttribute((const void*)tdnn_gemm_kernel_p8<PREC, EPI>, hipFuncAttributeMaxDynamicSharedMemorySize, kP8Lds);
    if (e != hipSuccess) return e;
    attr_done.fetch_or(1ull << (attr_dev & 63), std::memory_order_release);
  }
  GemmArgs b = a;
  build_groups(&b);
  b.p8_ktiles = 0;
  for (int i = 0; i < b.ngrp; ++i) b.p8_ktiles += (b.grp[i].ksteps >> 1) * b.grp[i].nshift;
  b.p8_ktiles_lo = 0;
  if constexpr (PrecMx2(PREC)) {
    build_lo_groups(&b);
    for (int i = 0; i < b.ngrp_lo; ++i) b.p8_ktiles_lo += (b.grp[b.ngrp + i].ksteps >> 1) * b.grp[b.ngrp + i].nshift;
  }
  b.p8 = 1;
  b.p8_whole = (a.p8_whole == 1 || (a.p8_whole == 2 && b.p8_ktiles + b.p8_ktiles_lo <= 8)) ? 1 : 0;
  b.sk_mtiles = a.m_tiles >> 1;
  const int nt = a.n_tiles >> 1;
  int grid = device_cu_count() / 8 * 8;
  if (grid < 8) return hipErrorInvalidValue;
  int l = 4;
  while (l > 1 && (nt % l || (grid / 8) % l)) l >>= 1;
  if (nt % 3 == 0 && nt <= 6 && grid / 8 >= nt) l = nt;
  b.sk_lanes = l;
  const int tiles_min = std::max(1, (b.sk_mtiles / 8) * (nt / l));
  grid = 8 * l * std::min(grid / 8 / l, tiles_min);
  SkWorkspace w;
  hipError_t e = sk_workspace(s, grid, (size_t)grid * 256 * 256 * sizeof(float), &w, &b.sk_epoch, &b.sk_error);
  if (e != hipSuccess) return e;
  b.sk_ws = w.ws;
  b.sk_flags = w.flags;
  note_kernel("_p8", PREC, EPI, 0);
  XV_LAUNCH((tdnn_gemm_kernel_p8<PREC, EPI>), dim3(grid), dim3(512), kP8Lds, s, b);
  return hipGetLastError();
}

template <int PREC, int EPI>
static hipError_t launch_one_v2(const GemmArgs& a, hipStream_t s) {
  constexpr int lds = 3 * (PrecXPlanes(PREC) * (256 + 16) * kBK * 2 + PrecWPlanes(PREC) * kTileBytes) + (PrecMx(PREC) ? 1536 : 0) + (PrecMx2(PREC) ? 3 * (256 + 16) * 4 : 0);
  static std::atomic<unsigned long long> attr_done{0};
  int attr_dev = 0;
  if (lds_attr_needed(&attr_done, &attr_dev)) {
    hipError_t e = hipFuncSetAttribute((const void*)tdnn_gemm_kernel_v2<PREC, EPI>,
                                       hipFuncAttributeMaxDynamicSharedMemorySize, lds);
    if (e != hipSuccess) return e;
    attr_done.fetch_or(1ull << (attr_dev & 63), std::memory_order_release);
  }
  const int mt = a.m_tiles >> 1;
  const int mt8 = (mt + 7) / 8 * 8;
  dim3 grid(mt8 * a.n_tiles), block(512);
  GemmArgs b = a;
  build_groups(&b);
  if constexpr (PrecMx2(PREC)) build_lo_groups(&b);
  {
    static const int pct = DebugKnobInt("gemm_stagger", 85);
    const int cus = device_cu_count();
    b.stagger_wgs = cus;
    b.stagger_units = ((int)grid.x > 2 * cus) ? (int)(((long)b.total_ksteps * (400 + 600 * PrecPasses(PREC)) + 14000) * pct / 100 / 2048) : 0;
  }
  note_kernel("_v2", PREC, EPI, 0);
  XV_LAUNCH((tdnn_gemm_kernel_v2<PREC, EPI>), grid, block, lds, s, b);
  return hipGetLastError();
}

template <int PREC, int EPI>
static hipError_t launch_one(const GemmArgs& a, hipStream_t s) {
  if (a.p8) {
    if constexpr (((PREC == kPrecFp16 || PREC == kPrecFp16Mx || PREC == kPrecFp16Mx2) && (EPI == kEpiAct || EPI == kEpiStats)) ||
                  (PREC == kPrecFp16MxE && EPI == kEpiAct))
      return launch_one_p8<PREC, EPI>(a, s);
    else return hipErrorInvalidValue;
  }
  const int variant = gemm_variant();
  const bool sk_default = PREC == kPrecFp16x2 || PREC == kPrecFp16Mx || a.total_ksteps >= 32;
  if constexpr (PrecMx(PREC)) {
    if (PrecMx2(PREC) ? !gemm_mx2_applicable(a) : !gemm_mx_applicable(a)) return hipErrorInvalidValue;
    if (variant != 2 && variant != 1 && sk_max_mf() == 8 && sk_applicable<PREC, 8>(a)) return launch_one_sk<PREC, EPI, 8>(a, s);
    return launch_one_v2<PREC, EPI>(a, s);
  } else {
    if (variant == 4 || (variant == 0 && sk_default)) {
      if (sk_max_mf() == 8 && sk_applicable<PREC, 8>(a)) return launch_one_sk<PREC, EPI, 8>(a, s);
      if ((variant == 4 || PrecXPlanes(PREC) == 2) && sk_applicable<PREC, 4>(a)) return launch_one_sk<PREC, EPI, 4>(a, s);
    }
    if (variant != 1 && (a.m_tiles & 1) == 0) return launch_one_v2<PREC, EPI>(a, s);
    constexpr int lds = kTileBytes * (PrecXPlanes(PREC) + PrecWPlanes(PREC)) * 2;
    static std::atomic<unsigned long long> attr_done{0};
    int attr_dev = 0;
    if (lds_attr_needed(&attr_done, &attr_dev)) {
      hipError_t e = hipFuncSetAttribute((const void*)tdnn_gemm_kernel<PREC, EPI>,
                                         hipFuncAttributeMaxDynamicSharedMemorySize, lds);
      if (e != hipSuccess) return e;
      attr_done.fetch_or(1ull << (attr_dev & 63), std::memory_order_release);
    }
    const int mt8 = (a.m_tiles + 7) / 8 * 8;
    dim3 grid(mt8 * a.n_tiles), block(256);
    note_kernel("", PREC, EPI, 0);
    XV_LAUNCH((tdnn_gemm_kernel<PREC, EPI>), grid, block, lds, s, a);
    return hipGetLastError();
  }
}

template <int PREC, int EPI>
__global__ __launch_bounds__(256) void splitk_reduce_kernel(const GemmArgs a) {
  constexpr bool SPLIT = PrecXPlanes(PREC) == 2;
  constexpr bool F16 = PrecF16(PREC);
  const int n_pad = a.n_tiles * kBN;
  const int rows = a.m_tiles * kBM;
  const long idx = (long)blockIdx.x * blockDim.x + threadIdx.x;
  const int per_row = n_pad >> 2;
  if (idx >= (long)rows * per_row) return;
  const int row = (int)(idx / per_row);
  const int col = (int)(idx - (long)row * per_row) * 4;
  f32x4 v = {0.f, 0.f, 0.f, 0.f};
  const long slab = (long)rows * n_pad;
  const float* src = a.splitk_ws + (long)row * n_pad + col;
  int k = 0;
  for (; k + 8 <= a.ksplit; k += 8) {
    f32x4 t[8];
#pragma unroll
    for (int j = 0; j < 8; ++j) t[j] = *(const f32x4*)(src + (k + j) * slab);
#pragma unroll
    for (int j = 0; j < 8; ++j) v += t[j];
  }
  {
    f32x4 t[8];
#pragma unroll
    for (int j = 0; j < 8; ++j) t[j] = (k + j < a.ksplit) ? *(const f32x4*)(src + (k + j) * slab) : f32x4{0.f, 0.f, 0.f, 0.f};
#pragma unroll
    for (int j = 0; j < 8; ++j)
      if (k + j < a.ksplit) v += t[j];
  }
  const f32x4 b = *(const f32x4*)(a.bias + col);
  float y[4];
#pragma unroll
  for (int r = 0; r < 4; ++r) {
    float z = v[r] + b[r];
    if (a.relu) z = (z < 0.f) ? 0.f : z;
    if (a.bn) z = __builtin_fmaf(z, a.scale[col + r], a.offset[col + r]);
    y[r] = z;
  }
  if constexpr (EPI == kEpiF32) {
    if (row < a.m_valid) *(f32x4*)(a.out_f32 + (long)row * a.ldf + col) = f32x4{y[0], y[1], y[2], y[3]};
  } else {
    const uint16_t h0 = to16<F16>(y[0]), h1 = to16<F16>(y[1]), h2 = to16<F16>(y[2]), h3 = to16<F16>(y[3]);
    unsigned int* dh = (unsigned int*)(a.out_hi + (long)row * a.ldo + col);
    dh[0] = (unsigned int)h0 | ((unsigned int)h1 << 16);
    dh[1] = (unsigned int)h2 | ((unsigned int)h3 << 16);
    if constexpr (SPLIT) {
      const uint16_t l0 = to16<F16>(y[0] - from16<F16>(h0)), l1 = to16<F16>(y[1] - from16<F16>(h1));
      const uint16_t l2 = to16<F16>(y[2] - from16<F16>(h2)), l3 = to16<F16>(y[3] - from16<F16>(h3));
      unsigned int* dl = (unsigned int*)(a.out_lo + (long)row * a.ldo + col);
      dl[0] = (unsigned int)l0 | ((unsigned int)l1 << 16);
      dl[1] = (unsigned int)l2 | ((unsigned int)l3 << 16);
    }
  }
}

template <int PREC, int EPI>
static hipError_t launch_splitk(const GemmArgs& a, hipStream_t s) {
  constexpr int lds = kTileBytes * (PrecXPlanes(PREC) + PrecWPlanes(PREC)) * kSplitKStages;
  static std::atomic<unsigned long long> attr_done{0};
  int attr_dev = 0;
  if (lds_attr_needed(&attr_done, &attr_dev)) {
    hipError_t e = hipFuncSetAttribute((const void*)tdnn_gemm_kernel<PREC, kEpiSplitK>,
                                       hipFuncAttributeMaxDynamicSharedMemorySize, lds);
    if (e != hipSuccess) return e;
    attr_done.fetch_or(1ull << (attr_dev & 63), std::memory_order_release);
  }
  dim3 grid(a.m_tiles * a.n_tiles, a.ksplit), block(256);
  note_kernel("", PREC, kEpiSplitK, 0);
  XV_LAUNCH((tdnn_gemm_kernel<PREC, kEpiSplitK>), grid, block, lds, s, a);
  hipError_t e = hipGetLastError();
  if (e != hipSuccess) return e;
  const long total = (long)a.m_tiles * kBM * (a.n_tiles * kBN / 4);
  XV_LAUNCH((splitk_reduce_kernel<PREC, EPI>), dim3((unsigned)((total + 255) / 256)), dim3(256), 0, s, a);
  return hipGetLastError();
}

template <int PREC>
static hipError_t launch_prec(const GemmArgs& a, int epi, hipStream_t s) {
  if constexpr (PREC == kPrecFp16x3E) {
    if (a.ksplit > 1 || epi != kEpiAct || !a.out_lo4 || !a.out_lo4s) return hipErrorInvalidValue;
    return launch_one<PREC, kEpiAct>(a, s);
  } else if constexpr (PREC == kPrecFp16MxE) {
// ... 929 lines not shown
```

Before: 358,300 utt/s.

## Share one LDS frame image across TDNN context shifts in p8 GEMM

Adds a shared-frames variant of the p8 TDNN GEMM kernel for activation epilogues. It stages one LDS image of the input frame block plus a small halo and serves every context shift of a group from it, with shifted read bases, instead of reloading a separate X tile per shift. The aim is to cut repeated global-to-LDS traffic for spliced inputs. In exchange it adds a new LDS layout and swizzle, more complex load scheduling and generic vmcnt waits, and it drops the paired-tile fast loop. It is enabled by default when every group's halo fits.

```diff
diff --git a/include/xvec_hip.h b/include/xvec_hip.h
--- a/include/xvec_hip.h
+++ b/include/xvec_hip.h
@@ -231,6 +231,7 @@
                                const int32_t* seg_klen, uint8_t* w4b, uint8_t* w4b_scale);
 xv_status xv_tile_mx_scales(const uint8_t* natural, int32_t n_pad, int32_t k_len, int32_t epilogue, uint8_t* tiled);
 xv_status xv_kernel_tdnn_gemm(const xv_gemm_desc* d);
+const char* xv_kernel_last_gemm(void);
 
 xv_status xv_compressed_size(int32_t rows, int32_t cols, int32_t method, size_t* nbytes, const char** format);
 xv_status xv_compress_matrices(int device, const float* feats, const int32_t* row_off, int32_t n, int32_t cols, int32_t method,
diff --git a/speaker-embedding-with-phonetic-information_amd/__init__.py b/speaker-embedding-with-phonetic-information_amd/__init__.py
--- a/speaker-embedding-with-phonetic-information_amd/__init__.py
+++ b/speaker-embedding-with-phonetic-information_amd/__init__.py
@@ -117,7 +117,7 @@
     "xv_ctx_profile_report", "xv_extract_utterances", "xv_ctx_calibrate", "xv_ctx_set_fast_mode", "xv_ctx_fast_mode",
     "xv_calibrate_table", "xv_ctx_set_calibration", "xv_ctx_model_fingerprint", "xv_ctx_share_calibration",
     "xv_ctx_set_calibration_file", "xv_calibration_file_read", "xv_calibration_file_publish", "xv_recognize_feature_pipeline", "xv_ctx_set_lite_layers", "xv_ctx_lite_layers",
-    "xv_extract_table", "xv_frontend_cmvn_select", "xv_plan_chunks", "xv_ctx_create_broadcast", "xv_kernel_tdnn_gemm",
+    "xv_extract_table", "xv_frontend_cmvn_select", "xv_plan_chunks", "xv_ctx_create_broadcast", "xv_kernel_tdnn_gemm", "xv_kernel_last_gemm",
     "xv_backend_apply", "xv_segment_mean", "xv_scatter_stats", "xv_plda_transform", "xv_plda_score", "xv_lda_estimate",
     "xv_plda_estimate", "xv_plda_adapt",
     "xv_mfcc_options_default", "xv_mfcc_num_frames", "xv_mfcc_utt_seed", "xv_mfcc_compute", "xv_mfcc_compute_i16", "xv_mfcc_kernel_time", "xv_vad_energy",
@@ -1032,6 +1032,12 @@
     _check(lib().xv_kernel_tdnn_gemm(ctypes.byref(desc)))
 
 
+def kernel_last_gemm():
+    f = lib().xv_kernel_last_gemm
+    f.restype = ctypes.c_char_p
+    return f().decode()
+
+
 def kernel_first_layer(desc):
     _check(lib().xv_kernel_first_layer(ctypes.byref(desc)))
 
diff --git a/speaker-embedding-with-phonetic-information_amd/csrc/capi.cc b/speaker-embedding-with-phonetic-information_amd/csrc/capi.cc
--- a/speaker-embedding-with-phonetic-information_amd/csrc/capi.cc
+++ b/speaker-embedding-with-phonetic-information_amd/csrc/capi.cc
@@ -17,6 +17,7 @@
 #include "reverb.h"
 #include "wave.h"
 #include "kernels.h"
+#include "knobs.h"
 #include "calib_file.h"
 #include "fuse_pipe.h"
 #include "fuse_wav.h"
@@ -1047,6 +1048,7 @@
     a.out_lo4 = (uint8_t*)d->out_lo4;
     a.out_lo4s = (uint8_t*)d->out_lo4_scale;
     a.p8 = d->p8;
+    a.p8_shared = xv::DebugKnobInt("p8_shared", xv::kP8SharedDefault);
     a.out_range = d->out_range;
     if (d->ksplit > 1) {
       if (d->precision < xv::kPrecBf16x3 || d->precision > xv::kPrecFp16x3 || a.p8 ||
@@ -1084,6 +1086,8 @@
     return XV_OK;
   });
 }
+
+const char* xv_kernel_last_gemm(void) { return xv::last_gemm_kernel(); }
 
 namespace {
 struct DevMem {
diff --git a/speaker-embedding-with-phonetic-information_amd/csrc/engine.cc b/speaker-embedding-with-phonetic-information_amd/csrc/engine.cc
--- a/speaker-embedding-with-phonetic-information_amd/csrc/engine.cc
+++ b/speaker-embedding-with-phonetic-information_amd/csrc/engine.cc
@@ -659,6 +659,7 @@
   {
     use_p8_ = DebugKnobInt("p8", 1) != 0;
     p8_whole_ = DebugKnobInt("p8_whole", 0);
+    p8_shared_ = DebugKnobInt("p8_shared", kP8SharedDefault);
   }
   in_ld_ = RoundUp(info_.input_dim, kBK);
   stats_ld_ = RoundUp(2 * info_.pool_dim, kBK);
@@ -1164,6 +1165,7 @@
   GemmArgs g8 = *g;
   g8.p8 = 1;
   g8.p8_whole = p8_whole_;
+  g8.p8_shared = p8_shared_;
   if (mx) {
     g8.w4 = dl.w4p;
     g8.w4_scale = dl.w4p_scale + so;
diff --git a/speaker-embedding-with-phonetic-information_amd/csrc/engine.h b/speaker-embedding-with-phonetic-information_amd/csrc/engine.h
--- a/speaker-embedding-with-phonetic-information_amd/csrc/engine.h
+++ b/speaker-embedding-with-phonetic-information_amd/csrc/engine.h
@@ -204,6 +204,7 @@
   bool fast_mx() const { return has_fast() && fast_mode_ != kPrecFp16x2; }
   bool fast_mx2() const { return has_fast() && fast_mode_ == kPrecFp16Mx2; }
   int p8_whole_ = 0;
+  int p8_shared_ = kP8SharedDefault;
   bool use_p8_ = true;
   bool logits16() const { return frame_mode_ && info_.precision == kPrecFp16 && info_.layers[info_.output_layer].log_softmax; }
   int fast_min_pooled_ = 0;
diff --git a/speaker-embedding-with-phonetic-information_amd/csrc/kernels.h b/speaker-embedding-with-phonetic-information_amd/csrc/kernels.h
--- a/speaker-embedding-with-phonetic-information_amd/csrc/kernels.h
+++ b/speaker-embedding-with-phonetic-information_amd/csrc/kernels.h
@@ -66,6 +66,13 @@
   int ld4s;
   int pad2_;
 };
+
+constexpr int kP8SharedDefault = 1;
+constexpr int kP8sImageRows = 264;
+constexpr int kP8sMaxHalo = 8;
+constexpr int P8sFrameSlot(int row, int chunk) { return (chunk + 2 * ((row >> 1) & 3)) & 7; }
+constexpr int P8sFrameAddr(int row, int chunk) { return row * 128 + P8sFrameSlot(row, chunk) * 16; }
+constexpr bool P8sGroupQualifies(int nshift, int dstep) { return nshift > 1 && dstep > 0 && (nshift - 1) * dstep <= kP8sMaxHalo; }
 
 struct WalkGroup {
   int first_seg, nshift, ksteps, shift0, dstep, wcol0, wstride;
@@ -198,6 +205,7 @@
   int p8;
   int p8_ktiles;
   int p8_whole;
+  int p8_shared;
   int p8_ktiles_lo;
 };
 
diff --git a/speaker-embedding-with-phonetic-information_amd/csrc/kernels.hip b/speaker-embedding-with-phonetic-information_amd/csrc/kernels.hip
--- a/speaker-embedding-with-phonetic-information_amd/csrc/kernels.hip
+++ b/speaker-embedding-with-phonetic-information_amd/csrc/kernels.hip
@@ -1934,6 +1934,7 @@
 constexpr int kP8WSL = kP8PB + 2 * 3072;
 constexpr int kP8XSL = kP8WSL + 2 * 2048;
 constexpr int kP8Lds = kP8XSL + 2 * 1024;
+constexpr int kP8Img = kP8sImageRows * 128;
 
 __device__ __forceinline__ void wait_vmcnt_n(int n) {
   switch (n) {
@@ -1972,12 +1973,16 @@
 }
 #endif
 
-template <int PREC, int EPI>
-__global__ __launch_bounds__(512) void tdnn_gemm_kernel_p8(const GemmArgs a) {
+template <int PREC, int EPI, bool SHARED>
+__device__ __forceinline__ void tdnn_gemm_p8_body(const GemmArgs& a) {
   static_assert(PREC == kPrecFp16 || PREC == kPrecFp16Mx || PREC == kPrecFp16Mx2 || PREC == kPrecFp16MxE,
                 "single-pass fp16, the 1.25-pass arithmetic (with or without the residual plane of its output), the 1.5-pass arithmetic");
   constexpr bool MX = PrecMx(PREC);
   constexpr bool MX2 = PrecMx2(PREC);
+  static_assert(!(SHARED && (MX2 || EPI != kEpiAct)), "shared frames: the act epilogue of fp16, fp16mx, fp16mxe");
+  constexpr int OFS = SHARED ? 2 * (kP8Img - kP8XW) : 0;
+  constexpr int kW4o = kP8W4 + OFS, kSCo = kP8SC + OFS, kPBo = kP8PB + OFS;
+  static_assert(kPBo + 2 * 3072 <= kP8Lds, "LDS");
   constexpr bool SWAP = (EPI != kEpiStats);
   extern __shared__ __attribute__((aligned(16))) char smem[];
   const int tid = threadIdx.x;
@@ -2030,7 +2035,7 @@
 #pragma unroll
     for (int j = 0; j < 2; ++j) {
       const int ru = wave * 16 + j * 8 + (l >> 3);
-      const int c = (l & 7) ^ ((j * 4 + (l >> 4)) & 7);
+      const int c = (SHARED && !weights) ? (((l & 7) - 2 * (l >> 4)) & 7) : ((l & 7) ^ ((j * 4 + (l >> 4)) & 7));
       int row = ru;
       if (weights) {
         const int rho = ru & 63;
@@ -2065,7 +2070,7 @@
   const char* wtile = nullptr;
   int x_next = 0, x_wrap = 0, w_next = 0, w_wrap = 0;
   auto bind_group = [&]() __attribute__((always_inline)) {
-    if constexpr (!RECOMPUTE) unit_offsets(gi.ld, false, xoff_r);
+    if constexpr (!RECOMPUTE && !SHARED) unit_offsets(gi.ld, false, xoff_r);
     xb = (const char*)gi.hi + ((long)(m0 + gi.shift0 + ij * gi.dstep) * gi.ld + ic * 64) * 2;
     x_next = gi.dstep * gi.ld * 2;
     x_wrap = 128 - (gi.nshift - 1) * gi.dstep * gi.ld * 2;
@@ -2096,7 +2101,7 @@
   };
   auto issue = [&](const int unit, const int buf) __attribute__((always_inline)) {
     if (unit == 0 || unit == 3) {
-      const unsigned dst = st_lane + 2 * kP8XW + buf * kP8XW + (unit == 3 ? kP8Unit : 0);
+      const unsigned dst = st_lane + OFS + 2 * kP8XW + buf * kP8XW + (unit == 3 ? kP8Unit : 0);
       const char* src = wb + (unit == 3 ? (long)a.ldw * 128 : 0);
       unsigned woff[2] = {woff_r[0], woff_r[1]};
       if constexpr (RECOMPUTE) unit_offsets(a.ldw, true, woff);
@@ -2113,7 +2118,7 @@
   };
   auto issue_w4 = [&](const int blk) __attribute__((always_inline)) {
     if constexpr (MX) {
-      const unsigned d4 = lds_base + kP8W4 + wave * 2048;
+      const unsigned d4 = lds_base + kW4o + wave * 2048;
       unsigned woff4[2] = {woff4_r[0], woff4_r[1]};
       if constexpr (RECOMPUTE) w4_offsets(woff4);
       const uint8_t* w4t = a.w4 + (long)n0 * a.ldw4 + blk * 64;
@@ -2121,7 +2126,7 @@
       glds16_sbase(w4t, woff4[1], d4 + 1024);
       const int pc = wave & 3;
       glds4_sbase(a.w4_scale + ((long)(nt * 2 + (pc >> 1)) * (S >> 1) + blk) * 512 + (pc & 1) * 256, (unsigned)lane * 4u,
-                  lds_base + kP8SC + pc * 256);
+                  lds_base + kSCo + pc * 256);
     }
   };
   auto issue_scales = [&](const int sb) __attribute__((always_inline)) {
@@ -2135,10 +2140,70 @@
     }
   };
 
+  int rbg = 0, rbc = 0, rij = 0, r_ns = 1, r_ds = 0, r_nc = 1, rimg = 0;
+  int tiles_left = 0;
+  int xq_left = 0, xs_left = 0;
+  unsigned xo0 = 0u, xo1 = 0u;
+  int xsg = -1, x_ld = 0, x_halo = 1;
+  const char* xib = nullptr;
+  int xcur0 = 0;
+  auto img_setup = [&](const int g, const int c) __attribute__((always_inline)) {
+    const Grp& G = a.grp[g];
+    if (g != xsg) {
+      xsg = g;
+      unsigned off[2];
+      unit_offsets(G.ld, false, off);
+      xo0 = off[0];
+      xo1 = off[1];
+    }
+    x_ld = G.ld;
+    x_halo = (G.nshift - 1) * G.dstep;
+    xib = (const char*)G.hi + ((long)(m0 + G.shift0) * G.ld + c * 64) * 2;
+  };
+  auto img_piece = [&](const int k, const int img) __attribute__((always_inline)) {
+    if (k == 0 && wave == 7) {
+      const int l = lane_now();
+      const int r = min(l >> 3, x_halo - 1);
+      const int c = ((l & 7) - 2 * (l >> 4)) & 7;
+      glds16_sbase_m0(xib, (unsigned)((256 + r) * x_ld + c * 8) * 2u, lds_base + img * kP8Img + 256 * 128);
+    }
+    const char* src = xib + (long)(k >> 1) * x_ld * 256;
+    glds16_sbase_m0(src, (k & 1) ? xo1 : xo0, st_lane + img * kP8Img + (k >> 1) * kP8Unit + (k & 1) * 1024);
+  };
+  auto x_bases = [&]() __attribute__((always_inline)) {
+    const int row = wm * 64 + fr_i + rij * r_ds;
+    xcur0 = rimg * kP8Img + row * 128 + P8sFrameSlot(row, fr_g) * 16;
+  };
+  auto stage_next_block = [&]() __attribute__((always_inline)) {
+    xq_left = 0;
+    xs_left = 2 * (r_ns - rij) - 1;
+    if (tiles_left > r_ns - rij) {
+      const bool wrap = rbc + 1 == r_nc;
+      img_setup(wrap ? rbg + 1 : rbg, wrap ? 0 : rbc + 1);
+      xq_left = 4;
+    }
+  };
+  auto rd_adv = [&]() __attribute__((always_inline)) {
+    if (--tiles_left <= 0) return;
+    if (++rij == r_ns) {
+      rij = 0;
+      rimg ^= 1;
+      if (++rbc == r_nc) {
+        rbc = 0;
+        ++rbg;
+        r_ns = a.grp[rbg].nshift;
+        r_ds = a.grp[rbg].dstep;
+        r_nc = a.grp[rbg].ksteps >> 1;
+      }
+      stage_next_block();
+    }
+    x_bases();
+  };
+
   const int sw = (fr_g ^ ((fr_i >> 1) & 7)) * 16;
   const int xrd0 = (wm * 64 + fr_i) * 128 + sw, xrd1 = xrd0 ^ 64;
-  const int wrd0 = 2 * kP8XW + (wn * 64 + fr_i) * 128 + sw, wrd1 = wrd0 ^ 64;
-  const int w4rd = kP8W4 + (wn * 64 + fr_i) * 64 + (fr_g ^ ((fr_i >> 1) & 3)) * 16;
+  const int wrd0 = OFS + 2 * kP8XW + (wn * 64 + fr_i) * 128 + sw, wrd1 = wrd0 ^ 64;
+  const int w4rd = kW4o + (wn * 64 + fr_i) * 64 + (fr_g ^ ((fr_i >> 1) & 3)) * 16;
 
   int xs_b = 0;
   float xs_f[MX ? 4 : 1];
@@ -2186,8 +2251,8 @@
     constexpr int P = decltype(PP)::value, B = decltype(BB)::value, ODD = decltype(OO)::value;
     constexpr bool LO = decltype(LL)::value != 0;
     constexpr bool FAST = decltype(FF)::value != 0;
-    const char* xs0 = smem + xrd0 + B * kP8XW;
-    const char* xs1 = smem + xrd1 + B * kP8XW;
+    const char* xs0 = SHARED ? smem + xcur0 : smem + xrd0 + B * kP8XW;
+    const char* xs1 = SHARED ? smem + (xcur0 ^ 64) : smem + xrd1 + B * kP8XW;
     const char* ws0 = smem + wrd0 + B * kP8XW;
     const char* ws1 = smem + wrd1 + B * kP8XW;
     XV_FUZZ();
@@ -2245,7 +2310,19 @@
       c2 = c1;
       c1 = c0;
       c0 = 0;
-      if (unit >= 0) {
+      if constexpr (SHARED && (P == 0 || P == 3)) {
+        const int n = xq_left > xs_left ? 2 : (xq_left > 0 ? 1 : 0);
+        if (n > 0) {
+          img_piece(4 - xq_left, rimg ^ 1);
+          --xq_left;
+        }
+        if (n > 1) {
+          img_piece(4 - xq_left, rimg ^ 1);
+          --xq_left;
+        }
+        --xs_left;
+        c0 += n;
+      } else if (unit >= 0) {
         issue(unit, ibuf);
         c0 += 2;
       }
@@ -2259,11 +2336,11 @@
       }
       __builtin_amdgcn_sched_barrier(0);
       if constexpr (P == 1) {
-        if (!MX2 && steady) asm volatile("s_waitcnt vmcnt(%0)" ::"n"(8 + E1) : "memory");
+        if (!SHARED && !MX2 && steady) asm volatile("s_waitcnt vmcnt(%0)" ::"n"(8 + E1) : "memory");
         else wait_vmcnt_n(c0 + c1 + c2 + c3);
       }
       if constexpr (P == 3) {
-        if (!MX2 && steady) asm volatile("s_waitcnt vmcnt(%0)" ::"n"(6 + E1) : "memory");
+        if (!SHARED && !MX2 && steady) asm volatile("s_waitcnt vmcnt(%0)" ::"n"(6 + E1) : "memory");
         else wait_vmcnt_n(c0 + c1 + c2);
       }
     }
@@ -2275,6 +2352,7 @@
     constexpr int Q0 = (P == 0 || P == 3) ? 0 : 2;
     if (prio_load) __builtin_amdgcn_s_setprio(0);
     if (prio_mfma) __builtin_amdgcn_s_setprio(1);
+    if constexpr (SHARED && P == 3) rd_adv();
     if constexpr (MX2 && LO) {
       asm volatile("s_nop 4" ::: "memory");
       static_for<0, 2>([&](auto K) {
@@ -2307,7 +2385,7 @@
       });
     } else if constexpr (MX && ODD && P == 3) {
       int ws_v[2];
-      const char* sc = smem + kP8SC + wn * 512 + (fr_i * 4 + fr_g) * 4;
+      const char* sc = smem + kSCo + wn * 512 + (fr_i * 4 + fr_g) * 4;
       ws_v[0] = *(const int*)(sc);
       ws_v[1] = *(const int*)(sc + 256);
       static_for<0, 4>([&](auto PW) {
@@ -2443,12 +2521,12 @@
     if (EPI != kEpiSplitK && kind != 1 && wave < 6) {
 #pragma unroll
       for (int hh = 0; hh < 2; ++hh) {
-        const unsigned dst = lds_base + kP8PB + (part & 1) * 3072 + hh * 1536 + wave * 256;
+        const unsigned dst = lds_base + kPBo + (part & 1) * 3072 + hh * 1536 + wave * 256;
         if (wave < 2 || a.bn) {
           const float* src = (wave < 2 ? a.bias : wave < 4 ? a.scale : a.offset) + n0 + hh * 128 + (wave & 1) * 64;
           glds4_sbase(src, (unsigned)lane * 4u, dst);
         } else {
-          *(float*)(smem + kP8PB + (part & 1) * 3072 + hh * 1536 + wave * 256 + lane * 4) = wave < 4 ? 1.f : 0.f;
+          *(float*)(smem + kPBo + (part & 1) * 3072 + hh * 1536 + wave * 256 + lane * 4) = wave < 4 ? 1.f : 0.f;
         }
       }
     }
@@ -2457,6 +2535,26 @@
     if constexpr (MX) {
       if (first_walk) xs_request(gi.gmax, xg);
     }
+    if constexpr (SHARED) {
+      rbg = ig; rbc = ic; rij = ij; rimg = 0;
+      r_ns = gi.nshift; r_ds = gi.dstep; r_nc = gi.ksteps >> 1;
+      tiles_left = n_tiles_part;
+      img_setup(ig, ic);
+      for (int k = 0; k < 4; ++k) img_piece(k, 0);
+      x_bases();
+      issue(0, 0);
+      issue(3, 0);
+      if (n_tiles_part > 1) {
+        adv();
+        issue(0, 1);
+      }
+      stage_next_block();
+      if (xq_left) {
+        img_piece(0, 1);
+        img_piece(1, 1);
+        xq_left = 2;
+      }
+    } else {
     issue(0, 0);
     issue(1, 0);
     issue(2, 0);
@@ -2467,6 +2565,7 @@
       issue(0, 1);
       issue(1, 1);
       if (MX2 && it >= S) issue_scales(1);
+    }
     }
     if (MX && first_walk) xs_finish(xg);
   };
@@ -2548,7 +2647,7 @@
       }
     };
     int t = 0;
-    if constexpr (!MX2 && PREC != kPrecFp16MxE) {
+    if constexpr (!MX2 && PREC != kPrecFp16MxE && !SHARED) {
 #pragma nounroll
       for (; ntp - t > 3; t += 2) {
         enter_pair();
@@ -2568,7 +2667,7 @@
     XV_FUZZ();
     asm volatile("s_nop 15\n\ts_nop 15" ::: "memory");
     const int e_kind = kind, e_m0 = m0, e_n0 = n0;
-    const float* e_par = (const float*)(smem + kP8PB + (part & 1) * 3072 + wn * 1536);
+    const float* e_par = (const float*)(smem + kPBo + (part & 1) * 3072 + wn * 1536);
     if (part + 1 < n_parts) open_part(part + 1);
 #ifdef XVEC_CLOCK_PROBE
     const unsigned long long xp_e0 = __builtin_readcyclecounter();
@@ -2615,6 +2714,15 @@
     g_clock_probe[(slot * 512 + bid) * 2 + 1] = __builtin_amdgcn_s_memrealtime() - clk_r0;
   }
 #endif
+}
+
+template <int PREC, int EPI>
+__global__ __launch_bounds__(512) void tdnn_gemm_kernel_p8(const GemmArgs a) {
+  tdnn_gemm_p8_body<PREC, EPI, false>(a);
+}
+template <int PREC, int EPI>
+__global__ __launch_bounds__(512) void tdnn_gemm_kernel_p8s(const GemmArgs a) {
+  tdnn_gemm_p8_body<PREC, EPI, true>(a);
 }
 
 struct SkWorkspace {
@@ -2809,6 +2917,21 @@
   if (e != hipSuccess) return e;
   b.sk_ws = w.ws;
   b.sk_flags = w.flags;
+  if constexpr (EPI == kEpiAct && !PrecMx2(PREC)) {
+    bool shared = a.p8_shared != 0;
+    for (int i = 0; i < b.ngrp; ++i) shared = shared && P8sGroupQualifies(b.grp[i].nshift, b.grp[i].dstep);
+    if (shared) {
+      static std::atomic<unsigned long long> attr_done_s{0};
+      if (lds_attr_needed(&attr_done_s, &attr_dev)) {
+        e = hipFuncSetAttribute((const void*)tdnn_gemm_kernel_p8s<PREC, EPI>, hipFuncAttributeMaxDynamicSharedMemorySize, kP8Lds);
+        if (e != hipSuccess) return e;
+        attr_done_s.fetch_or(1ull << (attr_dev & 63), std::memory_order_release);
+      }
+      note_kernel("_p8s", PREC, EPI, 0);
+      XV_LAUNCH((tdnn_gemm_kernel_p8s<PREC, EPI>), dim3(grid), dim3(512), kP8Lds, s, b);
+      return hipGetLastError();
+    }
+  }
   note_kernel("_p8", PREC, EPI, 0);
   XV_LAUNCH((tdnn_gemm_kernel_p8<PREC, EPI>), dim3(grid), dim3(512), kP8Lds, s, b);
   return hipGetLastError();
```

Measured after the change: 330,400 utt/s. 7.8% lower.
